# minyoungg/pix2latent

Hardware: AMD Instinct MI355X
Metric: candidate-latent evals/sec (fwd+loss+bwd), BigGAN-256 pop=18 (higher is better)
Workload: dtype f32 (fp32 tensors everywhere; convolutions >= 32x32 and the self-attention multiply on the 16-bit MFMA pipe with fp32-grade operand splits and fp32 accumulate: the 16x16 Winograd, direct and sub-pixel 3x3 kernels and the 1x1 kernels (4x4 layers included) on power-of-two scaled operands in 2 fp16 pie

## Files before the change

### include/p2l.h

```cpp
#ifndef P2L_H_
#define P2L_H_

#include <stddef.h>
#include <stdint.h>

#ifdef __cplusplus
extern "C" {
#endif

#define P2L_OK 0
#define P2L_EINVAL (-1)
#define P2L_ELAUNCH (-2)
#define P2L_EWS (-3)
#define P2L_EUNSUP (-4)

int p2l_version(void);
const char* p2l_strerror(int rc);
int p2l_last_hip_error(void);


enum { P2L_ACT_NONE = 0, P2L_ACT_RELU = 1, P2L_ACT_TANH = 2,
       P2L_ACT_LRELU_SQRT2 = 3  };
enum { P2L_POOL_NONE = 0, P2L_POOL_MAX = 1, P2L_POOL_SUM = 2 };
enum { P2L_PRO_NONE = 0, P2L_PRO_AFFINE_RELU = 1, P2L_PRO_AFFINE = 2 };
// ... 49 lines not shown
int p2l_conv_arb_nblk(const P2LConv* d);
int p2l_conv_dgrad_arb(const P2LConv* d, const P2LArb* arb, const float* dy,
                       const float* w, float* dx, void* stream);
int p2l_conv_arb_split_fusable(const P2LConv* d);
int p2l_conv_arb_nblk_ws(const P2LConv* d);
int p2l_conv_dgrad_arb_ws(const P2LConv* d, const P2LArb* arb, const float* dy, const float* w,
                          float* dx, void* workspace, size_t ws_bytes, void* stream);
int p2l_arb_finish(const float* partial, float* ds, float* dt, int Bn, int nblk, int C,
                   int out_bstride, void* stream);
void p2l_arb_defer_begin(void);
int p2l_arb_defer_flush(void* stream);
void p2l_arb_defer_cancel(void);

int p2l_prof_begin(int max_launches);
typedef struct P2LProfTotals {
  uint32_t size;
  int32_t count[2];
  int32_t reserved0;
  double flops[2];
  double ms[2];
  double bytes[2];
  double exec_flops[2];
  double mfma_flops[2];
  double write_bytes[2];
  int32_t fam_count[8];
  double fam_ms[8], fam_flops[8], fam_mfma_flops[8], fam_bytes[8];
} P2LProfTotals;
enum { P2L_PROF_FAM_OTHER = 0,
       P2L_PROF_FAM_WINO_H2 = 1,
       P2L_PROF_FAM_DIRECT_H2 = 2,
       P2L_PROF_FAM_SUBPIX_H2 = 3,
       P2L_PROF_FAM_THIN = 4,
       P2L_PROF_FAM_PW = 5,
       P2L_PROF_FAM_DIRECT_H2R = 6 };
int p2l_prof_totals(P2LProfTotals* out);
int p2l_prof_step(int step, int period);
int p2l_prof_dump(const char* path);

typedef struct P2LConvExtra {
  const float* oscale;
  int32_t oscale_bstride;
  const float* noise;
  float noise_w;
  P2LAmax amax;
} P2LConvExtra;
int p2l_conv_amax_slots(const P2LConv* d);
int p2l_conv_fwd_ex(const P2LConv* d, const P2LConvExtra* ex, const float* x,
                    const float* w, const float* bias, const float* pro_s,
                    const float* pro_t, const float* res, const float* mask, float* y,
                    float* yp, void* workspace, size_t ws_bytes, void* stream);

int p2l_pack_conv_weight(const float* w_oihw, int O, int I, int taps, int N_pad,
                         int K_pad, int transpose_flip, float* w_packed,
                         void* stream);

int p2l_pack_conv_weight_subpix(const float* w_oihw, int O, int I, int N_pad,
                                int K_pad, int transpose_flip, int mode,
                                float* w_packed, void* stream);

enum { P2L_WFMT_F32 = 0, P2L_WFMT_BF16X3 = 1, P2L_WFMT_BF16X3W = 2, P2L_WFMT_PW = 3,
       P2L_WFMT_BF16X3T = 4, P2L_WFMT_FLAG_PW = 0x10, P2L_WFMT_FLAG_THIN = 0x20,
       P2L_WFMT_FLAG_ATTN_GEMM = 0x40,
       P2L_WFMT_FLAG_NO_AMAX = 0x80
                                       };
int p2l_pack_conv_weight_bf3t(const float* w_oihw, int O, int I, int N_pad, int K_pad,
                              int transpose_flip, float* w_packed, void* stream);
int p2l_pack_conv_weight_pw(const float* w_oihw, int O, int I, int N_pad, int K_pad,
                            int transpose_flip, float* w_packed, void* stream);
size_t p2l_packed_weight_floats(int taps, int N_pad, int K_pad, int wfmt);
enum {
  P2L_FORM_AUTO = 0,
  P2L_FORM_NO_WINO = 1,
  P2L_FORM_WINO_ANY = 2,
  P2L_FORM_WINO_8X16 = 4,
  P2L_FORM_NO_PW = 8,
  P2L_FORM_NO_THIN = 16,
  P2L_FORM_WINO_BF3 = 32,
  P2L_FORM_WINO_H2_8X16 = 64,
  P2L_FORM_WINO_H2_16X16 = 128,
  P2L_FORM_NO_H2R = 256,
  P2L_FORM_H2R_SEQ_EPI = 512,
  P2L_FORM_NO_SP_SKIP = 1024,
  P2L_FORM_NO_SP_PAIR = 2048,
  P2L_FORM_SP_PAIR = 4096
};
int p2l_wino_split_factor(int H, int W, int Cin, int Cout);
int p2l_pack_conv_weight_bf3w(const float* w_oihw, int O, int I, int taps, int N_pad,
                              int K_pad, int transpose_flip, float* w_packed, void* stream);
int p2l_pack_conv_weight_bf3(const float* w_oihw, int O, int I, int taps, int N_pad,
                             int K_pad, int transpose_flip, float* w_packed, void* stream);
int p2l_pack_conv_weight_subpix_bf3(const float* w_oihw, int O, int I, int N_pad, int K_pad,
                                    int transpose_flip, int mode, float* w_packed,
                                    void* stream);
size_t p2l_packed_subpix_weight_floats(int N_pad, int K_pad, int wfmt);
int p2l_pack_conv_weight_subpix_h2(const float* w_oihw, int O, int I, int N_pad, int K_pad,
                                   int transpose_flip, int mode, float* w_packed, void* stream);

typedef struct P2LGemm {
  int32_t batch, M, N, K;
  int32_t lda, ldb, ldc;
  int64_t stride_a, stride_b, stride_c;
  int32_t a_kmajor, b_kmajor;
  float alpha;
  int32_t accumulate;
} P2LGemm;
int p2l_gemm(const P2LGemm* d, const float* A, const float* B, float* C,
             void* stream);
size_t p2l_gemm_ws_bytes(const P2LGemm* d);
int p2l_gemm_ws(const P2LGemm* d, const float* A, const float* B, float* C, void* ws,
                size_t ws_bytes, void* stream);

typedef struct P2LAttn {
  int32_t B, Nq, Nk, d, dv;
} P2LAttn;
int p2l_attn_supported(const P2LAttn* d);
size_t p2l_attn_fwd_ws_bytes(const P2LAttn* d);
int p2l_attn_fwd(const P2LAttn* d, const float* q, const float* k, const float* v, float* out,
                 float* lse, void* ws, size_t ws_bytes, void* stream);
size_t p2l_attn_bwd_dv_ws_bytes(const P2LAttn* d);
int p2l_attn_bwd_dv(const P2LAttn* d, const float* q, const float* k, const float* dout,
                    const float* lse, float* dv, void* ws, size_t ws_bytes, void* stream);
size_t p2l_attn_bwd_qk_ws_bytes(const P2LAttn* d);
int p2l_attn_bwd_qk(const P2LAttn* d, const float* q, const float* k, const float* v,
                    const float* out, const float* dout, const float* lse, float* dst, float* dq,
                    float* dk, void* ws, size_t ws_bytes, void* stream);

int p2l_linear_fwd(const float* x, const float* W, const float* bias, float* y,
                   int Bn, int K, int N, void* stream);
int p2l_linear_bwd(const float* dy, const float* W, float* dx, int Bn, int K,
                   int N, int accumulate, void* stream);
int p2l_linear_fwd_ld(const float* x, int x_ld, const float* W, const float* bias, float* y,
                      int Bn, int K, int N, void* stream);
int p2l_linear_bwd_ld(const float* dy, const float* W, float* dx, int dx_ld, int Bn, int K,
                      int N, int accumulate, void* stream);

int p2l_cbn_fold_fwd(const float* g_raw, const float* b_raw, const float* mean,
                     const float* rstd, float* s, float* t, int Bn, int C,
                     int raw_ld, void* stream);
int p2l_cbn_fold_bwd(const float* ds, const float* dt, const float* mean,
                     const float* rstd, float* dg_raw, float* db_raw, int Bn,
                     int C, int raw_ld, void* stream);

int p2l_affine_relu_bwd_nblk(int P);
int p2l_affine_relu_bwd(const float* da, int da_ld, const float* x, int x_ld,
                        const float* s, const float* t, int st_bstride,
                        const float* skip, int skip_ld, int skip_C, int skip_ups,
                        float* dx, int dx_ld, float* ds, float* dt,
                        int dsdt_bstride, float* partial, int Bn, int H, int W,
                        int C, void* stream);

int p2l_scale_bwd(const float* da, int da_ld, const float* x, int x_ld, const float* s,
                  int st_bstride, const float* skip, int skip_ld, int skip_C, float* dx,
                  int dx_ld, float* ds, float* dt_scratch, int dsdt_bstride, float* partial,
                  int Bn, int H, int W, int C, void* stream);

int p2l_softmax_fwd(const float* S, float* P, int64_t rows, int cols,
                    void* stream);
int p2l_softmax_bwd(const float* P, const float* dP, float* dS, int64_t rows,
                    int cols, void* stream);

int p2l_maxpool2_bwd(const float* y, int y_ld, const float* dyp, int dyp_ld,
                     const float* add, int add_ld, float* dy, int dy_ld, int Bn,
                     int H, int W, int C, int relu_mask, void* stream);
int p2l_maxpool2_bwd_amax_slots(int H, int W, int C);
int p2l_maxpool2_bwd_amax(const float* y, int y_ld, const float* dyp, int dyp_ld,
                          const float* add, int add_ld, float* dy, int dy_ld, int Bn, int H,
                          int W, int C, int relu_mask, float* amax_out, void* stream);
int p2l_relu_mask(const float* y, int y_ld, const float* g, int g_ld, float* dy,
// ... 364 lines not shown
```

### pix2latent_amd/_native.py

```python
import ctypes as C
import os

import torch

_HERE = os.path.dirname(os.path.abspath(__file__))
LIB_PATH = os.environ.get('P2L_LIB_PATH') or os.path.join(_HERE, 'libp2l_hip.so')

c_float_p = C.c_void_p


class P2LConv(C.Structure):
    _fields_ = [('B', C.c_int32), ('H', C.c_int32), ('W', C.c_int32),
                ('Cin', C.c_int32), ('Cout', C.c_int32), ('taps', C.c_int32),
                ('ups', C.c_int32), ('x_ld', C.c_int32), ('pro', C.c_int32),
                ('pro_bstride', C.c_int32), ('alpha', C.c_float), ('act', C.c_int32),
                ('pool', C.c_int32), ('y_ld', C.c_int32), ('yp_ld', C.c_int32),
                ('n_store', C.c_int32), ('res_ld', C.c_int32), ('res_ups', C.c_int32),
                ('mask_ld', C.c_int32), ('splitk', C.c_int32), ('ext', C.c_int32),
                ('wfmt', C.c_int32), ('form', C.c_int32), ('algo_flops', C.c_double),
                ('w_floats', C.c_int64)]


class P2LAmax(C.Structure):
    _fields_ = [('out', C.c_void_p), ('outp', C.c_void_p), ('in_', C.c_void_p), ('in_n', C.c_int32),
# ... 62 lines not shown


class P2LSg2Rgb(C.Structure):
    _fields_ = [('cin', C.c_int32), ('res', C.c_int32), ('latent_idx', C.c_int32),
                ('after_conv', C.c_int32), ('w', C.c_void_p), ('wt', C.c_void_p),
                ('mod_w', C.c_void_p), ('mod_b', C.c_void_p), ('bias', C.c_void_p)]


class P2LStyleGAN2(C.Structure):
    _fields_ = [('size', C.c_int32), ('n_conv', C.c_int32), ('n_rgb', C.c_int32),
                ('style_dim', C.c_int32), ('n_latent', C.c_int32), ('noise_total', C.c_int32),
                ('map_w', C.c_void_p * 8), ('map_b', C.c_void_p * 8), ('const_input', C.c_void_p),
                ('conv', P2LSg2Conv * P2L_SG2_MAX_CONVS), ('rgb', P2LSg2Rgb * P2L_SG2_MAX_RGBS),
                ('wfmt', C.c_int32), ('reserved1', C.c_int32)]


class P2LVggLpips(C.Structure):
    _fields_ = [('w', C.c_void_p * 13), ('b', C.c_void_p * 13), ('wt', C.c_void_p * 13),
                ('lin', C.c_void_p * 5), ('in_s', C.c_void_p), ('in_t', C.c_void_p),
                ('wfmt', C.c_int32), ('reserved1', C.c_int32)]


class P2LGConv(C.Structure):
    _fields_ = [(n, C.c_int32) for n in (
        'B', 'Hi', 'Wi', 'Cin', 'Cout', 'KH', 'KW', 'stride', 'pad', 'x_ld', 'y_ld', 'res_ld',
        'mask_ld', 'n_store', 'relu', 'reserved0')]


class P2LAlexLpips(C.Structure):
    _fields_ = [('w', C.c_void_p * 5), ('b', C.c_void_p * 5), ('wt', C.c_void_p * 5),
                ('lin', C.c_void_p * 5), ('in_s', C.c_void_p), ('in_t', C.c_void_p)]


class P2LSqueezeLpips(C.Structure):
    _fields_ = [('w0', C.c_void_p), ('b0', C.c_void_p), ('wt0', C.c_void_p),
                ('sq_w', C.c_void_p * 8), ('sq_b', C.c_void_p * 8), ('e1_w', C.c_void_p * 8), ('e1_b', C.c_void_p * 8),
                ('e3_w', C.c_void_p * 8), ('e3_b', C.c_void_p * 8),
                ('sq_wt', C.c_void_p * 8), ('e1_wt', C.c_void_p * 8), ('e3_wt', C.c_void_p * 8),
                ('lin', C.c_void_p * 7), ('in_s', C.c_void_p), ('in_t', C.c_void_p)]


class P2LLossCache7(C.Structure):
    _fields_ = [('nft', C.c_void_p * 7), ('wt', C.c_void_p * 7), ('wsum', C.c_void_p)]


class P2LLossCache(C.Structure):
    _fields_ = [('nft', C.c_void_p * 5), ('wt', C.c_void_p * 5), ('wsum', C.c_void_p)]


class P2LProfTotals(C.Structure):
    _fields_ = [('size', C.c_uint32), ('count', C.c_int32 * 2), ('reserved0', C.c_int32),
                ('flops', C.c_double * 2), ('ms', C.c_double * 2), ('bytes', C.c_double * 2),
                ('exec_flops', C.c_double * 2), ('mfma_flops', C.c_double * 2),
                ('write_bytes', C.c_double * 2),
                ('fam_count', C.c_int32 * 8), ('fam_ms', C.c_double * 8), ('fam_flops', C.c_double * 8),
                ('fam_mfma_flops', C.c_double * 8), ('fam_bytes', C.c_double * 8)]


PROF_FAMILIES = {0: 'other (exact-fp32 / bf16x3 direct, 8x16 Winograd)', 1: 'wino16s_conv_kernel<.., H2>',
                 2: 'conv_h2_kernel<9, ..>', 3: 'conv_h2_kernel<4, ..>', 4: 'conv_thinin/thinout_kernel',
                 5: 'pw_h2_kernel / pw_conv_kernel', 6: 'conv_h2r_kernel<..>'}


def prof_totals():
    t = P2LProfTotals()
    t.size = C.sizeof(P2LProfTotals)
    check(lib().p2l_prof_totals(C.byref(t)), 'p2l_prof_totals')
    return t


prof_end = prof_totals


ACT_NONE, ACT_RELU, ACT_TANH, ACT_LRELU_SQRT2 = 0, 1, 2, 3
WFMT_F32, WFMT_BF16X3, WFMT_BF16X3W, WFMT_PW, WFMT_BF16X3T = 0, 1, 2, 3, 4
WFMT_FLAG_PW, WFMT_FLAG_THIN, WFMT_FLAG_ATTN_GEMM, WFMT_FLAG_NO_AMAX = 0x10, 0x20, 0x40, 0x80
FORM_AUTO, FORM_NO_WINO, FORM_WINO_ANY, FORM_WINO_8X16, FORM_NO_PW, FORM_NO_THIN, FORM_WINO_BF3 = 0, 1, 2, 4, 8, 16, 32
FORM_WINO_H2_8X16, FORM_WINO_H2_16X16 = 64, 128
FORM_H2R_SEQ_EPI = 512
FORM_NO_SP_SKIP = 1024
FORM_NO_SP_PAIR = 2048
FORM_SP_PAIR = 4096
FORM_NO_H2R = 256


def default_wfmt():
    v = os.environ.get('P2L_CONV_WFMT', 'bf16x3').lower()
    if v in ('f32', 'fp32', '0'):
        return WFMT_F32
    if v in ('bf16x3-direct', 'bf3d', '1'):
        return WFMT_BF16X3
    if v in ('bf16x3', 'bf3', 'bf16x3w', '2'):
        return WFMT_BF16X3W
    raise ValueError('P2L_CONV_WFMT=%r (expected f32, bf16x3 or bf16x3-direct)' % v)


def default_thin():
    return os.environ.get('P2L_THIN', '1') != '0' and default_wfmt() != WFMT_F32


def default_attn_gemm():
    return os.environ.get('P2L_ATTN', '1') == '0'


def default_no_amax():
    return os.environ.get('P2L_AMAX', '1') == '0'


def default_pw():
    return os.environ.get('P2L_PW', '1') != '0' and default_wfmt() != WFMT_F32


def pack_conv_weight(src, taps, n_pad, k_pad, flip, wfmt, subpix_mode=None):
    L = lib()
    O, I = src.shape[0], src.shape[1]
    src = src.detach().float().contiguous()
    if taps == 1 and wfmt == WFMT_PW:
        dst = torch.empty(L.p2l_packed_weight_floats(1, n_pad, k_pad, WFMT_PW), device=src.device,
                          dtype=torch.float32)
        check(L.p2l_pack_conv_weight_pw(ptr(src), O, I, n_pad, k_pad, int(flip), ptr(dst), stream()),
              'p2l_pack_conv_weight_pw')
        return dst
    if taps != 9:
        wfmt = WFMT_F32
    if subpix_mode is not None:
        dst = torch.empty(L.p2l_packed_subpix_weight_floats(n_pad, k_pad, wfmt), device=src.device,
                          dtype=torch.float32)
        fn = {WFMT_F32: L.p2l_pack_conv_weight_subpix,
              WFMT_BF16X3W: L.p2l_pack_conv_weight_subpix_h2}.get(wfmt, L.p2l_pack_conv_weight_subpix_bf3)
        check(fn(ptr(src), O, I, n_pad, k_pad, int(flip), int(subpix_mode), ptr(dst), stream()),
              'p2l_pack_conv_weight_subpix')
        return dst
    n = L.p2l_packed_weight_floats(taps, n_pad, k_pad, wfmt)
    dst = torch.empty(n, device=src.device, dtype=torch.float32)
    if wfmt == WFMT_BF16X3T:
        check(L.p2l_pack_conv_weight_bf3t(ptr(src), O, I, n_pad, k_pad, int(flip), ptr(dst), stream()),
              'p2l_pack_conv_weight_bf3t')
        return dst
    fn = {WFMT_F32: L.p2l_pack_conv_weight, WFMT_BF16X3: L.p2l_pack_conv_weight_bf3,
          WFMT_BF16X3W: L.p2l_pack_conv_weight_bf3w}[wfmt]
    check(fn(ptr(src), O, I, taps, n_pad, k_pad, int(flip), ptr(dst), stream()),
          'p2l_pack_conv_weight')
    return dst
def pack_gconv_weight(src, taps, n_pad, k_pad, flip):
    L = lib()
    src = src.detach().float().contiguous()
    dst = torch.empty(taps * n_pad * k_pad, device=src.device, dtype=torch.float32)
    check(L.p2l_pack_gconv_weight(ptr(src), src.shape[0], src.shape[1], taps, n_pad, k_pad, int(flip), ptr(dst),
                                  stream()), 'p2l_pack_gconv_weight')
    return dst


POOL_NONE, POOL_MAX, POOL_SUM = 0, 1, 2
PRO_NONE, PRO_AFFINE_RELU, PRO_AFFINE = 0, 1, 2

EXPORTS = [
    'p2l_version', 'p2l_strerror', 'p2l_last_hip_error',
    'p2l_conv_workspace_bytes', 'p2l_conv_amax_slots', 'p2l_selftest_amaxreg', 'p2l_conv_suggest_splitk', 'p2l_conv_fwd', 'p2l_conv_fwd_ex',
    'p2l_pack_conv_weight', 'p2l_pack_conv_weight_subpix', 'p2l_pack_conv_weight_bf3',
    'p2l_pack_conv_weight_bf3w', 'p2l_packed_weight_floats', 
    'p2l_pack_conv_weight_bf3t',
    'p2l_pack_conv_weight_pw', 'p2l_adam_step_dev',
    'p2l_attn_supported', 'p2l_attn_fwd_ws_bytes', 'p2l_attn_fwd', 'p2l_attn_bwd_dv_ws_bytes',
    'p2l_attn_bwd_dv', 'p2l_attn_bwd_qk_ws_bytes', 'p2l_attn_bwd_qk',
    'p2l_pack_conv_weight_subpix_bf3', 'p2l_pack_conv_weight_subpix_h2', 'p2l_packed_subpix_weight_floats', 'p2l_gemm', 'p2l_gemm_ws_bytes', 'p2l_gemm_ws', 'p2l_linear_fwd', 'p2l_linear_bwd',
    'p2l_cbn_fold_fwd', 'p2l_cbn_fold_bwd', 'p2l_affine_relu_bwd_nblk',
    'p2l_affine_relu_bwd', 'p2l_softmax_fwd', 'p2l_softmax_bwd', 'p2l_maxpool2_bwd', 'p2l_maxpool2_bwd_amax', 'p2l_maxpool2_bwd_amax_slots',
    'p2l_relu_mask', 'p2l_nchw3_to_nhwc16', 'p2l_nhwc16_to_nchw3', 'p2l_tanh_bwd16',
    'p2l_weight_sum', 'p2l_weight_map', 'p2l_l1_loss_nblk', 'p2l_l1_loss_fwd',
    'p2l_l1_loss_bwd', 'p2l_lpips_normalize', 'p2l_lpips_tap_nblk', 'p2l_lpips_tap_fwd',
    'p2l_lpips_tap_bwd', 'p2l_lpips_tap_pool_bwd', 'p2l_bilinear_adjoint', 'p2l_reduce_rows', 'p2l_adam_step',
    'p2l_clamp', 'p2l_affine_grid_sample', 'p2l_affine_grid_sample_bwd', 'p2l_affine_grid_sample_bwd_ws_bytes', 'p2l_vec_scale_div', 'p2l_concat2', 'p2l_split2',
    'p2l_biggan_ws_bytes', 'p2l_biggan_fwd', 'p2l_biggan_bwd', 'p2l_biggan_ws_lookup',
    'p2l_loss_cache_floats', 'p2l_projloss_ws_bytes', 'p2l_projloss_ws_lookup', 'p2l_projloss_prepare',
    'p2l_projloss_fwd', 'p2l_projloss_bwd', 'p2l_mfma_probe', 'p2l_prof_begin', 'p2l_prof_totals', 'p2l_prof_step', 'p2l_prof_dump', 'p2l_wino_split_factor', 'p2l_linear_fwd_ld', 'p2l_linear_bwd_ld', 'p2l_scale_bwd',
    'p2l_sg2_pixelnorm_fwd', 'p2l_sg2_pixelnorm_bwd', 'p2l_sg2_bias_lrelu_fwd', 'p2l_sg2_lrelu_bwd',
    'p2l_sg2_demod_fwd', 'p2l_sg2_demod_bwd', 'p2l_sg2_blur_fwd', 'p2l_sg2_act_bwd_nblk',
    'p2l_sg2_styled_act_bwd', 'p2l_sg2_blur_bwd', 'p2l_sg2_rgb_up_fwd', 'p2l_sg2_rgb_up_bwd',
    'p2l_sg2_clamp16_fwd', 'p2l_sg2_clamp16_bwd', 'p2l_broadcast_rows', 'p2l_add_inplace',
    'p2l_sg2_ws_bytes', 'p2l_sg2_ws_lookup', 'p2l_sg2_synthesis_fwd', 'p2l_sg2_synthesis_bwd', 'p2l_sg2_mapping_fwd',
    'p2l_sg2_mapping_bwd', 'p2l_conv_arb_fusable', 'p2l_conv_arb_nblk',
    'p2l_conv_dgrad_arb', 'p2l_conv_arb_split_fusable', 'p2l_conv_arb_nblk_ws',
    'p2l_conv_dgrad_arb_ws', 'p2l_arb_finish', 'p2l_arb_defer_begin', 'p2l_arb_defer_flush',
    'p2l_arb_defer_cancel',
    'p2l_gconv_fwd', 'p2l_maxpool3s2_fwd', 'p2l_maxpool3s2_bwd', 'p2l_conv1_dgrad',
    'p2l_alex_cache_floats', 'p2l_alexloss_ws_bytes', 'p2l_alexloss_prepare', 'p2l_alexloss_fwd',
    'p2l_alexloss_bwd',
    'p2l_pack_gconv_weight', 'p2l_sqz_cache_floats', 'p2l_sqzloss_ws_bytes', 'p2l_sqzloss_prepare', 'p2l_sqzloss_fwd',
    'p2l_sqzloss_bwd', 'p2l_sqzloss_ws_lookup',
    'p2l_sg2_blur_fwd_amax', 'p2l_sg2_styled_act_bwd_amax', 'p2l_sg2_blur_bwd_amax', 'p2l_sg2_noise_relayout',
    'p2l_sg2_rows_defer_begin', 'p2l_sg2_rows_defer_flush', 'p2l_sg2_rows_defer_cancel',
    'p2l_color_adjust_ws_bytes', 'p2l_color_adjust',
    'p2l_gram_f64_ws_bytes', 'p2l_gram_f64', 'p2l_gram_f64_wide_ws_bytes', 'p2l_gram_f64_wide',
    'p2l_poisson_blend_ws_bytes', 'p2l_poisson_blend',
    'p2l_sg2_noise_reg_ws_bytes', 'p2l_sg2_noise_reg_fwd', 'p2l_sg2_noise_reg_bwd', 'p2l_sg2_noise_normalize',
    'p2l_area_pool3_to_nhwc16', 'p2l_area_pool_nchw', 'p2l_area_unpool16_add_nchw3',
    'p2l_latent_prior_ws_bytes', 'p2l_latent_prior_fwd', 'p2l_latent_prior_bwd',
    'p2l_l2_loss_nblk', 'p2l_l2_loss_fwd', 'p2l_l2_loss_bwd', 'p2l_adam_step_sched',
]

_lib = None
ABI_VERSION = 101


class NativeError(RuntimeError):
    pass


def lib():
    global _lib
    if _lib is None:
        if not os.path.exists(LIB_PATH):
            raise NativeError(
                'libp2l_hip.so not found at %s: the HIP extension is required '
                '(no CPU fallback). Run __graft_entry__.build().' % LIB_PATH)
        _lib = C.CDLL(LIB_PATH)
        if _lib.p2l_version() < ABI_VERSION:
            v, _lib = _lib.p2l_version(), None
            raise NativeError('libp2l_hip.so at %s is version %d, this package binds version %d: rebuild it '
                              '(__graft_entry__.build())' % (LIB_PATH, v, ABI_VERSION))
        _lib.p2l_strerror.restype = C.c_char_p
        _lib.p2l_arb_defer_begin.restype = None
        _lib.p2l_arb_defer_cancel.restype = None
        _lib.p2l_sg2_rows_defer_begin.restype = None
        _lib.p2l_sg2_rows_defer_cancel.restype = None
        for name in ('p2l_conv_workspace_bytes', 'p2l_biggan_ws_bytes',
                     'p2l_projloss_ws_bytes', 'p2l_loss_cache_floats', 'p2l_sg2_ws_bytes',
                     'p2l_alexloss_ws_bytes', 'p2l_alex_cache_floats', 'p2l_sqzloss_ws_bytes', 'p2l_sqz_cache_floats', 'p2l_gemm_ws_bytes',
                     'p2l_packed_weight_floats', 'p2l_packed_subpix_weight_floats', 'p2l_attn_fwd_ws_bytes', 'p2l_affine_grid_sample_bwd_ws_bytes',
                     'p2l_attn_bwd_dv_ws_bytes', 'p2l_attn_bwd_qk_ws_bytes', 'p2l_color_adjust_ws_bytes',
                     'p2l_gram_f64_ws_bytes', 'p2l_gram_f64_wide_ws_bytes', 'p2l_poisson_blend_ws_bytes',
                     'p2l_sg2_noise_reg_ws_bytes', 'p2l_latent_prior_ws_bytes'):
            getattr(_lib, name).restype = C.c_size_t
        vp, i32, i64_, f32_ = C.c_void_p, C.c_int, C.c_int64, C.c_float
        _lib.p2l_relu_mask.argtypes = [vp, i32, vp, i32, vp, i32, i64_, i32, vp]
        _lib.p2l_tanh_bwd16.argtypes = [vp, vp, i64_, vp]
        _lib.p2l_clamp.argtypes = [vp, i64_, f32_, f32_, vp]
        _lib.p2l_adam_step.argtypes = [vp, vp, vp, vp, i64_, f32_, f32_, f32_, f32_, i32, vp]
        _lib.p2l_adam_step_dev.argtypes = [vp, vp, vp, vp, i64_, f32_, f32_, f32_, f32_, vp, i32, vp]
        _lib.p2l_adam_step_sched.argtypes = [vp, vp, vp, vp, i64_, vp, i32, f32_, f32_, f32_, vp, i32, vp]
        _lib.p2l_l2_loss_nblk.argtypes = [i32, i32]
        _lib.p2l_l2_loss_fwd.argtypes = [vp, vp, vp, vp, vp, vp, vp, i32, i32, i32, vp]
        _lib.p2l_l2_loss_bwd.argtypes = [vp, vp, vp, vp, vp, vp, vp, i32, i32, i32, i32, vp]
        _lib.p2l_reduce_rows.argtypes = [vp, vp, i32, i32, f32_, vp, i32, vp]
        _lib.p2l_vec_scale_div.argtypes = [vp, vp, vp, i32, f32_, vp]
        _lib.p2l_sg2_bias_lrelu_fwd.argtypes = [vp, vp, f32_, i32, i32, vp]
        _lib.p2l_sg2_clamp16_fwd.argtypes = [vp, vp, i64_, vp]
        _lib.p2l_sg2_clamp16_bwd.argtypes = [vp, vp, vp, i64_, vp]
        _lib.p2l_broadcast_rows.argtypes = [vp, vp, i64_, i32, vp]
        _lib.p2l_add_inplace.argtypes = [vp, vp, i64_, vp]
        _lib.p2l_sg2_styled_act_bwd.argtypes = [vp, vp, vp, vp, f32_, vp, vp, vp, vp, vp, vp, i32, i32, i32, vp]
        _lib.p2l_sg2_styled_act_bwd_amax.argtypes = [vp, vp, vp, vp, f32_, vp, vp, vp, vp, vp, vp, i32, i32, i32, vp, vp]
        _lib.p2l_softmax_fwd.argtypes = [vp, vp, i64_, i32, vp]
        _lib.p2l_softmax_bwd.argtypes = [vp, vp, vp, i64_, i32, vp]
        _lib.p2l_sg2_blur_fwd.argtypes = [vp, vp, vp, f32_, vp, vp, i32, i32, i32, i32, vp]
        _lib.p2l_sg2_blur_fwd_amax.argtypes = [vp, vp, vp, f32_, vp, vp, i32, i32, i32, i32, vp, vp, vp]
        _lib.p2l_sg2_blur_bwd.argtypes = [vp, vp, i32, i32, i32, i32, vp]
        _lib.p2l_sg2_blur_bwd_amax.argtypes = [vp, vp, i32, i32, i32, i32, vp, vp]
        _lib.p2l_gram_f64_ws_bytes.argtypes = [C.c_int64, C.c_int, C.c_int]
        _lib.p2l_gram_f64.argtypes = [C.c_void_p, C.c_int64, C.c_int, C.c_int64, C.c_int, C.c_void_p,
                                      C.c_void_p, C.c_void_p, C.c_size_t, C.c_void_p]
        _lib.p2l_gram_f64_wide_ws_bytes.argtypes = [C.c_int64, C.c_int]
        _lib.p2l_gram_f64_wide.argtypes = [C.c_void_p, C.c_int64, C.c_int, C.c_int64, C.c_void_p, C.c_void_p,
                                           C.c_void_p, C.c_size_t, C.c_void_p]
        _lib.p2l_poisson_blend_ws_bytes.argtypes = [i32, i32, i32, i32]
        _lib.p2l_poisson_blend.argtypes = [vp, i64_, vp, i64_, vp, vp, i32, i32, i32, i32, C.c_double, i32,
                                           vp, vp, vp, C.c_size_t, vp]
        _lib.p2l_poisson_blend.restype = i32
        _lib.p2l_sg2_noise_reg_ws_bytes.argtypes = [vp, i32, i32]
        _lib.p2l_sg2_noise_reg_fwd.argtypes = [vp, vp, i32, i32, vp, vp, vp, C.c_size_t, vp]
        _lib.p2l_sg2_noise_reg_bwd.argtypes = [vp, vp, i32, i32, vp, vp, vp, C.c_size_t, vp]
        _lib.p2l_sg2_noise_normalize.argtypes = [vp, vp, i32, i32, vp, C.c_size_t, vp]
        _lib.p2l_area_pool3_to_nhwc16.argtypes = [vp, vp, i32, i32, i32, i32, vp]
        _lib.p2l_area_pool_nchw.argtypes = [vp, vp, vp, i32, i32, i32, i32, i32, vp]
        _lib.p2l_area_unpool16_add_nchw3.argtypes = [vp, vp, vp, i32, i32, i32, i32, vp]
        _lib.p2l_latent_prior_ws_bytes.argtypes = [i32, i32, i32]
        _lib.p2l_latent_prior_fwd.argtypes = [vp, vp, vp, vp, i32, i32, i32, i32, i32, vp, vp, C.c_size_t, vp]
        _lib.p2l_latent_prior_bwd.argtypes = [vp, vp, vp, vp, i32, i32, i32, i32, i32, vp, C.c_size_t, vp, vp]
    return _lib


def check(rc, what=''):
    if rc != 0:
        L = lib()
        raise NativeError('%s failed: %s (rc=%d, hipError=%d)' % (
            what or 'p2l call', L.p2l_strerror(rc).decode(), rc, L.p2l_last_hip_error()))


def ptr(t):
    if t is None:
        return C.c_void_p(0)
    assert t.dtype == torch.float32 and t.is_contiguous(), 'expect contiguous fp32'
    return C.c_void_p(t.data_ptr())


def stream():
    return C.c_void_p(torch.cuda.current_stream().cuda_stream)


def f32(v):
    return C.c_float(float(v))


def i64(v):
    return C.c_int64(int(v))
```

### pix2latent_amd/csrc/p2l_conv.hip

```cpp
#include "p2l_conv_k.h"

#include <cstdlib>
#include <cstring>
#include <cstddef>
#include <array>
#include <atomic>
#include <cstdio>
#include <mutex>
#include <string>
#include <vector>

using namespace p2lconv;

namespace {

struct ConvProf {
  std::atomic<bool> on{false};
  int n = 0;
  std::vector<hipEvent_t> ev;
  std::vector<double> flops;
  std::vector<double> xflops;
  std::vector<int> nprod;
  std::vector<double> bytes;
  std::vector<double> wbytes;
// ... 981 lines not shown
  const int nchunks = 4 * (d->Cin / 16);
  while (s > 1 && nchunks / s < 8) s >>= 1;
  return s <= 2 ? 1 : s;
}

extern "C" int p2l_conv_suggest_splitk(const P2LConv* d) {
  ConvK k{};
  if (d && d->ups == 3 && d->ext) return subpix_bwd_split(d);
  if (!d || d->ups >= 2) return 1;
  if (choose_tile(d, k) == P2L_OK && wino_split(d) > 1 && !(d->form & P2L_FORM_WINO_ANY) &&
      (d->H / 8) * (d->W / 16) * (d->Cout / 64) < 64)
    return wino_split(d);
  if (choose_tile(d, k) != P2L_OK || k.partial || wino_shape(d) || pw_any(d)) return 1;
  return direct_split(d);
}

static bool wino_h2(const P2LConv* d) {
  return wino_shape(d) && d->H % 16 == 0 && d->W % 16 == 0 &&
         !(d->form & (P2L_FORM_WINO_8X16 | P2L_FORM_WINO_BF3));
}
static int effective_splitk(const P2LConv* d);
static bool finish_v4_ok(const P2LConv* d) {
#ifdef P2L_AB_SCALAR_FINISH
  return false;
#endif
  return d->n_store % 4 == 0 && d->Cout % 4 == 0 && d->y_ld % 4 == 0 && d->yp_ld % 4 == 0 &&
         d->res_ld % 4 == 0 && d->mask_ld % 4 == 0;
}
extern "C" int p2l_conv_amax_slots(const P2LConv* d) {
  if (!d) return 0;
  if (wino_shape(d)) {
    if (d->H % 16 || d->W % 16 || (d->form & P2L_FORM_WINO_8X16)) return 0;
    if (d->splitk > 1 && wino_split(d) == d->splitk) {
      const int per_image = (d->H / 2) * (d->W / 2) * (d->n_store / 4);
      return (per_image % 64 == 0 && d->n_store % 4 == 0) ? per_image / 64 : 0;
    }
    return (d->H / 16) * (d->W / 16) * (d->Cout / 64) * 8;
  }
  if (d->ups == 3 && effective_splitk(d) > 1) return 0;
  if (effective_splitk(d) > 1) {
    const int per_image = (d->H / 2) * (d->W / 2) * (finish_v4_ok(d) ? d->n_store / 4 : d->n_store);
    return (per_image % 64 == 0) ? per_image / 64 : 0;
  }
  ConvK k{};
  if (choose_tile(d, k) != P2L_OK || k.tb_log != 0 || k.partial) return 0;
  const int tm = thin_shape(d);
  if (tm >= 0) {
    const bool geom = k.tw_log == 4 && k.th_log == 3;
    return (tm == 1 && geom) ? k.tiles_x * k.tiles_y * 4 : 0;
  }
#ifdef P2L_AB_PW_SLOTS_R4
  const int nnt = pw_shape(d) ? d->Cout / 64 : d->Cout / choose_bn(d, k.n_mtiles);
#else
  const int nnt = (pw_shape(d) || pw_small_h2(d)) ? d->Cout / 64 : direct_h2r(d) ? 1 : d->Cout / choose_bn(d, k.n_mtiles);
#endif
  return k.tiles_x * k.tiles_y * nnt * (d->ups == 2 ? 4 : 1) * 4;
}
extern "C" size_t p2l_conv_workspace_bytes(const P2LConv* d) {
  const size_t h2 = (wino_h2(d) || direct_h2(d) || pw_small_h2(d)) ? (size_t)d->B * 64 * sizeof(float) : 0;
  if (d->splitk <= 1) return h2;
  return h2 + (size_t)d->splitk * d->B * d->H * d->W * d->Cout * sizeof(float);
}

static int effective_splitk(const P2LConv* d) {
  if (d->splitk > 1 && d->ups == 3 && d->ext && subpix_bwd_split(d) > 1) {
    const int nchunks = 4 * (d->Cin / 16);
    const int sk = d->splitk > nchunks ? nchunks : d->splitk;
    return cdiv(nchunks, cdiv(nchunks, sk));
  }
  if (d->splitk > 1 && d->ups == 0 && wino_split(d) == d->splitk && wino_shape(d)) return d->splitk;
  if (d->splitk <= 1 || d->ups >= 2 || wino_shape(d) || pw_any(d)) return 1;
  const int kc = (d->taps == 9) ? 16 : (d->Cin % 32 == 0 ? 32 : 16);
  const int nchunks = d->Cin / kc;
  int sk = d->splitk > nchunks ? nchunks : d->splitk;
  const int per = cdiv(nchunks, sk);
  return cdiv(nchunks, per);
}

static int conv_launch_impl(const P2LConv* d, const P2LArb* arb, const P2LConvExtra* ex,
                            const float* x, const float* w,
                            const float* bias, const float* pro_s,
                            const float* pro_t, const float* res,
                            const float* mask, float* y, float* yp,
                            void* workspace, size_t ws_bytes, void* stream) {
  if (!d || !x || !w) return P2L_EINVAL;
  if (d->taps != 1 && d->taps != 9) return P2L_EINVAL;
  const int kc = (d->taps == 9) ? 16 : (d->Cin % 32 == 0 ? 32 : 16);
  if (d->Cin % kc || d->Cout % 32 || d->B < 1) return P2L_EINVAL;
  if (d->x_ld % 4 || d->x_ld < d->Cin) return P2L_EINVAL;
  if (d->pro != P2L_PRO_NONE && (!pro_s || !pro_t || d->pro_bstride % 4)) return P2L_EINVAL;
  if (d->pool != P2L_POOL_NONE && !yp) return P2L_EINVAL;
  if (!y && !yp) return P2L_EINVAL;
  if (d->ups && d->taps != 9) return P2L_EUNSUP;
  if (d->taps == 9 && d->wfmt != P2L_WFMT_F32 && d->wfmt != P2L_WFMT_BF16X3 &&
      d->wfmt != P2L_WFMT_BF16X3W && d->wfmt != P2L_WFMT_BF16X3T)
    return P2L_EUNSUP;
  if (d->taps == 1 && d->wfmt != P2L_WFMT_F32 && d->wfmt != P2L_WFMT_PW) return P2L_EUNSUP;
  if (d->ups < 0 || d->ups > 3) return P2L_EINVAL;
  if (d->w_floats != 0) {
    const size_t need = d->ups >= 2 ? p2l_packed_subpix_weight_floats(d->Cout, d->Cin, d->wfmt)
                                    : p2l_packed_weight_floats(d->taps, d->Cout, d->Cin, d->wfmt);
    if (d->w_floats < 0 || (size_t)d->w_floats < need) return P2L_EINVAL;
  }
  if (d->n_store < 1 || d->n_store > d->Cout || d->n_store % 4) return P2L_EINVAL;
  if ((y && d->y_ld % 4) || (yp && d->yp_ld % 4) || (res && d->res_ld % 4) ||
      (mask && d->mask_ld % 4))
    return P2L_EINVAL;
  if ((y && d->y_ld < d->n_store) || (yp && d->yp_ld < d->n_store) || (res && d->res_ld < d->n_store) ||
      (mask && d->mask_ld < d->n_store))
    return P2L_EINVAL;
  if (d->pro != P2L_PRO_NONE && d->pro_bstride != 0 && d->pro_bstride < d->Cin) return P2L_EINVAL;
  if (arb) {
    if (arb->x && arb->x_ld < d->n_store) return P2L_EINVAL;
    if (arb->st_bstride != 0 && arb->st_bstride < d->n_store) return P2L_EINVAL;
    if (arb->skip && (arb->skip_C < 0 || arb->skip_C > d->n_store || arb->skip_ld < arb->skip_C)) return P2L_EINVAL;
  }
  if (ex && ex->oscale && ex->oscale_bstride != 0 && ex->oscale_bstride < d->n_store) return P2L_EINVAL;
  {
    const int64_t px = (int64_t)d->B * d->H * d->W;
    int64_t ldmax = d->x_ld;
    if (d->y_ld > ldmax) ldmax = d->y_ld;
    if (d->res_ld > ldmax) ldmax = d->res_ld;
    if (d->mask_ld > ldmax) ldmax = d->mask_ld;
    if (px * ldmax >= ((int64_t)1 << 31)) return P2L_EUNSUP;
  }

  ConvK k{};
  k.x = x; k.w = w; k.bias = bias; k.pro_s = pro_s; k.pro_t = pro_t;
  k.res = res; k.mask = mask; k.y = y; k.yp = yp; k.ws = (float*)workspace;
  k.B = d->B; k.H = d->H; k.W = d->W; k.Cin = d->Cin; k.Cout = d->Cout;
  k.x_ld = d->x_ld; k.y_ld = d->y_ld; k.yp_ld = d->yp_ld; k.res_ld = d->res_ld;
  k.mask_ld = d->mask_ld; k.n_store = d->n_store; k.pro_bstride = d->pro_bstride;
  k.alpha = d->alpha; k.act = d->act; k.pool = d->pool; k.res_ups = d->res_ups;
  k.ups = d->ups;
  k.form = d->form;
  int rc = choose_tile(d, k);
  if (rc) return rc;
  k.iH = d->H; k.iW = d->W; k.ibH = d->H; k.ibW = d->W; k.obH = d->H; k.obW = d->W;
  k.hp = halo_pitch(1 << k.tw_log, d->wfmt != P2L_WFMT_F32 && d->taps == 9);
  const bool bf3_3x3 = d->taps == 9 && d->wfmt != P2L_WFMT_F32;
  if (ex) {
    k.oscale = ex->oscale; k.oscale_bstride = ex->oscale_bstride;
    k.noise = ex->noise; k.noise_w = ex->noise_w;
  }
  if ((k.oscale || k.noise || d->act == P2L_ACT_LRELU_SQRT2) && !finish_v4_ok(d) && !wino_shape(d) &&
      effective_splitk(d) > 1)
    return P2L_EUNSUP;
  if (k.partial && (arb || d->pool != P2L_POOL_NONE || d->splitk > 1)) return P2L_EUNSUP;
  if (arb) {
    if ((k.tb_log != 0 && effective_splitk(d) <= 1) || res || mask || d->act != P2L_ACT_NONE ||
        d->pool == P2L_POOL_MAX || !arb->x || !arb->s || !arb->t || !arb->partial)
      return P2L_EUNSUP;
    k.arb_x = arb->x; k.arb_s = arb->s; k.arb_t = arb->t; k.arb_skip = arb->skip;
    k.arb_partial = arb->partial; k.arb_x_ld = arb->x_ld; k.arb_bstride = arb->st_bstride;
    k.arb_skip_ld = arb->skip_ld; k.arb_skip_C = arb->skip_C; k.arb_skip_ups = arb->skip_ups;
    k.arb_nblk = k.n_mtiles / d->B;
    k.arb_nomask = arb->nomask;
  }
  const int bn = direct_h2r(d) ? 64 : choose_bn(d, k.n_mtiles);
  k.n_ntiles = d->Cout / bn;
  k.nchunks = d->Cin / kc;
  const bool wino_sliced = wino_shape(d) && d->splitk > 1 && wino_split(d) == d->splitk;
  k.splitk = (d->splitk < 1 || (wino_shape(d) && !wino_sliced) || pw_any(d)) ? 1 : d->splitk;
  if (k.splitk > k.nchunks) k.splitk = k.nchunks;
  k.chunks_per_split = cdiv(k.nchunks, k.splitk);
  k.splitk = cdiv(k.nchunks, k.chunks_per_split);
  const bool h2_direct = direct_h2(d), h2_pw_small = pw_small_h2(d);
  const size_t h2_bytes = (wino_h2(d) || h2_direct || h2_pw_small) ? (size_t)d->B * 64 * sizeof(float) : 0;
  const bool use_h2 = h2_bytes && workspace &&
                      ws_bytes >= h2_bytes + (k.splitk > 1 ? (size_t)k.splitk * d->B * d->H * d->W * d->Cout * sizeof(float) : 0);
  if (use_h2) {
    k.amax = (float*)workspace;
    k.ws = (float*)workspace + (size_t)d->B * 64;
  }
  {
    const P2LAmax* am = ex ? &ex->amax : (arb ? &arb->amax : nullptr);
    if (am && am->in && am->in_n > 0 && !(am->in_applied && d->pro == P2L_PRO_NONE) &&
        (use_h2 || (pw_shape(d) && !(d->form & P2L_FORM_WINO_BF3)))) {
      k.amax_in = am->in; k.amax_in_n = am->in_n;
      k.amax_in_applied = am->in_applied ? 1 : 0;
    }
    int nslots = (am && (am->out || am->outp)) ? p2l_conv_amax_slots(d) : 0;
    if (thin_shape(d) >= 0 && ex && (ex->oscale || ex->noise)) nslots = 0;
    if (nslots > 0 && h2_pw_small && !use_h2 && effective_splitk(d) <= 1) return P2L_EWS;
    if (nslots > 0 && direct_h2r(d) && !use_h2) return P2L_EWS;
    if (nslots > 0) { k.amax_out = am->out; k.amax_outp = am->outp; k.amax_out_n = nslots; }
    if (nslots > 0 && am->out && am->next_s && am->next_t && !arb) {
      if (am->next_bstride != 0 && am->next_bstride < d->n_store) return P2L_EINVAL;
      k.amax_ps = am->next_s; k.amax_pt = am->next_t; k.amax_pbstride = am->next_bstride;
    }
  }
  if (k.splitk > 1) {
    const size_t need = (use_h2 ? h2_bytes : 0) + (size_t)k.splitk * d->B * d->H * d->W * d->Cout * sizeof(float);
    if (!workspace || ws_bytes < need) return P2L_EWS;
    if (arb) k.arb_nblk = p2l_conv_arb_nblk_ws(d);
    if (arb && d->ups < 2 && !wino_shape(d) && finish_v4_ok(d) &&
        (arb->x_ld % 4 || (arb->skip && arb->skip_ld % 4)))
      return P2L_EINVAL;
  }
  hipStream_t st = (hipStream_t)stream;

  int prof_slot = -1;
  bool prof_ok = g_prof.on;
  if (prof_ok) {
    hipStreamCaptureStatus cs = hipStreamCaptureStatusNone;
    if (hipStreamIsCapturing(st, &cs) != hipSuccess || cs != hipStreamCaptureStatusNone) prof_ok = false;
  }
  if (prof_ok) {
    std::lock_guard<std::mutex> lk(g_prof.mu);
    if (g_prof.on && g_prof.n < (int)g_prof.flops.size() && (g_prof.seq++ % g_prof.period) == g_prof.phase)
      prof_slot = g_prof.n++;
  }
  if (prof_slot >= 0) {
    g_prof.flops[prof_slot] = d->algo_flops > 0.0
        ? d->algo_flops
        : 2.0 * d->B * d->H * d->W * (double)d->Cin * d->Cout * d->taps;
    g_prof.xflops[prof_slot] =
        2.0 * d->B * d->H * d->W * (double)d->Cin * d->Cout * (d->ups >= 2 ? 4 : d->taps);
    g_prof.kind[prof_slot] = d->taps == 9 ? 0 : 1;
    g_prof.fam[prof_slot] = P2L_PROF_FAM_OTHER;
    g_prof.nprod[prof_slot] = (d->wfmt == P2L_WFMT_F32 || (d->taps == 1 && !pw_shape(d))) ? 16 : 6;
    g_prof.shape[prof_slot] = {d->taps, d->B, d->H, d->W, d->Cin, d->Cout, d->ups, d->pro,
                               arb ? (arb->skip ? 2 : 1) : 0, d->splitk};
    {
      const double opx = (double)d->B * d->H * d->W;
      const double ipx = d->ups == 1 || d->ups == 2 ? opx / 4 : (d->ups == 3 ? opx * 4 : opx);
      double by = ipx * d->Cin + (double)d->taps * d->Cin * d->Cout;
      if (y) by += opx * d->n_store;
      if (yp) by += opx / 4 * d->n_store;
      if (res) by += (d->res_ups ? opx / 4 : opx) * d->n_store;
      if (mask) by += opx * d->n_store;
      if (arb) by += opx * d->n_store * (arb->skip ? 2.0 : 1.0);
      g_prof.bytes[prof_slot] = 4.0 * by;
      g_prof.wbytes[prof_slot] = 4.0 * ((y ? opx * d->n_store : 0.0) + (yp ? opx / 4 * d->n_store : 0.0));
    }
    (void)hipEventRecord(g_prof.ev[2 * prof_slot], st);
  }
  if (wino_shape(d)) {
    ConvK kw = k;
    kw.w = w + (size_t)9 * d->Cout * d->Cin * 3 / 2;
    if (use_h2) {
      kw.w += p2l_wino_weight_floats(d->Cout, d->Cin);
      kw.w_tail = reinterpret_cast<const unsigned*>(kw.w + (size_t)d->Cout * d->Cin * 16);
    }
    kw.tiles_x = d->W / 16; kw.tiles_y = d->H / 8;
    kw.n_mtiles = d->B * kw.tiles_x * kw.tiles_y;
    kw.n_ntiles = d->Cout / 64;
    kw.nchunks = d->Cin / 16;
    if (wino_sliced) {
      kw.splitk = d->splitk;
      kw.chunks_per_split = kw.nchunks / kw.splitk;
    } else {
      kw.splitk = 1;
    }
    rc = p2l_wino_launch(kw, d->pro, st);
    if (rc == P2L_OK && wino_sliced) {
      const size_t total = (size_t)k.B * (k.H >> 1) * (k.W >> 1) * (k.n_store >> 2);
      hipLaunchKernelGGL(conv_splitk_finish4, dim3(cdiv(total, 256)), dim3(256), 0, st, k);
      rc = p2l_check_launch();
    }
    if (prof_slot >= 0) {
      g_prof.xflops[prof_slot] = 2.0 * d->B * d->H * d->W * (double)d->Cin * d->Cout * 4;
      if (use_h2) g_prof.nprod[prof_slot] = 3;
      g_prof.fam[prof_slot] = use_h2 ? P2L_PROF_FAM_WINO_H2 : P2L_PROF_FAM_OTHER;
      (void)hipEventRecord(g_prof.ev[2 * prof_slot + 1], st);
    }
    return rc;
  }
  if (pw_shape(d)) {
    ConvK kp = k;
    kp.w = w + (size_t)d->Cout * d->Cin;
    if (k.amax_in != nullptr) {
      kp.w += (size_t)d->Cout * d->Cin * 3 / 2;
      kp.w_tail = reinterpret_cast<const unsigned*>(kp.w + (size_t)d->Cout * d->Cin);
    }
    kp.n_ntiles = d->Cout / 64;
    kp.nchunks = d->Cin / 64;
    kp.splitk = 1;
    rc = p2l_pw_launch(kp, d->pro, st);
    if (prof_slot >= 0) {
      if (k.amax_in != nullptr) g_prof.nprod[prof_slot] = 3;
      g_prof.fam[prof_slot] = P2L_PROF_FAM_PW;
      (void)hipEventRecord(g_prof.ev[2 * prof_slot + 1], st);
    }
    return rc;
  }
  {
    const int tm = thin_shape(d);
    const bool geom = k.tw_log == 4 && k.th_log == 3 && k.tb_log == 0 && !k.partial && !(ex && (ex->oscale || ex->noise));
    if (tm == 1 && geom) {
      ConvK kt = k;
      kt.w = w + (size_t)9 * d->Cout * d->Cin * 3 / 2;
      kt.splitk = 1;
      rc = p2l_thinin_launch(kt, d->pro, st);
      if (prof_slot >= 0) {
        g_prof.xflops[prof_slot] = 2.0 * d->B * d->H * d->W * 32.0 * d->Cout;
        g_prof.fam[prof_slot] = P2L_PROF_FAM_THIN;
        (void)hipEventRecord(g_prof.ev[2 * prof_slot + 1], st);
      }
      return rc;
    }
    if (tm == 0 && geom && !arb && !res && !mask && d->pool == P2L_POOL_NONE && y) {
      ConvK kt = k;
      kt.w = w + (size_t)9 * d->Cout * d->Cin * 3 / 2;
      kt.nchunks = d->Cin / 16;
      kt.splitk = 1;
      rc = p2l_thinout_launch(kt, d->pro, st);
      if (prof_slot >= 0) {
        g_prof.xflops[prof_slot] = 2.0 * d->B * d->H * d->W * 1.5 * d->Cin * 32.0;
        g_prof.fam[prof_slot] = P2L_PROF_FAM_THIN;
        (void)hipEventRecord(g_prof.ev[2 * prof_slot + 1], st);
      }
      return rc;
    }
  }
  if (d->ups >= 2) {
    const int sk3 = (d->taps == 9 && d->splitk > 1) ? ((d->ups == 3 && d->ext) ? effective_splitk(d) : 1) : 1;
    if (sk3 > 1 && !(use_h2 && direct_h2(d))) return P2L_EWS;
    if (d->taps != 9 || (k.splitk != 1 && sk3 == 1) || d->Cin % 16 || d->pool != P2L_POOL_NONE ||
        (arb && k.tb_log != 0 && sk3 == 1) || (d->ups == 2 && (res || mask)))
      return P2L_EUNSUP;
    {
      int gH, gW;
      grid_dims(d, gH, gW);
      const int e = d->ext ? 1 : 0, e2 = d->ext ? 2 : 0;
      k.H = gH; k.W = gW;
      if (d->ups == 2) {
        k.iH = d->H >> 1; k.iW = d->W >> 1; k.ibH = k.iH; k.ibW = k.iW;
        k.obH = d->H + e2; k.obW = d->W + e2;
      } else {
        k.iH = (d->H >> 1) + e; k.iW = (d->W >> 1) + e;
        k.ibH = d->H + e2; k.ibW = d->W + e2;
        k.obH = gH; k.obW = gW;
      }
    }
    k.sp_mode = d->ups - 1;
    k.sp_skip = (d->ext && !(d->form & P2L_FORM_NO_SP_SKIP)) ? 1 : 0;
    k.sp_ncc = d->Cin / 16;
    k.nchunks = (d->ups == 3) ? 4 * k.sp_ncc : k.sp_ncc;
    k.chunks_per_split = cdiv(k.nchunks, sk3);
    k.splitk = sk3;
    k.ups = 0;
    const int a_rows_sp = (1 << k.tb_log) * ((1 << k.th_log) + 2) * ((1 << k.tw_log) + 2);
    const bool small_sp = (a_rows_sp * 4 <= 3 * 256) && k.tb_log == 0;
    const bool bf3 = bf3_3x3;
    if (use_h2 && h2_direct) {
      ConvK kh = k;
      kh.hp = halo_pitch_h2(1 << k.tw_log);
      kh.w = w + (size_t)16 * d->Cout * d->Cin * 3 / 2;
      kh.w_tail = reinterpret_cast<const unsigned*>(kh.w + (size_t)16 * d->Cout * d->Cin);
      if (kh.amax_in == nullptr) {
        ConvK ka = kh;
        ka.H = k.ibH; ka.W = k.ibW;
        rc = p2l_amax_launch(ka, d->pro, st);
        if (rc) return rc;
      }
#ifdef P2L_AB_NO_SP_PAIR
      const bool pair = d->ups == 2 && !(d->form & P2L_FORM_NO_SP_PAIR) && (d->form & P2L_FORM_SP_PAIR);
#else
      const bool pair = d->ups == 2 && !(d->form & P2L_FORM_NO_SP_PAIR) &&
                        ((d->ext && bn == 64) || (d->form & P2L_FORM_SP_PAIR));
#endif
      rc = p2l_h2_launch(kh, d->pro, pair ? 8 : 4, bn, small_sp, st);
      if (rc == P2L_OK && k.splitk > 1) {
        const bool arb_al = !arb || (k.arb_x_ld % 4 == 0 && (!k.arb_skip || k.arb_skip_ld % 4 == 0));
        if (finish_v4_ok(d) && arb_al) {
          const size_t total = (size_t)k.B * (k.H >> 1) * (k.W >> 1) * (k.n_store >> 2);
          hipLaunchKernelGGL(conv_splitk_finish_v4, dim3(cdiv(total, 64)), dim3(256), 0, st, k);
        } else {
          const size_t total = (size_t)k.B * (k.H >> 1) * (k.W >> 1) * k.n_store;
          hipLaunchKernelGGL(conv_splitk_finish, dim3(cdiv(total, 64)), dim3(256), 0, st, k);
        }
        rc = p2l_check_launch();
      }
      if (prof_slot >= 0) {
        g_prof.nprod[prof_slot] = 3;
        g_prof.fam[prof_slot] = P2L_PROF_FAM_SUBPIX_H2;
        (void)hipEventRecord(g_prof.ev[2 * prof_slot + 1], st);
      }
      return rc;
    }
    const int a_lds_sp = (1 << k.tb_log) * ((1 << k.th_log) + 2) * k.hp;
    size_t lds_sp = (size_t)(a_lds_sp + 4 * bn) * (bf3 ? 24 : 20) * sizeof(float);
    const size_t lds_epi = (size_t)4 * 32 * (bn + 4) * sizeof(float);
    if (lds_epi > lds_sp) lds_sp = lds_epi;
    dim3 grid(k.n_mtiles * k.n_ntiles, d->ups == 2 ? 4 : 1), block(256);
#define P2L_LAUNCH_SP(BNV, AIT, PROV)                                                     \
    do {                                                                                  \
      if (bf3) { P2L_LAUNCH_SP2(BNV, AIT, PROV, true); } else { P2L_LAUNCH_SP2(BNV, AIT, PROV, false); } \
    } while (0)
#define P2L_LAUNCH_SP2(BNV, AIT, PROV, BF3V)                                              \
    do {                                                                                  \
      auto kfn = pick_kernel<4, BNV, 16, AIT, PROV, false, BF3V>();                       \
      static std::atomic<bool> attr_set{false};                                                       \
      if (!attr_set) {                                                                    \
        (void)hipFuncSetAttribute((const void*)kfn,                                       \
                                  hipFuncAttributeMaxDynamicSharedMemorySize, 160 * 1024); \
        attr_set = true;                                                                  \
      }                                                                                   \
      hipLaunchKernelGGL(kfn, grid, block, lds_sp, st, k);                                \
    } while (0)
#define P2L_LAUNCH_SP_PRO(BNV, AIT)                                                       \
    do {                                                                                  \
      if (d->pro == P2L_PRO_NONE) P2L_LAUNCH_SP(BNV, AIT, P2L_PRO_NONE);                  \
      else if (d->pro == P2L_PRO_AFFINE_RELU) P2L_LAUNCH_SP(BNV, AIT, P2L_PRO_AFFINE_RELU); \
      else P2L_LAUNCH_SP(BNV, AIT, P2L_PRO_AFFINE);                                       \
    } while (0)
    if (bn == 64) {
      if (small_sp) P2L_LAUNCH_SP_PRO(64, 3); else P2L_LAUNCH_SP_PRO(64, 5);
    } else {
      if (small_sp) P2L_LAUNCH_SP_PRO(32, 3); else P2L_LAUNCH_SP_PRO(32, 5);
    }
#undef P2L_LAUNCH_SP_PRO
#undef P2L_LAUNCH_SP
#undef P2L_LAUNCH_SP2
    rc = p2l_check_launch();
    if (prof_slot >= 0) (void)hipEventRecord(g_prof.ev[2 * prof_slot + 1], st);
    return rc;
  }
  const int TW = 1 << k.tw_log, TH = 1 << k.th_log, TB = 1 << k.tb_log;
  const int a_rows = (d->taps == 9) ? TB * (TH + 2) * (TW + 2) : 128;
  const bool bf3 = bf3_3x3;
  const int a_rows_lds = (d->taps == 9) ? TB * (TH + 2) * k.hp : 128;
  size_t lds = (size_t)(a_rows_lds + d->taps * bn) * (bf3 ? 24 : kc + 4) * sizeof(float);
  {
    const size_t lds_epi = (size_t)4 * 32 * (bn + 4) * sizeof(float);
    if (lds_epi > lds) lds = lds_epi;
  }

  if (d->taps == 9 && use_h2 && h2_direct) {
    ConvK kh = k;
    kh.hp = halo_pitch_h2(TW);
    kh.w = w + (size_t)9 * d->Cout * d->Cin * 3 / 2;
    if (p2l_wino_weight_ok(d->Cout, d->Cin))
      kh.w += p2l_wino_weight_floats(d->Cout, d->Cin) + p2l_wino_h2_weight_floats(d->Cout, d->Cin);
    kh.w_tail = reinterpret_cast<const unsigned*>(kh.w + (size_t)9 * d->Cout * d->Cin);
    if (kh.amax_in == nullptr) {
      rc = p2l_amax_launch(kh, d->pro, st);
      if (rc) return rc;
    }
    const bool small = (a_rows * 4 <= 3 * 256) && TB == 1;
    const bool h2r = direct_h2r(d) && k.splitk == 1 && !k.partial && TB == 1 && p2l_h2r_takes(kh);
    rc = h2r ? p2l_h2r_launch(kh, d->pro, st) : p2l_h2_launch(kh, d->pro, 9, bn, small, st);
    if (prof_slot >= 0) { g_prof.nprod[prof_slot] = 3; g_prof.fam[prof_slot] = h2r ? P2L_PROF_FAM_DIRECT_H2R : P2L_PROF_FAM_DIRECT_H2; }
  } else
  if (d->taps == 9) {
    const bool small = (a_rows * 4 <= 3 * 256) && TB == 1;
    if (bf3) {
      if (bn == 64) rc = small ? launch_conv<9, 64, 16, 3, true>(k, d->pro, d->ups, lds, st)
                               : launch_conv<9, 64, 16, 5, true>(k, d->pro, d->ups, lds, st);
      else          rc = small ? launch_conv<9, 32, 16, 3, true>(k, d->pro, d->ups, lds, st)
                               : launch_conv<9, 32, 16, 5, true>(k, d->pro, d->ups, lds, st);
    } else
    if (bn == 64) rc = small ? launch_conv<9, 64, 16, 3>(k, d->pro, d->ups, lds, st)
                             : launch_conv<9, 64, 16, 5>(k, d->pro, d->ups, lds, st);
    else          rc = small ? launch_conv<9, 32, 16, 3>(k, d->pro, d->ups, lds, st)
                             : launch_conv<9, 32, 16, 5>(k, d->pro, d->ups, lds, st);
  } else if (d->taps == 1 && use_h2 && h2_pw_small) {
    ConvK kp = k;
    kp.w = w + (size_t)d->Cout * d->Cin + (size_t)d->Cout * d->Cin * 3 / 2;
    kp.w_tail = reinterpret_cast<const unsigned*>(kp.w + (size_t)d->Cout * d->Cin);
    kp.n_ntiles = d->Cout / 64;
    if (kp.amax_in == nullptr) {
      rc = p2l_amax_launch(kp, d->pro, st);
      if (rc) return rc;
    }
    rc = p2l_pw_launch(kp, d->pro, st);
    if (prof_slot >= 0) { g_prof.nprod[prof_slot] = 3; g_prof.fam[prof_slot] = P2L_PROF_FAM_PW; }
  } else if (kc == 32) {
    if (bn == 64) rc = launch_conv<1, 64, 32, 4>(k, d->pro, 0, lds, st);
    else          rc = launch_conv<1, 32, 32, 4>(k, d->pro, 0, lds, st);
  } else {
    if (bn == 64) rc = launch_conv<1, 64, 16, 2>(k, d->pro, 0, lds, st);
    else          rc = launch_conv<1, 32, 16, 2>(k, d->pro, 0, lds, st);
  }
  if (rc) return rc;
  if (k.splitk > 1) {
    if (finish_v4_ok(d)) {
      const size_t total = (size_t)k.B * (k.H >> 1) * (k.W >> 1) * (k.n_store >> 2);
      hipLaunchKernelGGL(conv_splitk_finish_v4, dim3(cdiv(total, 64)), dim3(256), 0, st, k);
    } else {
      const size_t total = (size_t)k.B * (k.H >> 1) * (k.W >> 1) * k.n_store;
      hipLaunchKernelGGL(conv_splitk_finish, dim3(cdiv(total, 64)), dim3(256), 0, st, k);
    }
    rc = p2l_check_launch();
  }
  if (prof_slot >= 0) (void)hipEventRecord(g_prof.ev[2 * prof_slot + 1], st);
  return rc;
}

extern "C" int p2l_conv_fwd(const P2LConv* d, const float* x, const float* w,
                            const float* bias, const float* pro_s,
                            const float* pro_t, const float* res,
                            const float* mask, float* y, float* yp,
                            void* workspace, size_t ws_bytes, void* stream) {
  return conv_launch_impl(d, nullptr, nullptr, x, w, bias, pro_s, pro_t, res, mask, y, yp,
                          workspace, ws_bytes, stream);
}

extern "C" int p2l_conv_fwd_ex(const P2LConv* d, const P2LConvExtra* ex, const float* x,
                               const float* w, const float* bias, const float* pro_s,
                               const float* pro_t, const float* res, const float* mask,
                               float* y, float* yp, void* workspace, size_t ws_bytes,
                               void* stream) {
  return conv_launch_impl(d, nullptr, ex, x, w, bias, pro_s, pro_t, res, mask, y, yp, workspace,
                          ws_bytes, stream);
}

extern "C" int p2l_conv_arb_fusable(const P2LConv* d) {
  ConvK k{};
  if (!d || choose_tile(d, k) != P2L_OK) return 0;
  return k.tb_log == 0;
}

extern "C" int p2l_conv_arb_nblk(const P2LConv* d) {
  ConvK k{};
  if (!d || choose_tile(d, k) != P2L_OK) return 0;
  return k.n_mtiles / d->B;
}

extern "C" int p2l_conv_arb_split_fusable(const P2LConv* d) {
  ConvK k{};
  if (!d || choose_tile(d, k) != P2L_OK || k.partial) return 0;
  return effective_splitk(d) > 1 && d->pool != P2L_POOL_MAX;
}

extern "C" int p2l_conv_arb_nblk_ws(const P2LConv* d) {
  if (!d) return 0;
  const int sh = d->ups == 3 ? 2 : 1;
  return effective_splitk(d) > 1 ? (d->H >> sh) * (d->W >> sh) : p2l_conv_arb_nblk(d);
}

static int dgrad_arb_unsplit(const P2LConv* d, const P2LArb* arb, const float* dy, const float* w,
                             float* dx, void* workspace, size_t ws_bytes, void* stream);
static int arb_outputs_ok(const P2LConv* d, const P2LArb* arb) {
  if (!arb->ds || !arb->dt) return P2L_EINVAL;
  if (arb->dsdt_bstride % 4 || arb->dsdt_bstride < d->Cout) return P2L_EINVAL;
  return P2L_OK;
}
extern "C" int p2l_conv_dgrad_arb_ws(const P2LConv* d, const P2LArb* arb, const float* dy,
                                     const float* w, float* dx, void* workspace, size_t ws_bytes,
                                     void* stream) {
  if (!d || !arb || !dx) return P2L_EINVAL;
  if (int rc0 = arb_outputs_ok(d, arb)) return rc0;
  P2LConv dd = *d;
  if (dd.ups == 3) dd.pool = P2L_POOL_NONE;
  if (effective_splitk(&dd) <= 1) return dgrad_arb_unsplit(d, arb, dy, w, dx, workspace, ws_bytes, stream);
  const bool pooled = dd.pool == P2L_POOL_SUM;
  int rc = conv_launch_impl(&dd, arb, nullptr, dy, w, nullptr, nullptr, nullptr, nullptr, nullptr,
                            pooled ? nullptr : dx, pooled ? dx : nullptr, workspace, ws_bytes,
                            stream);
  if (rc) return rc;
  return p2l_arb_finish(arb->partial, arb->ds, arb->dt, dd.B, p2l_conv_arb_nblk_ws(&dd), dd.Cout,
                        arb->dsdt_bstride, stream);
}

static int dgrad_arb_unsplit(const P2LConv* d, const P2LArb* arb, const float* dy, const float* w,
                             float* dx, void* workspace, size_t ws_bytes, void* stream) {
  if (!d || !arb || !dx) return P2L_EINVAL;
  if (int rc0 = arb_outputs_ok(d, arb)) return rc0;
  P2LConv dd = *d;
  dd.splitk = 1;
  if (dd.ups == 3) dd.pool = P2L_POOL_NONE;
  const bool pooled = dd.pool == P2L_POOL_SUM;
  int rc = conv_launch_impl(&dd, arb, nullptr, dy, w, nullptr, nullptr, nullptr, nullptr, nullptr,
                            pooled ? nullptr : dx, pooled ? dx : nullptr, workspace, ws_bytes, stream);
  if (rc) return rc;
  const int nblk = p2l_conv_arb_nblk(&dd);
  return p2l_arb_finish(arb->partial, arb->ds, arb->dt, dd.B, nblk, dd.Cout,
                        arb->dsdt_bstride, stream);
}
extern "C" int p2l_conv_dgrad_arb(const P2LConv* d, const P2LArb* arb, const float* dy,
                                  const float* w, float* dx, void* stream) {
  return dgrad_arb_unsplit(d, arb, dy, w, dx, nullptr, 0, stream);
}

extern "C" int p2l_pack_conv_weight_subpix(const float* w_oihw, int O, int I, int N_pad,
                                           int K_pad, int transpose_flip, int mode,
                                           float* w_packed, void* stream) {
  if (!w_oihw || !w_packed || mode < 0 || mode > 1) return P2L_EINVAL;
  const int N = transpose_flip ? I : O, K = transpose_flip ? O : I;
  if (K_pad % 16 || N_pad % 32 || N_pad < N || K_pad < K) return P2L_EINVAL;
  const size_t total = (size_t)16 * K_pad * N_pad;
  hipLaunchKernelGGL(pack_subpix_kernel, dim3(cdiv(total, 256)), dim3(256), 0,
                     (hipStream_t)stream, w_oihw, w_packed, O, I, N_pad, K_pad, transpose_flip,
                     mode, 0);
  return p2l_check_launch();
}

// ... 200 lines not shown
```

### pix2latent_amd/csrc/p2l_conv_k.h

```cpp
#pragma once
#include "p2l_common.h"

namespace p2lconv {

struct ConvK {
  const float* x;
  const float* w;
  const float* bias;
  const float* pro_s;
  const float* pro_t;
  const float* res;
  const float* mask;
  float* y;
  float* yp;
  float* ws;
  int B, H, W, Cin, Cout;
  int x_ld, y_ld, yp_ld, res_ld, mask_ld, n_store;
  int pro_bstride;
  float alpha;
  int act, pool, res_ups, ups;
  int nchunks, chunks_per_split, splitk;
  int tw_log, th_log, tb_log;
  int tiles_x_log, tiles_y_log;
  int n_mtiles, n_ntiles;
// ... 163 lines not shown
  }
  const unsigned ppix = (unsigned)((b * (k.H >> 1) + (oy0 >> 1)) * (k.W >> 1) + (ox0 >> 1));

  if (!arb) {
    f32x4 bias4 = {0, 0, 0, 0};
    if (k.bias) bias4 = ld4(k.bias, (unsigned)n);
    f32x4 osc = {1.f, 1.f, 1.f, 1.f};
    if (k.oscale) osc = ld4(k.oscale, (unsigned)(b * k.oscale_bstride + n));
    f32x4 ns4 = {1.f, 1.f, 1.f, 1.f}, nt4 = {0, 0, 0, 0};
    if (k.amax_ps) { ns4 = ld4(k.amax_ps, (unsigned)(b * k.amax_pbstride + n)); nt4 = ld4(k.amax_pt, (unsigned)(b * k.amax_pbstride + n)); }
#pragma unroll
    for (int s = 0; s < 4; ++s) {
      if (!ok[s]) continue;
      const unsigned pix = pix0 + sub[s];
      f32x4 t = v[s] * osc + bias4;
      if (k.noise) t += k.noise_w * k.noise[(size_t)pix];
      if (k.res) t += ld4(k.res, (k.res_ups ? ppix : pix) * (unsigned)k.res_ld + (unsigned)n);
      t = act4(t, k.act);
      if (k.mask) {
        const f32x4 m = ld4(k.mask, pix * (unsigned)k.mask_ld + (unsigned)n);
        t.x = m.x > 0.f ? t.x : 0.f; t.y = m.y > 0.f ? t.y : 0.f;
        t.z = m.z > 0.f ? t.z : 0.f; t.w = m.w > 0.f ? t.w : 0.f;
      }
      if (k.y) st4(k.y, pix * (unsigned)k.y_ld + (unsigned)n, t);
      if (k.amax_out) S.amax = absmax4(S.amax, k.amax_ps ? t * ns4 + nt4 : t);
      v[s] = t;
    }
    if (k.pool) {
      f32x4 p;
      if (k.pool == P2L_POOL_MAX) {
        p.x = fmaxf(fmaxf(v[0].x, v[1].x), fmaxf(v[2].x, v[3].x));
        p.y = fmaxf(fmaxf(v[0].y, v[1].y), fmaxf(v[2].y, v[3].y));
        p.z = fmaxf(fmaxf(v[0].z, v[1].z), fmaxf(v[2].z, v[3].z));
        p.w = fmaxf(fmaxf(v[0].w, v[1].w), fmaxf(v[2].w, v[3].w));
      } else {
        p = (v[0] + v[1]) + (v[2] + v[3]);
      }
      st4(k.yp, ppix * (unsigned)k.yp_ld + (unsigned)n, p);
      if (k.amax_outp) S.amaxp = absmax4(S.amaxp, p);
    }
  } else {
    const f32x4 s4 = ld4(k.arb_s, (unsigned)(b * k.arb_bstride + n));
    const f32x4 t4 = ld4(k.arb_t, (unsigned)(b * k.arb_bstride + n));
    const bool has_skip = k.arb_skip && n < k.arb_skip_C;
    const int nv = pool_sum ? 1 : 4;
    if (pool_sum) v[0] = (v[0] + v[1]) + (v[2] + v[3]);
    float* dst = pool_sum ? k.yp : k.y;
    const unsigned dld = (unsigned)(pool_sum ? k.yp_ld : k.y_ld);
#pragma unroll
    for (int s = 0; s < 4; ++s) {
      if (s < nv) {
        const unsigned pix = pool_sum ? ppix : pix0 + sub[s];
        const f32x4 xv = ld4(k.arb_x, pix * (unsigned)k.arb_x_ld + (unsigned)n);
        const f32x4 pre = xv * s4 + t4;
        f32x4 g = v[s];
        if (!k.arb_nomask) {
          g.x = pre.x > 0.f ? g.x : 0.f; g.y = pre.y > 0.f ? g.y : 0.f;
          g.z = pre.z > 0.f ? g.z : 0.f; g.w = pre.w > 0.f ? g.w : 0.f;
        }
        f32x4 o = g * s4;
        if (has_skip) {
          const unsigned ld = (unsigned)k.arb_skip_ld;
          if (k.arb_skip_ups) {
            const int Wo = pool_sum ? (k.W >> 1) : k.W, Ho = pool_sum ? (k.H >> 1) : k.H;
            const int yy = pool_sum ? (oy0 >> 1) : oy0 + (s >> 1);
            const int xx = pool_sum ? (ox0 >> 1) : ox0 + (s & 1);
            const unsigned W2 = 2u * (unsigned)Wo;
            const unsigned cq = ((unsigned)(b * 2 * Ho + 2 * yy)) * W2 + 2u * (unsigned)xx;
            o += (ld4(k.arb_skip, cq * ld + n) + ld4(k.arb_skip, (cq + 1) * ld + n)) +
                 (ld4(k.arb_skip, (cq + W2) * ld + n) + ld4(k.arb_skip, (cq + W2 + 1) * ld + n));
          } else {
            o += ld4(k.arb_skip, pix * ld + (unsigned)n);
          }
        }
        st4(dst, pix * dld + (unsigned)n, o);
        if (k.amax_out || k.amax_outp) { if (pool_sum) S.amaxp = absmax4(S.amaxp, o); else S.amax = absmax4(S.amax, o); }
        S.sgx += g * xv;
        S.sg += g;
      }
    }
  }
}

template <int COLS, int C4>
__device__ __forceinline__ void epi_arb_reduce(const ConvK& k, EpiSums& S, float* smem, int wave,
                                               int lane, int tid, size_t slot, int n0,
                                               const EpiSums* S2 = nullptr) {
  f32x4 sgx = S.sgx, sg = S.sg;
  f32x4 sgx2 = {0, 0, 0, 0}, sg2 = {0, 0, 0, 0};
  if (C4 == 16 && S2 != nullptr) { sgx2 = S2->sgx; sg2 = S2->sg; }
#pragma unroll
  for (int o = C4; o < 64; o <<= 1) {
    sgx.x += __shfl_xor(sgx.x, o, 64); sgx.y += __shfl_xor(sgx.y, o, 64);
    sgx.z += __shfl_xor(sgx.z, o, 64); sgx.w += __shfl_xor(sgx.w, o, 64);
    sg.x += __shfl_xor(sg.x, o, 64); sg.y += __shfl_xor(sg.y, o, 64);
    sg.z += __shfl_xor(sg.z, o, 64); sg.w += __shfl_xor(sg.w, o, 64);
    if (C4 == 16 && S2 != nullptr) {
      sgx2.x += __shfl_xor(sgx2.x, o, 64); sgx2.y += __shfl_xor(sgx2.y, o, 64);
      sgx2.z += __shfl_xor(sgx2.z, o, 64); sgx2.w += __shfl_xor(sgx2.w, o, 64);
      sg2.x += __shfl_xor(sg2.x, o, 64); sg2.y += __shfl_xor(sg2.y, o, 64);
      sg2.z += __shfl_xor(sg2.z, o, 64); sg2.w += __shfl_xor(sg2.w, o, 64);
    }
  }
  if (C4 == 16 && S2 != nullptr) { sgx = sgx + sgx2; sg = sg + sg2; }
  __syncthreads();
  float* red = smem;
  if (lane < C4 && wave < 4) {
    *reinterpret_cast<f32x4*>(red + wave * COLS + lane * 4) = sgx;
    *reinterpret_cast<f32x4*>(red + (4 + wave) * COLS + lane * 4) = sg;
  }
  __syncthreads();
  if (tid < COLS && n0 + tid < k.n_store) {
    const float a = (red[tid] + red[COLS + tid]) + (red[2 * COLS + tid] + red[3 * COLS + tid]);
    const float t = (red[4 * COLS + tid] + red[5 * COLS + tid]) +
                    (red[6 * COLS + tid] + red[7 * COLS + tid]);
    const size_t o = slot * k.Cout + n0 + tid;
    k.arb_partial[o] = a;
    k.arb_partial[(size_t)k.B * k.arb_nblk * k.Cout + o] = t;
  }
}

template <int NT>
__device__ __forceinline__ void epilogue_vec_items(const ConvK& k, float* smem, int wave, int lane, int b0,
                                                   int y0, int x0, int n0, int tile_in_image, int osh,
                                                   int ph_y, int ph_x);
template <int NT>
__device__ __forceinline__ void epilogue_vec(const ConvK& k, const f32x16 (&acc)[NT],
                                             float* smem, int wave, int lane, int b0, int y0,
                                             int x0, int n0, int tile_in_image, int osh,
                                             int ph_y, int ph_x) {
  constexpr int COLS = NT * 32, EP = COLS + 4;
  const int l31 = lane & 31, lhi = lane >> 5;
  float* tb = smem + wave * 32 * EP;
#pragma unroll
  for (int j = 0; j < NT; ++j)
#pragma unroll
    for (int r = 0; r < 16; ++r)
      tb[((r & 3) + 8 * (r >> 2) + 4 * lhi) * EP + j * 32 + l31] = acc[j][r];
  __syncthreads();
  epilogue_vec_items<NT>(k, smem, wave, lane, b0, y0, x0, n0, tile_in_image, osh, ph_y, ph_x);
}
template <int NT>
__device__ __forceinline__ void epilogue_vec_items(const ConvK& k, float* smem, int wave, int lane, int b0,
                                                   int y0, int x0, int n0, int tile_in_image, int osh,
                                                   int ph_y, int ph_x) {
  constexpr int COLS = NT * 32, EP = COLS + 4, C4 = COLS / 4, ITEMS = 8 * C4;
  float* tb = smem + wave * 32 * EP;

  const int TWh = (1 << k.tw_log) >> 1, THh = (1 << k.th_log) >> 1;
  EpiSums S, S2;
#pragma unroll
  for (int it0 = 0; it0 < ITEMS; it0 += 64) {
    EpiSums& Sx = (it0 == 0) ? S : S2;
    const int it = it0 + lane;
    const int q = it / C4, c4 = it - q * C4;
    const int n = n0 + c4 * 4;
    const int Q = wave * 8 + q;
    const int qx = Q & (TWh - 1), qy = (Q >> (k.tw_log - 1)) & (THh - 1);
    const int b = b0 + (Q >> (k.tw_log + k.th_log - 2));
    if (b >= k.B || n >= k.n_store) continue;
    const int oy0 = y0 + 2 * qy, ox0 = x0 + 2 * qx;
    f32x4 v[4];
#pragma unroll
    for (int s = 0; s < 4; ++s)
      v[s] = *reinterpret_cast<const f32x4*>(tb + (4 * q + s) * EP + c4 * 4) * k.alpha;
    epi_item(k, v, b, oy0, ox0, n, osh, ph_y, ph_x, Sx);
  }
  static_assert(ITEMS == 64 || ITEMS == 128, "one or two items per lane");
  if (k.arb_x != nullptr)
    epi_arb_reduce<COLS, C4>(k, S, smem, wave, lane, threadIdx.x,
                             (size_t)b0 * k.arb_nblk + tile_in_image, n0, &S2);
  S.amax = fmaxf(S.amax, S2.amax); S.amaxp = fmaxf(S.amaxp, S2.amaxp);
  if (k.amax_out != nullptr || k.amax_outp != nullptr) {
    float m = S.amax, mp = S.amaxp;
#pragma unroll
    for (int o = 1; o < 64; o <<= 1) { m = fmaxf(m, __shfl_xor(m, o, 64)); mp = fmaxf(mp, __shfl_xor(mp, o, 64)); }
    if (lane == 0) {
      const int nph = osh ? 4 : 1;
      const size_t slot = (size_t)b0 * k.amax_out_n +
                          (((size_t)tile_in_image * k.n_ntiles + n0 / COLS) * nph + (osh ? ph_y * 2 + ph_x : 0)) * 4 + wave;
      if (k.amax_out != nullptr) k.amax_out[slot] = m;
      if (k.amax_outp != nullptr) k.amax_outp[slot] = mp;
    }
  }
}


}

int p2l_pw_launch(const p2lconv::ConvK& k, int pro, hipStream_t st);

size_t p2l_thin_weight_floats(int N_pad, int K_pad);
int p2l_thin_mode(int N_pad, int K_pad);
int p2l_thin_pack(const float* w_oihw, int O, int I, int N_pad, int K_pad, int flip, float* dst,
                  hipStream_t st);
int p2l_thinin_launch(const p2lconv::ConvK& k, int pro, hipStream_t st);
int p2l_thinout_launch(const p2lconv::ConvK& k, int pro, hipStream_t st);

extern "C" size_t p2l_wino_weight_floats(int N_pad, int K_pad);
extern "C" int p2l_wino_weight_ok(int N_pad, int K_pad);
extern "C" int p2l_wino_split_factor(int H, int W, int Cin, int Cout);
extern "C" size_t p2l_wino_h2_weight_floats(int N_pad, int K_pad);
extern "C" size_t p2l_pw_h2_weight_floats(int N_pad, int K_pad);
int p2l_pw_pack_h2(const float* w_oihw, int O, int I, int N_pad, int K_pad, int flip, float* dst, hipStream_t st);
int p2l_wino_pack(const float* w_oihw, int O, int I, int N_pad, int K_pad, int transpose_flip,
                  float* dst, hipStream_t st);
int p2l_wino_launch(const p2lconv::ConvK& k, int pro, hipStream_t st);
int p2l_amax_launch(const p2lconv::ConvK& k, int pro, hipStream_t st);

size_t p2l_h2_weight_floats(int N_pad, int K_pad, int subpix);
int p2l_h2_pack(const float* w_oihw, int O, int I, int N_pad, int K_pad, int flip, int mode, float* dst,
                hipStream_t st);
int p2l_h2_launch(const p2lconv::ConvK& k, int pro, int taps, int bn, bool small, hipStream_t st);

bool p2l_h2r_shape(int taps, int ups, int H, int W, int Cin, int Cout, int x_ld);
bool p2l_h2r_takes(const p2lconv::ConvK& k);
int p2l_h2r_launch(const p2lconv::ConvK& k, int pro, hipStream_t st);
```

### pix2latent_amd/csrc/p2l_h2.hip

```cpp
#include "p2l_conv_k.h"

#include <atomic>
#include <type_traits>

using namespace p2lconv;

namespace {

#ifndef P2L_H2_ABL
#define P2L_H2_ABL 0
#endif

__device__ __forceinline__ int h2c(int c, int row) { return c ^ ((row >> 2) & 3) ^ (((row >> 1) & 1) << 1); }

#define P2L_WAIT(VM, LGKM) __builtin_amdgcn_s_waitcnt(((VM) & 15) | (7 << 4) | ((LGKM) << 8) | (((VM) >> 4) << 14))

template <int TAPS, int BN, int A_ITERS, int PRO, bool SKIP = false>
__global__ __launch_bounds__(256, 2) void conv_h2_kernel(const ConvK k) {
  constexpr bool SUBPIX = (TAPS == 4 || TAPS == 8);
  constexpr int NP = (TAPS == 8) ? 2 : 1;
  constexpr int NT = BN / 32;
  constexpr int B_ITEMS = TAPS * BN * 4;
  constexpr int B_ITERS = (B_ITEMS + 255) / 256;
  constexpr int SL = SUBPIX ? 16 : TAPS;
  constexpr int T0 = (TAPS == 4) ? 2 : 4;
  constexpr int NU = TAPS * NT, U0 = T0 * NT;
  constexpr int H0 = U0 * 128;
  static_assert(H0 % 256 == 0, "half 0 must be whole DMA instructions");
  constexpr int NH1_MIN = (B_ITEMS - H0) / 256;
  constexpr bool S_UNI = (A_ITERS == 3);
  constexpr int S_ITERS = S_UNI ? 1 : A_ITERS;
  constexpr int NA_LD = A_ITERS + ((PRO != P2L_PRO_NONE) ? 2 * S_ITERS : 0);

  extern __shared__ __attribute__((aligned(16))) float smem[];

  const int tid = threadIdx.x;
  const int lane = tid & 63, wave = tid >> 6;
  const int l31 = lane & 31, lhi = lane >> 5;

  const int TW = 1 << k.tw_log, TH = 1 << k.th_log, TB = 1 << k.tb_log;
  const int HW_ = TW + 2, HH_ = TH + 2;
  const int HP = k.hp;
  const int a_rows = TB * HH_ * HW_;
  const int a_rows_lds = TB * HH_ * HP;
  char* As = reinterpret_cast<char*>(smem);
  char* Bs = As + (size_t)a_rows_lds * 64;
  const int main_floats = max(a_rows_lds * 16 + TAPS * BN * 16, 4 * 32 * (BN + 4));
  float* scl = smem + main_floats;

  const int swz = xcd_remap(blockIdx.x, gridDim.x);
  const int mt = swz / k.n_ntiles, nt = swz - mt * k.n_ntiles;
  const int tiles_per_image = k.tiles_x * k.tiles_y;
  const int bt = mt / tiles_per_image;
  const int tile_in_image = mt - bt * tiles_per_image;
  const int ty = tile_in_image / k.tiles_x, tx = tile_in_image - ty * k.tiles_x;
  const int n0 = nt * BN;
  const int y0 = ty << k.th_log, x0 = tx << k.tw_log, b0 = bt << k.tb_log;

  const bool sp_fwd = SUBPIX && (TAPS == 8 || k.sp_mode == 1);
  const bool sp_bwd = (TAPS == 4) && k.sp_mode == 2;
  const int z = sp_fwd ? 0 : blockIdx.y;
  const int ph_y = sp_fwd ? (TAPS == 8 ? (int)blockIdx.y : (int)(blockIdx.y >> 1)) : 0;
  const int ph_x = (sp_fwd && TAPS == 4) ? (int)(blockIdx.y & 1) : 0;
  const int c_begin = z * k.chunks_per_split;
  const int c_end = min(k.nchunks, c_begin + k.chunks_per_split);

  const int av = tid & 3;
  int a_goff[A_ITERS];
  int a_soff[A_ITERS];
  int a_row[A_ITERS];
  float a_xs[S_ITERS];
  int a_tb[S_ITERS];
  unsigned a_valid = 0;
#pragma unroll
  for (int it = 0; it < A_ITERS; ++it) {
    const int p = (tid + 256 * it) >> 2;
    a_goff[it] = 0;
    a_soff[it] = 0;
    a_row[it] = -1;
    if (it < S_ITERS) { a_xs[it] = 1.f; a_tb[it] = 0; }
    if (p < a_rows) {
      const int tb = p / (HH_ * HW_);
      const int rem = p - tb * (HH_ * HW_);
      const int hy = rem / HW_, hx = rem - hy * HW_;
      const int iy = y0 + hy - 1, ix = x0 + hx - 1;
      a_row[it] = (tb * HH_ + hy) * HP + hx;
      const int b = b0 + tb;
      if (!S_UNI) a_tb[it] = tb;
      if (b < k.B && iy >= 0 && iy < k.iH && ix >= 0 && ix < k.iW) {
        int pix;
        if (sp_bwd)
          pix = (b * k.ibH + 2 * iy) * k.ibW + 2 * ix;
        else
          pix = (b * k.ibH + iy) * k.ibW + ix;
        a_goff[it] = pix * k.x_ld + av * 4;
        a_soff[it] = b * k.pro_bstride + av * 4;
        a_valid |= 1u << it;
      }
    }
  }
  const int s_uni = b0 * k.pro_bstride + av * 4;
// ... 221 lines not shown
        const int tn = (u + 1) / NT, jn = (u + 1) - tn * NT;
        if (!(SUBPIX && SKIP) || ((live >> tn) & 1u)) {
          if (jn == 0) lda(tn, af[tn & 1]);
          ldb(u + 1, bq[(u + 1) & 1]);
        }
      }
      __builtin_amdgcn_sched_barrier(0);
      const h16x8 (&a)[2] = af[tap & 1];
      const h16x8 (&b)[2] = bq[u & 1];
      if (SUBPIX && SKIP && !((live >> tap) & 1u)) continue;
      const int ja = (TAPS == 8) ? (tap >> 2) * NT + j : j;
      if (!(P2L_H2_ABL & 8)) {
      acc[ja] = __builtin_amdgcn_mfma_f32_32x32x16_f16(a[1], b[0], acc[ja], 0, 0, 0);
      acc[ja] = __builtin_amdgcn_mfma_f32_32x32x16_f16(a[0], b[1], acc[ja], 0, 0, 0);
      acc[ja] = __builtin_amdgcn_mfma_f32_32x32x16_f16(a[0], b[0], acc[ja], 0, 0, 0);
      } else { acc[ja][0] += (float)a[0][0] * (float)b[0][0]; }
      __builtin_amdgcn_sched_barrier(0);
    }
    P2L_WAIT(63, 0);
    if (!(P2L_H2_ABL & 16)) __builtin_amdgcn_s_barrier();
    if (more) {
      if (!(P2L_H2_ABL & 1)) write_a();
      __builtin_amdgcn_sched_barrier(0);
      const bool more2 = (c + 2 < c_end);
      if (!(P2L_H2_ABL & 4)) dma_b(c + 1, H1c{});
      __builtin_amdgcn_sched_barrier(0);
      if (more2 && !(P2L_H2_ABL & 2)) load_a(c + 2);
      __builtin_amdgcn_sched_barrier(0);
      if (more2) P2L_WAIT(NA_LD + NH1_MIN, 0); else P2L_WAIT(NH1_MIN, 0);
    } else {
      P2L_WAIT(63, 0);
    }
    if (!(P2L_H2_ABL & 16)) __builtin_amdgcn_s_barrier();
  }

  if (S_UNI) {
    const float os = scl[1];
#pragma unroll
    for (int j = 0; j < NP * NT; ++j)
#pragma unroll
      for (int r = 0; r < 16; ++r) acc[j][r] *= os;
  } else {
#pragma unroll
    for (int g = 0; g < 4; ++g) {
      const int Q = wave * 8 + 2 * g + lhi;
      const float os = scl[2 * (Q >> (k.tw_log + k.th_log - 2)) + 1];
#pragma unroll
      for (int j = 0; j < NP * NT; ++j)
#pragma unroll
        for (int s = 0; s < 4; ++s) acc[j][4 * g + s] *= os;
    }
  }

  if (k.splitk > 1) {
    const size_t mtot = (size_t)k.B * k.H * k.W;
#pragma unroll
    for (int g = 0; g < 4; ++g) {
      const int Q = wave * 8 + 2 * g + lhi;
      const int qx = Q & ((TW >> 1) - 1);
      const int qy = (Q >> (k.tw_log - 1)) & ((TH >> 1) - 1);
      const int b = b0 + (Q >> (k.tw_log + k.th_log - 2));
      if (b >= k.B) continue;
      const size_t pix0 = ((size_t)b * k.H + y0 + 2 * qy) * k.W + x0 + 2 * qx;
#pragma unroll
      for (int j = 0; j < NT; ++j) {
        float* wp = k.ws + ((size_t)z * mtot + pix0) * k.Cout + n0 + j * 32 + l31;
        wp[0] = acc[j][g * 4 + 0];
        wp[k.Cout] = acc[j][g * 4 + 1];
        wp[(size_t)k.W * k.Cout] = acc[j][g * 4 + 2];
        wp[(size_t)(k.W + 1) * k.Cout] = acc[j][g * 4 + 3];
      }
    }
  } else {
    __syncthreads();
    if (!(P2L_H2_ABL & 32) || acc[0][0] == 12345.678f) {
      if (TAPS == 8) {
#pragma unroll
        for (int p = 0; p < NP; ++p) {
          if (p) __syncthreads();
          epilogue_vec<NT>(k, reinterpret_cast<f32x16 (&)[NT]>(acc[p * NT]), smem, wave, lane, b0, y0, x0, n0,
                           tile_in_image, 1, ph_y, p);
        }
      } else {
        epilogue_vec<NT>(k, reinterpret_cast<f32x16 (&)[NT]>(acc[0]), smem, wave, lane, b0, y0, x0, n0, tile_in_image,
                         sp_fwd ? 1 : 0, ph_y, ph_x);
      }
    }
  }
}
#undef P2L_WAIT

__global__ void h2_wmax_kernel(const float* w, size_t n, unsigned* tail) {
  float mx = 0.f;
  for (size_t i = (size_t)blockIdx.x * 256 + threadIdx.x; i < n; i += (size_t)gridDim.x * 256)
    mx = fmaxf(mx, fabsf(w[i]));
#pragma unroll
  for (int o = 1; o < 64; o <<= 1) mx = fmaxf(mx, __shfl_xor(mx, o, 64));
  if ((threadIdx.x & 63) == 0) atomicMax(tail, __builtin_bit_cast(unsigned, mx));
}
__global__ void h2_tail_x4_kernel(unsigned* tail) {
  const float m = __builtin_bit_cast(float, tail[0]);
  tail[0] = __builtin_bit_cast(unsigned, m > 0.f && m < 1e37f ? 4.f * m : m);
}

__device__ __forceinline__ unsigned h2_sp_tapset(int mode, int flip, int p, int i) {
  if (mode == 0) {
    if (!flip) {
      if (p == 0) return i == 0 ? 1u : 6u;
      return i == 0 ? 3u : 4u;
    }
    const int u = 2 * i - p;
    return u == 2 ? 1u : u == 0 ? 6u : u == 1 ? 3u : 4u;
  }
  if (!flip) {
    if (p == 0) return i == 0 ? 4u : 1u;
    return i == 0 ? 2u : 0u;
  }
  if (p == 0) return i == 0 ? 1u : 4u;
  return i == 0 ? 0u : 2u;
}

__global__ __launch_bounds__(256) void h2_pack_kernel(const float* __restrict__ src, float* __restrict__ dst,
                                                      int O, int I, int N_pad, int K_pad, int flip,
                                                      int mode, const unsigned* tail) {
  const int n_slabs = mode < 0 ? 9 : 16;
  const size_t total = (size_t)(K_pad >> 4) * (N_pad >> 5) * n_slabs * 32 * 2;
  const size_t idx = (size_t)blockIdx.x * 256 + threadIdx.x;
  if (idx >= total) return;
  float scale, inv;
  h2_scales(tail[0], scale, inv);
  const int kh = (int)(idx & 1);
  size_t r = idx >> 1;
  const int row = (int)(r & 31); r >>= 5;
  const int slab = (int)(r % n_slabs); r /= n_slabs;
  const int tile = (int)(r % (N_pad >> 5));
  const int q = (int)(r / (N_pad >> 5));
  const int n = tile * 32 + row;
  const bool n_ok = flip ? (n < I) : (n < O);
  h16x8 ph, pm;
  for (int e = 0; e < 8; ++e) {
    const int c = q * 16 + kh * 8 + e;
    const bool ok = n_ok && (flip ? (c < O) : (c < I));
    float v = 0.f;
    if (ok) {
      if (mode < 0) {
        v = flip ? src[((size_t)c * I + n) * 9 + (8 - slab)] : src[((size_t)n * I + c) * 9 + slab];
      } else {
        const int ph_ = slab >> 2, tap = slab & 3;
        const unsigned my = h2_sp_tapset(mode, flip, ph_ >> 1, tap >> 1);
        const unsigned mx = h2_sp_tapset(mode, flip, ph_ & 1, tap & 1);
        for (int dy = 0; dy < 3; ++dy)
          for (int dx = 0; dx < 3; ++dx)
            if (((my >> dy) & 1u) && ((mx >> dx) & 1u))
              v += flip ? src[((size_t)c * I + n) * 9 + dy * 3 + dx]
                        : src[((size_t)n * I + c) * 9 + dy * 3 + dx];
      }
    }
    const float x = v * scale;
    const _Float16 h = (_Float16)x;
    ph[e] = h; pm[e] = (_Float16)(x - (float)h);
  }
  char* rb = reinterpret_cast<char*>(dst) +
             ((((size_t)q * (N_pad >> 5) + tile) * n_slabs + slab) * 32 + row) * 64;
  *reinterpret_cast<h16x8*>(rb + h2c(kh, row) * 16) = ph;
  *reinterpret_cast<h16x8*>(rb + h2c(2 + kh, row) * 16) = pm;
}

}

size_t p2l_h2_weight_floats(int N_pad, int K_pad, int subpix) {
  return (size_t)N_pad * K_pad * (subpix ? 16 : 9) + 4;
}
int p2l_h2_pack(const float* w_oihw, int O, int I, int N_pad, int K_pad, int flip, int mode, float* dst,
                hipStream_t st) {
  const int n_slabs = mode < 0 ? 9 : 16;
  unsigned* tail = reinterpret_cast<unsigned*>(dst + (size_t)N_pad * K_pad * n_slabs);
  if (hipMemsetAsync(tail, 0, 16, st) != hipSuccess) return P2L_ELAUNCH;
  const size_t nw = (size_t)O * I * 9;
  hipLaunchKernelGGL(h2_wmax_kernel, dim3((unsigned)(cdiv(nw, 256) < 256 ? cdiv(nw, 256) : 256)), dim3(256), 0, st,
                     w_oihw, nw, tail);
  if (mode >= 0) hipLaunchKernelGGL(h2_tail_x4_kernel, dim3(1), dim3(1), 0, st, tail);
  const size_t total = (size_t)(K_pad >> 4) * (N_pad >> 5) * n_slabs * 32 * 2;
  hipLaunchKernelGGL(h2_pack_kernel, dim3(cdiv(total, 256)), dim3(256), 0, st, w_oihw, dst, O, I, N_pad, K_pad,
                     flip, mode, tail);
  return p2l_check_launch();
}

size_t p2l_h2_lds_bytes(const ConvK& k, int taps, int bn) {
  const int TB = 1 << k.tb_log, TH = 1 << k.th_log;
  const int a_rows_lds = TB * (TH + 2) * k.hp;
  int main_floats = a_rows_lds * 16 + taps * bn * 16;
  const int epi = 4 * 32 * (bn + 4);
  if (epi > main_floats) main_floats = epi;
  return (size_t)(main_floats + 2 * TB + 16) * sizeof(float);
}

int p2l_h2_launch(const ConvK& k, int pro, int taps, int bn, bool small, hipStream_t st) {
  dim3 grid(k.n_mtiles * k.n_ntiles, taps == 8 ? 2 : (taps == 4 && k.sp_mode == 1) ? 4 : k.splitk), block(256);
  const size_t lds = p2l_h2_lds_bytes(k, taps, bn);
#define P2L_H2L(TAPS, BNV, AIT, PROV)                                                         \
  do {                                                                                        \
    if ((TAPS == 4 || TAPS == 8) && k.sp_skip) P2L_H2K(TAPS, BNV, AIT, PROV, (TAPS == 4 || TAPS == 8)); \
    else P2L_H2K(TAPS, BNV, AIT, PROV, false);                                                \
  } while (0)
#define P2L_H2K(TAPS, BNV, AIT, PROV, SKIPV)                                                  \
  do {                                                                                        \
    auto kfn = conv_h2_kernel<TAPS, BNV, AIT, PROV, SKIPV>;                                   \
    static std::atomic<bool> attr_set{false};                                                 \
    if (!attr_set) {                                                                          \
      (void)hipFuncSetAttribute((const void*)kfn, hipFuncAttributeMaxDynamicSharedMemorySize, \
                                160 * 1024);                                                  \
      attr_set = true;                                                                        \
    }                                                                                         \
    hipLaunchKernelGGL(kfn, grid, block, lds, st, k);                                         \
  } while (0)
#define P2L_H2P(TAPS, BNV, AIT)                                                               \
  do {                                                                                        \
    if (pro == P2L_PRO_NONE) P2L_H2L(TAPS, BNV, AIT, P2L_PRO_NONE);                           \
    else if (pro == P2L_PRO_AFFINE_RELU) P2L_H2L(TAPS, BNV, AIT, P2L_PRO_AFFINE_RELU);        \
    else P2L_H2L(TAPS, BNV, AIT, P2L_PRO_AFFINE);                                             \
  } while (0)
  if (taps == 9) {
    if (bn == 64) { if (small) P2L_H2P(9, 64, 3); else P2L_H2P(9, 64, 5); }
    else          { if (small) P2L_H2P(9, 32, 3); else P2L_H2P(9, 32, 5); }
  } else if (taps == 8) {
    if (bn == 64) { if (small) P2L_H2P(8, 64, 3); else P2L_H2P(8, 64, 5); }
    else          { if (small) P2L_H2P(8, 32, 3); else P2L_H2P(8, 32, 5); }
  } else {
    if (bn == 64) { if (small) P2L_H2P(4, 64, 3); else P2L_H2P(4, 64, 5); }
    else          { if (small) P2L_H2P(4, 32, 3); else P2L_H2P(4, 32, 5); }
  }
#undef P2L_H2P
#undef P2L_H2L
#undef P2L_H2K
  return p2l_check_launch();
}
```

### pix2latent_amd/csrc/p2l_pw.hip

```cpp
#include "p2l_conv_k.h"
#include <type_traits>

#include <atomic>

using namespace p2lconv;

namespace {

template <int KS> struct PwCfg {
  static constexpr int SUB = KS / 16;
  static constexpr int A_FLOATS = SUB * 128 * 24;
  static constexpr int B_FLOATS = SUB * 64 * 24;
  static constexpr size_t LDS_BYTES = (size_t)(A_FLOATS + B_FLOATS) * sizeof(float);
};

__device__ __forceinline__ void pw_store_split(float* As, int row, int q4, const f32x4 x) {
  bf16x4 ph, pm, pl;
  split3(x, ph, pm, pl);
  char* rb = reinterpret_cast<char*>(As) + row * 96 + (q4 & 1) * 8;
  char* rq = rb + bf3_chunk(q4 >> 1, row) * 16;
  *reinterpret_cast<bf16x4*>(rq) = ph;
  *reinterpret_cast<bf16x4*>(rq + 32) = pm;
  *reinterpret_cast<bf16x4*>(rq + 64) = pl;
}
// ... 59 lines not shown
  auto write_lds = [&]() {
#pragma unroll
    for (int it = 0; it < A_ITERS; ++it) {
      f32x4 v = xr[it];
      if (PRO != P2L_PRO_NONE) {
        v = v * sr + tr;
        if (PRO == P2L_PRO_AFFINE_RELU) {
          v.x = fmaxf(v.x, 0.f); v.y = fmaxf(v.y, 0.f);
          v.z = fmaxf(v.z, 0.f); v.w = fmaxf(v.w, 0.f);
        }
      }
      const int p = (tid + 256 * it) / VPP;
      pw_store_split(As + (av >> 2) * (128 * 24), p, av & 3, v);
    }
#pragma unroll
    for (int it = 0; it < B_ITERS; ++it)
      *reinterpret_cast<f32x4*>(Bs + (tid + 256 * it) * 4) = wr[it];
  };

  f32x16 acc[2];
#pragma unroll
  for (int j = 0; j < 2; ++j)
#pragma unroll
    for (int r = 0; r < 16; ++r) acc[j][r] = 0.f;

  const int a_row = wave * 32 + l31;
  const int a_c = bf3_chunk(lhi, a_row) * 4, b_c = bf3_chunk(lhi, l31) * 4;
  const int nstages = k.Cin / KS;
  load_regs(0);
  write_lds();
  __syncthreads();
  for (int st = 0; st < nstages; ++st) {
    const bool more = st + 1 < nstages;
    if (more) load_regs(st + 1);
#pragma unroll
    for (int sub = 0; sub < PW_SUB; ++sub) {
      const float* ar = As + (sub * 128 + a_row) * 24 + a_c;
      const bf16x8 a1 = *reinterpret_cast<const bf16x8*>(ar);
      const bf16x8 a2 = *reinterpret_cast<const bf16x8*>(ar + 8);
      const bf16x8 a3 = *reinterpret_cast<const bf16x8*>(ar + 16);
#pragma unroll
      for (int j = 0; j < 2; ++j) {
        const float* br = Bs + (sub * 64 + j * 32 + l31) * 24 + b_c;
        const bf16x8 b1 = *reinterpret_cast<const bf16x8*>(br);
        const bf16x8 b2 = *reinterpret_cast<const bf16x8*>(br + 8);
        const bf16x8 b3 = *reinterpret_cast<const bf16x8*>(br + 16);
        f32x16 t = acc[j];
        t = __builtin_amdgcn_mfma_f32_32x32x16_bf16(a3, b1, t, 0, 0, 0);
        t = __builtin_amdgcn_mfma_f32_32x32x16_bf16(a1, b3, t, 0, 0, 0);
        t = __builtin_amdgcn_mfma_f32_32x32x16_bf16(a2, b2, t, 0, 0, 0);
        t = __builtin_amdgcn_mfma_f32_32x32x16_bf16(a2, b1, t, 0, 0, 0);
        t = __builtin_amdgcn_mfma_f32_32x32x16_bf16(a1, b2, t, 0, 0, 0);
        t = __builtin_amdgcn_mfma_f32_32x32x16_bf16(a1, b1, t, 0, 0, 0);
        acc[j] = t;
      }
    }
    __syncthreads();
    if (more) write_lds();
    __syncthreads();
  }
  epilogue_vec<2>(k, acc, smem, wave, lane, b0, y0, x0, n0, tile_in_image, 0, 0, 0);
}


constexpr int PWH_SUB = 2;
constexpr int PWH_A_FLOATS = PWH_SUB * 128 * 16, PWH_B_FLOATS = PWH_SUB * 64 * 16;
constexpr int PWH_EPI_FLOATS = 4 * 32 * (64 + 4);
constexpr size_t PWH_LDS_BYTES =
    (size_t)(PWH_A_FLOATS + PWH_B_FLOATS > PWH_EPI_FLOATS ? PWH_A_FLOATS + PWH_B_FLOATS : PWH_EPI_FLOATS) * sizeof(float);
__device__ __forceinline__ int h2_chunk(int c, int row) { return c ^ ((row >> 2) & 3); }
__device__ __forceinline__ int h2_chunk_a(int c, int row, int sub) { return h2_chunk(c, row) ^ ((sub & 1) << 1); }
__device__ __forceinline__ void pw_store_split_h2(float* As, int row, int q4, int sub, const f32x4 x) {
  const h16x4 h = __builtin_convertvector(x, h16x4);
  const f32x4 w = __builtin_convertvector(h, f32x4);
  const h16x4 m = __builtin_convertvector(x - w, h16x4);
  char* rb = reinterpret_cast<char*>(As) + row * 64 + (q4 & 1) * 8;
  *reinterpret_cast<h16x4*>(rb + h2_chunk_a(q4 >> 1, row, sub) * 16) = h;
  *reinterpret_cast<h16x4*>(rb + h2_chunk_a(2 + (q4 >> 1), row, sub) * 16) = m;
}

#ifndef P2L_PW_ABL
#define P2L_PW_ABL 0
#endif
template <int PRO, bool SM = false>
__global__ __launch_bounds__(256, SM ? 3 : 4) void pw_h2_kernel(const ConvK k) {
  constexpr int KS = 32, VPP = KS / 4;
  constexpr int A_ITERS = 128 * VPP / 256;
  extern __shared__ __attribute__((aligned(16))) float smem[];
  float* As = smem;
  float* Bs = smem + PWH_A_FLOATS;
  float* scl = smem + PWH_LDS_BYTES / sizeof(float);

  const int tid = threadIdx.x;
  const int lane = tid & 63, wave = tid >> 6;
  const int l31 = lane & 31, lhi = lane >> 5;

  const int TW = 1 << k.tw_log, TH = 1 << k.th_log;
  const int swz = xcd_remap(blockIdx.x, gridDim.x);
  const int mt = swz / k.n_ntiles, nt = swz - mt * k.n_ntiles;
  const int tiles_per_image = k.tiles_x * k.tiles_y;
  const int bt = mt / tiles_per_image;
  const int b0 = SM ? (bt << k.tb_log) : bt;
  const int tile_in_image = mt - bt * tiles_per_image;
  const int ty = tile_in_image / k.tiles_x, tx = tile_in_image - ty * k.tiles_x;
  const int n0 = nt * 64;
  const int y0 = ty << k.th_log, x0 = tx << k.tw_log;

  float x_scale = 1.f, out_scale = 1.f;
  {
    float sw, inv_w;
    h2_scales(__builtin_amdgcn_readfirstlane(k.w_tail[0]), sw, inv_w);
    if (!SM) {
      float a = 0.f, ms = 0.f, mt_ = 0.f;
      for (int i = tid; i < k.amax_in_n; i += 256) a = fmaxf(a, k.amax_in[(size_t)b0 * k.amax_in_n + i]);
      const bool bound = PRO != P2L_PRO_NONE && !k.amax_in_applied;
      if (bound) {
        const float* ps = k.pro_s + (size_t)b0 * k.pro_bstride;
        const float* pt = k.pro_t + (size_t)b0 * k.pro_bstride;
        for (int c = tid; c < k.Cin; c += 256) { ms = fmaxf(ms, fabsf(ps[c])); mt_ = fmaxf(mt_, fabsf(pt[c])); }
      }
#pragma unroll
      for (int o = 1; o < 64; o <<= 1) {
        a = fmaxf(a, __shfl_xor(a, o, 64));
        if (PRO != P2L_PRO_NONE) { ms = fmaxf(ms, __shfl_xor(ms, o, 64)); mt_ = fmaxf(mt_, __shfl_xor(mt_, o, 64)); }
      }
      if (lane == 0) { smem[wave * 4] = a; smem[wave * 4 + 1] = ms; smem[wave * 4 + 2] = mt_; }
      __syncthreads();
      a = fmaxf(fmaxf(smem[0], smem[4]), fmaxf(smem[8], smem[12]));
      ms = fmaxf(fmaxf(smem[1], smem[5]), fmaxf(smem[9], smem[13]));
      mt_ = fmaxf(fmaxf(smem[2], smem[6]), fmaxf(smem[10], smem[14]));
      __syncthreads();
      if (PRO != P2L_PRO_NONE) a = (bound ? ms * a + mt_ : a) * 1.001f;
      float inv_x;
      h2_scales(__builtin_amdgcn_readfirstlane(__builtin_bit_cast(unsigned, a)), x_scale, inv_x);
      out_scale = inv_x * inv_w;
    } else {
      const int TBn = 1 << k.tb_log;
      for (int t = wave; t < TBn; t += 4) {
        const int b = b0 + t;
        float a = 0.f, ms = 0.f, mt_ = 0.f;
        if (b < k.B) {
          if (k.amax_in != nullptr) {
            for (int i = lane; i < k.amax_in_n; i += 64) a = fmaxf(a, k.amax_in[(size_t)b * k.amax_in_n + i]);
            if (PRO != P2L_PRO_NONE && !k.amax_in_applied) {
              const f32x4* ps = reinterpret_cast<const f32x4*>(k.pro_s + (size_t)b * k.pro_bstride);
              const f32x4* pt = reinterpret_cast<const f32x4*>(k.pro_t + (size_t)b * k.pro_bstride);
              for (int c = lane; c < (k.Cin >> 2); c += 64) {
                const f32x4 s4 = ps[c], t4 = pt[c];
                ms = fmaxf(fmaxf(ms, fmaxf(fabsf(s4.x), fabsf(s4.y))), fmaxf(fabsf(s4.z), fabsf(s4.w)));
                mt_ = fmaxf(fmaxf(mt_, fmaxf(fabsf(t4.x), fabsf(t4.y))), fmaxf(fabsf(t4.z), fabsf(t4.w)));
              }
            }
          } else {
            a = k.amax[b * 64 + lane];
          }
        }
#pragma unroll
        for (int o = 1; o < 64; o <<= 1) {
          a = fmaxf(a, __shfl_xor(a, o, 64));
          if (PRO != P2L_PRO_NONE) { ms = fmaxf(ms, __shfl_xor(ms, o, 64)); mt_ = fmaxf(mt_, __shfl_xor(mt_, o, 64)); }
        }
        if (PRO != P2L_PRO_NONE && k.amax_in != nullptr) a = (k.amax_in_applied ? a : ms * a + mt_) * 1.001f;
        float xs, inv_x;
        h2_scales(__builtin_bit_cast(unsigned, a), xs, inv_x);
        if (lane == 0) { scl[2 * t] = xs; scl[2 * t + 1] = inv_x * inv_w; }
      }
      __syncthreads();
    }
// ... 112 lines not shown
      *reinterpret_cast<f32x4*>(Bs + (tid + 256 * it) * 4) = wr[it];
  };

  f32x16 acc[2];
#pragma unroll
  for (int j = 0; j < 2; ++j)
#pragma unroll
    for (int r = 0; r < 16; ++r) acc[j][r] = 0.f;

  const int a_row = wave * 32 + l31;
  const int a_h = h2_chunk(lhi, a_row) * 4, a_m = h2_chunk(2 + lhi, a_row) * 4;
  const int b_h = h2_chunk(lhi, l31) * 4, b_m = h2_chunk(2 + lhi, l31) * 4;
  const int nstages = k.Cin / KS;
  const int st_lo = SM ? (int)blockIdx.y * k.chunks_per_split : 0;
  const int st_hi = SM ? min(nstages, st_lo + k.chunks_per_split) : nstages;
  using S0_ = std::integral_constant<int, 0>;
  using S1_ = std::integral_constant<int, NSET - 1>;
  auto stage = [&](int st, auto P_, auto Q_, auto FULL_) {
    constexpr bool full = decltype(FULL_)::value;
    const bool more = full || st + 1 < st_hi;
    if (DEEP) {
      if (more && !(P2L_PW_ABL & 2)) load_b(st + 1);
      if ((full || st + 2 < st_hi) && !(P2L_PW_ABL & 2)) load_a(st + 2, P_);
    } else if (more && !(P2L_PW_ABL & 2)) {
      load_a(st + 1, P_);
      load_b(st + 1);
    }
#pragma unroll
    for (int sub = 0; sub < PWH_SUB; ++sub) {
      const float* ar = As + (sub * 128 + a_row) * 16;
      const h16x8 ah = *reinterpret_cast<const h16x8*>(ar + ((sub & 1) ? a_m : a_h));
      const h16x8 am = *reinterpret_cast<const h16x8*>(ar + ((sub & 1) ? a_h : a_m));
#pragma unroll
      for (int j = 0; j < 2; ++j) {
        const float* br = Bs + (sub * 64 + j * 32 + l31) * 16;
        const h16x8 bh = *reinterpret_cast<const h16x8*>(br + b_h);
        const h16x8 bm = *reinterpret_cast<const h16x8*>(br + b_m);
        f32x16 t = acc[j];
        if (!(P2L_PW_ABL & 8)) {
        t = __builtin_amdgcn_mfma_f32_32x32x16_f16(am, bh, t, 0, 0, 0);
        t = __builtin_amdgcn_mfma_f32_32x32x16_f16(ah, bm, t, 0, 0, 0);
        t = __builtin_amdgcn_mfma_f32_32x32x16_f16(ah, bh, t, 0, 0, 0);
        } else { t[0] += (float)am[0] * (float)bh[0] + (float)ah[1] * (float)bm[1]; }
        acc[j] = t;
      }
    }
    if (!(P2L_PW_ABL & 16)) __syncthreads();
    if (more && !(P2L_PW_ABL & 1)) write_lds(Q_, st + 1);
    if (!(P2L_PW_ABL & 16)) __syncthreads();
  };
  load_a(st_lo, S0_{});
  load_b(st_lo);
  if (!SM && DEEP && PRO != P2L_PRO_NONE) {
    const float* ps = k.pro_s + (size_t)b0 * k.pro_bstride;
    const float* pt = k.pro_t + (size_t)b0 * k.pro_bstride;
    for (int c = tid * 4; c < k.Cin; c += 1024) {
      *reinterpret_cast<f32x4*>(st_lds + c) = *reinterpret_cast<const f32x4*>(ps + c);
      *reinterpret_cast<f32x4*>(st_lds + k.Cin + c) = *reinterpret_cast<const f32x4*>(pt + c);
    }
    __syncthreads();
  }
  write_lds(S0_{}, st_lo);
  if (DEEP && st_lo + 1 < st_hi) load_a(st_lo + 1, S1_{});
  __syncthreads();
  if (DEEP) {
    int st = st_lo;
    for (; st + 3 < st_hi; st += 2) {
      stage(st, S0_{}, S1_{}, std::true_type{});
      stage(st + 1, S1_{}, S0_{}, std::true_type{});
    }
    for (; st < st_hi; st += 2) {
      stage(st, S0_{}, S1_{}, std::false_type{});
      if (st + 1 < st_hi) stage(st + 1, S1_{}, S0_{}, std::false_type{});
    }
  } else {
    for (int st = st_lo; st < st_hi; ++st) stage(st, S0_{}, S0_{}, std::false_type{});
  }
  if (!SM) {
#pragma unroll
    for (int j = 0; j < 2; ++j)
#pragma unroll
      for (int r = 0; r < 16; ++r) acc[j][r] *= out_scale;
    if (!(P2L_PW_ABL & 32) || acc[0][0] == 12345.678f)
    epilogue_vec<2>(k, acc, smem, wave, lane, b0, y0, x0, n0, tile_in_image, 0, 0, 0);
    return;
  }
#pragma unroll
  for (int g = 0; g < 4; ++g) {
    const int Q = wave * 8 + 2 * g + lhi;
    const float os = scl[2 * (Q >> (k.tw_log + k.th_log - 2)) + 1];
#pragma unroll
    for (int j = 0; j < 2; ++j)
#pragma unroll
      for (int s = 0; s < 4; ++s) acc[j][4 * g + s] *= os;
  }
  if (k.splitk > 1) {
    const size_t mtot = (size_t)k.B * k.H * k.W;
#pragma unroll
    for (int g = 0; g < 4; ++g) {
      const int Q = wave * 8 + 2 * g + lhi;
      const int qx = Q & ((TW >> 1) - 1);
      const int qy = (Q >> (k.tw_log - 1)) & ((TH >> 1) - 1);
      const int b = b0 + (Q >> (k.tw_log + k.th_log - 2));
      if (b >= k.B) continue;
      const size_t pix0 = ((size_t)b * k.H + y0 + 2 * qy) * k.W + x0 + 2 * qx;
#pragma unroll
      for (int j = 0; j < 2; ++j) {
        float* wp = k.ws + ((size_t)blockIdx.y * mtot + pix0) * k.Cout + n0 + j * 32 + l31;
        wp[0] = acc[j][g * 4 + 0];
        wp[k.Cout] = acc[j][g * 4 + 1];
        wp[(size_t)k.W * k.Cout] = acc[j][g * 4 + 2];
        wp[(size_t)(k.W + 1) * k.Cout] = acc[j][g * 4 + 3];
      }
    }
    return;
  }
  __syncthreads();
  epilogue_vec<2>(k, acc, smem, wave, lane, b0, y0, x0, n0, tile_in_image, 0, 0, 0);
}

__global__ void pw_wmax_kernel(const float* w, size_t n, unsigned* tail) {
  float mx = 0.f;
  for (size_t i = (size_t)blockIdx.x * 256 + threadIdx.x; i < n; i += (size_t)gridDim.x * 256)
    mx = fmaxf(mx, fabsf(w[i]));
#pragma unroll
  for (int o = 1; o < 64; o <<= 1) mx = fmaxf(mx, __shfl_xor(mx, o, 64));
  if ((threadIdx.x & 63) == 0) atomicMax(tail, __builtin_bit_cast(unsigned, mx));
}
__global__ void pw_pack_h2_kernel(const float* w, float* dst, int O, int I, int N_pad, int K_pad,
                                  int flip, const unsigned* tail) {
  const size_t idx = (size_t)blockIdx.x * 256 + threadIdx.x;
  const size_t total = (size_t)(K_pad >> 4) * N_pad * 2;
  if (idx >= total) return;
  float scale, inv;
  h2_scales(tail[0], scale, inv);
  const int kh = (int)(idx & 1);
  size_t q = idx >> 1;
  const int n = (int)(q % N_pad);
  const int cc = (int)(q / N_pad);
  const int N = flip ? I : O, K = flip ? O : I;
  h16x8 ph, pm;
  for (int e = 0; e < 8; ++e) {
    const int kk = cc * 16 + kh * 8 + e;
    float v = 0.f;
    if (n < N && kk < K) v = flip ? w[(size_t)kk * I + n] : w[(size_t)n * I + kk];
    const float x = v * scale;
    const _Float16 h = (_Float16)x;
    ph[e] = h; pm[e] = (_Float16)(x - (float)h);
  }
  const int row = n & 31;
  char* rb = reinterpret_cast<char*>(dst) + (((size_t)cc * (N_pad >> 5) + (n >> 5)) * 32 + row) * 64;
  *reinterpret_cast<h16x8*>(rb + h2_chunk(kh, row) * 16) = ph;
  *reinterpret_cast<h16x8*>(rb + h2_chunk(2 + kh, row) * 16) = pm;
}

}

extern "C" size_t p2l_pw_h2_weight_floats(int N_pad, int K_pad) { return (size_t)N_pad * K_pad + 4; }
int p2l_pw_pack_h2(const float* w_oihw, int O, int I, int N_pad, int K_pad, int flip, float* dst,
                   hipStream_t st) {
  unsigned* tail = reinterpret_cast<unsigned*>(dst + (size_t)N_pad * K_pad);
  if (hipMemsetAsync(tail, 0, 16, st) != hipSuccess) return P2L_ELAUNCH;
  const size_t nw = (size_t)O * I;
  hipLaunchKernelGGL(pw_wmax_kernel, dim3((unsigned)(cdiv(nw, 256) < 256 ? cdiv(nw, 256) : 256)), dim3(256), 0, st,
                     w_oihw, nw, tail);
  const size_t total = (size_t)(K_pad >> 4) * N_pad * 2;
  hipLaunchKernelGGL(pw_pack_h2_kernel, dim3(cdiv(total, 256)), dim3(256), 0, st, w_oihw, dst, O, I, N_pad,
                     K_pad, flip, tail);
  return p2l_check_launch();
}

int p2l_pw_launch(const ConvK& k, int pro, hipStream_t st) {
  dim3 grid(k.n_mtiles * k.n_ntiles), block(256);
#define P2L_PW(PRO)                                                                          \
  do {                                                                                       \
    static std::atomic<bool> attr_set{false};                                                \
    if (!attr_set) {                                                                         \
      (void)hipFuncSetAttribute((const void*)pw_bf3_kernel<PRO, 32>,                         \
                                hipFuncAttributeMaxDynamicSharedMemorySize, 160 * 1024);     \
      attr_set = true;                                                                       \
    }                                                                                        \
    hipLaunchKernelGGL((pw_bf3_kernel<PRO, 32>), grid, block, PwCfg<32>::LDS_BYTES, st, k);  \
  } while (0)
#define P2L_PWH(PRO, SMV)                                                                    \
  do {                                                                                       \
    static std::atomic<bool> attr_set{false};                                                \
    if (!attr_set) {                                                                         \
      (void)hipFuncSetAttribute((const void*)pw_h2_kernel<PRO, SMV>,                         \
                                hipFuncAttributeMaxDynamicSharedMemorySize, 160 * 1024);     \
      attr_set = true;                                                                       \
    }                                                                                        \
    hipLaunchKernelGGL((pw_h2_kernel<PRO, SMV>), gridh, block,                               \
                       PWH_LDS_BYTES + 128 + ((!SMV && PRO != P2L_PRO_NONE) ? (size_t)k.Cin * 8 : 0), st, k); \
  } while (0)
  if (k.amax_in != nullptr || k.amax != nullptr) {
    const bool sm = k.amax != nullptr;
    dim3 gridh(k.n_mtiles * k.n_ntiles, sm ? k.splitk : 1);
    if (sm) {
      if (pro == P2L_PRO_NONE) P2L_PWH(P2L_PRO_NONE, true);
      else if (pro == P2L_PRO_AFFINE_RELU) P2L_PWH(P2L_PRO_AFFINE_RELU, true);
      else P2L_PWH(P2L_PRO_AFFINE, true);
      return p2l_check_launch();
    }
    if (pro == P2L_PRO_NONE) P2L_PWH(P2L_PRO_NONE, false);
    else if (pro == P2L_PRO_AFFINE_RELU) P2L_PWH(P2L_PRO_AFFINE_RELU, false);
    else P2L_PWH(P2L_PRO_AFFINE, false);
    return p2l_check_launch();
  }
#undef P2L_PWH
  if (pro == P2L_PRO_NONE) P2L_PW(P2L_PRO_NONE);
  else if (pro == P2L_PRO_AFFINE_RELU) P2L_PW(P2L_PRO_AFFINE_RELU);
  else P2L_PW(P2L_PRO_AFFINE);
#undef P2L_PW
  return p2l_check_launch();
}
```

### pix2latent_amd/csrc/p2l_wino.hip

```cpp
#include "p2l_conv_k.h"

#include <atomic>
#include <type_traits>

using namespace p2lconv;

namespace {

constexpr int WN_THREADS = 256;
constexpr int WN_RAW_PITCH = 24;
constexpr int WN_RAW_ROWS = 10 * 18;
constexpr int WN_RAW_FLOATS = WN_RAW_ROWS * WN_RAW_PITCH;
constexpr int WN_V_ROWS = 16 * 32;
constexpr int WN_DUMP_PITCH = 32;
constexpr size_t WN_LDS_BYTES = (size_t)(WN_RAW_FLOATS + WN_V_ROWS * 24) * sizeof(float);
static_assert(16 * 32 * WN_DUMP_PITCH <= WN_RAW_FLOATS + WN_V_ROWS * 24, "epilogue dump fits");

__device__ __forceinline__ void store_split(float* Vs, int row, int v, const f32x4 x) {
  bf16x4 ph, pm, pl;
  split3(x, ph, pm, pl);
  char* rb = reinterpret_cast<char*>(Vs) + row * 96 + (v & 1) * 8;
  char* rq = rb + bf3_chunk(v >> 1, row) * 16;
  *reinterpret_cast<bf16x4*>(rq) = ph;
  *reinterpret_cast<bf16x4*>(rq + 32) = pm;
// ... 161 lines not shown
#pragma unroll
    for (int fi = 0; fi < 4; ++fi)
#pragma unroll
      for (int r = 0; r < 16; ++r) {
        const int tile = (r & 3) + 8 * (r >> 2) + 4 * lhi;
        dump[((4 * wave + fi) * 32 + tile) * WN_DUMP_PITCH + l31] = acc[fi][j][r];
      }
    __syncthreads();
    const int nb = n0 + j * 32;
    if (nb + e_c4 * 4 < k.n_store) {
      f32x4 T[2][4];
#pragma unroll
      for (int jj = 0; jj < 4; ++jj) {
        const f32x4 m0 = *reinterpret_cast<const f32x4*>(dump + ((0 + jj) * 32 + e_t) * WN_DUMP_PITCH + e_c4 * 4);
        const f32x4 m1 = *reinterpret_cast<const f32x4*>(dump + ((4 + jj) * 32 + e_t) * WN_DUMP_PITCH + e_c4 * 4);
        const f32x4 m2 = *reinterpret_cast<const f32x4*>(dump + ((8 + jj) * 32 + e_t) * WN_DUMP_PITCH + e_c4 * 4);
        const f32x4 m3 = *reinterpret_cast<const f32x4*>(dump + ((12 + jj) * 32 + e_t) * WN_DUMP_PITCH + e_c4 * 4);
        T[0][jj] = (m0 + m1) + m2;
        T[1][jj] = (m1 - m2) - m3;
      }
      f32x4 v[4];
#pragma unroll
      for (int i = 0; i < 2; ++i) {
        v[2 * i + 0] = ((T[i][0] + T[i][1]) + T[i][2]) * k.alpha;
        v[2 * i + 1] = ((T[i][1] - T[i][2]) - T[i][3]) * k.alpha;
      }
      epi_item(k, v, b, y0 + 2 * ety, x0 + 2 * etx, nb + e_c4 * 4, 0, 0, 0, S);
    }
    if (k.arb_x != nullptr) {
      epi_arb_reduce<32, 8>(k, S, smem, wave, lane, tid,
                            (size_t)b * k.arb_nblk + tile_in_image, nb);
      S = EpiSums();
    }
    __syncthreads();
  }
}

__device__ __forceinline__ const char* sgpr_ptr(const char* p) {
  const unsigned long long v = reinterpret_cast<unsigned long long>(p);
  const unsigned lo = __builtin_amdgcn_readfirstlane((unsigned)v);
  const unsigned hi = __builtin_amdgcn_readfirstlane((unsigned)(v >> 32));
  return reinterpret_cast<const char*>(((unsigned long long)hi << 32) | lo);
}

constexpr int W16_THREADS = 512;
constexpr int W16_RAW_ROWS = 18 * 18;
constexpr int W16_RAW_FLOATS = W16_RAW_ROWS * WN_RAW_PITCH;
constexpr int W16_V_FLOATS = 16 * 64 * 16;
constexpr size_t W16_LDS_BYTES = (size_t)(W16_RAW_FLOATS + 2 * W16_V_FLOATS) * sizeof(float);
static_assert(W16_LDS_BYTES <= 160 * 1024, "one block per CU");
static_assert(16 * 64 * WN_DUMP_PITCH <= 2 * W16_V_FLOATS, "epilogue dump fits");
constexpr size_t W8_LDS_BYTES = (size_t)(10 * 18 * WN_RAW_PITCH + 2 * 16 * 32 * 16) * sizeof(float);

struct TxTable {
  int slot[48];
  constexpr TxTable() : slot{} {
    constexpr int seq[28] = {0 * 8 + 0, -1, 0 * 8 + 1, -1, 0 * 8 + 2, 0 * 8 + 3,
                             1 * 8 + 0, -1, 1 * 8 + 1, -1, 1 * 8 + 2, 1 * 8 + 3, 1 * 8 + 4, 1 * 8 + 5,
                             2 * 8 + 0, -1, 2 * 8 + 1, -1, 2 * 8 + 2, 2 * 8 + 3,
                             3 * 8 + 0, -1, 3 * 8 + 1, -1, 3 * 8 + 2, 3 * 8 + 3, 3 * 8 + 4, 3 * 8 + 5};
    int n = 0;
    for (int g = 0; g < 48; ++g) {
      const int q = g % 12;
      slot[g] = -1;
      if (g < 8 || q == 9 || q == 11) continue;
      if (n < 28) slot[g] = seq[n];
      ++n;
    }
  }
};
constexpr TxTable kTx{};

struct TxTableH {
  int slot[24];
  constexpr TxTableH() : slot{} {
    constexpr int seq[20] = {0 * 8 + 0, 0 * 8 + 1, 0 * 8 + 2, 0 * 8 + 3,
                             1 * 8 + 0, 1 * 8 + 1, 1 * 8 + 2, 1 * 8 + 3, 1 * 8 + 4, 1 * 8 + 5,
                             2 * 8 + 0, 2 * 8 + 1, 2 * 8 + 2, 2 * 8 + 3,
                             3 * 8 + 0, 3 * 8 + 1, 3 * 8 + 2, 3 * 8 + 3, 3 * 8 + 4, 3 * 8 + 5};
    for (int g = 0; g < 24; ++g) slot[g] = g < 4 ? -1 : seq[g - 4];
  }
};
constexpr TxTableH kTxH{};
template <int PRO, int ABL = 0, bool H2 = false, int MT = 2>
__global__ __launch_bounds__(256 * MT, 1) void wino16s_conv_kernel(const ConvK k) {
  static_assert(MT == 2 || (MT == 1 && H2), "the 4-wave block exists in the fp16 x 2 arithmetic only");
  constexpr int THREADS = 256 * MT, TILES = 32 * MT, NW = 4 * MT, NF = 4 / MT;
  constexpr int RAW_ROWS = (8 * MT + 2) * 18, RAW_FLOATS = RAW_ROWS * WN_RAW_PITCH, V_FLOATS = 16 * TILES * 16;
  constexpr int FV = TILES * 16;
  extern __shared__ __attribute__((aligned(16))) float smem[];
  float* raw = smem;
  float* Vs = smem + RAW_FLOATS;

  const int tid = threadIdx.x;
  const int lane = tid & 63, wave = __builtin_amdgcn_readfirstlane(tid >> 6);
  const int l31 = lane & 31, lhi = lane >> 5;

  const int swz = xcd_remap(blockIdx.x, gridDim.x);
  const int mt = swz / k.n_ntiles, nt = swz - mt * k.n_ntiles;
  const int tiles_per_image = k.tiles_x * k.tiles_y;
  const int b = __builtin_amdgcn_readfirstlane(mt / tiles_per_image);
  const int tile_in_image = mt - b * tiles_per_image;
  const int by = tile_in_image / k.tiles_x, bx = tile_in_image - by * k.tiles_x;
  const int y0 = by * (8 * MT), x0 = bx * 16, n0 = __builtin_amdgcn_readfirstlane(nt * 64);

  const int z = blockIdx.y;
  const int c_lo = z * k.chunks_per_split;
  const int nchunks = min(k.chunks_per_split, k.nchunks - c_lo);

  float x_scale = 1.f, out_scale = 1.f;

  constexpr int A_ITERS = 3;
  const int sv = tid & 3;
  unsigned a_goff[A_ITERS];
  const int a_loff0 = (tid >> 2) * WN_RAW_PITCH + sv * 4;
  const bool a_third = tid < 4 * (RAW_ROWS - THREADS / 2);
  unsigned a_valid = 0;
#pragma unroll
  for (int it = 0; it < A_ITERS; ++it) {
    const int p = (tid + THREADS * it) >> 2;
    a_goff[it] = 0x80000000u;
    if (p < RAW_ROWS) {
      const int hy = p / 18, hx = p - hy * 18;
      const int iy = y0 + hy - 1, ix = x0 + hx - 1;
      if (iy >= 0 && iy < k.H && ix >= 0 && ix < k.W) {
        a_goff[it] = ((iy * k.W + ix) * k.x_ld + sv * 4) * 4;
        a_valid |= 1u << it;
      }
    }
  }
  const char* ps_img = reinterpret_cast<const char*>(k.pro_s + (size_t)b * k.pro_bstride);
  const char* pt_img = reinterpret_cast<const char*>(k.pro_t + (size_t)b * k.pro_bstride);
  const unsigned s_off = sv * 16;
  f32x4 xr[A_ITERS], sr, tr;
  const __amdgpu_buffer_rsrc_t x_rs = __builtin_amdgcn_make_buffer_rsrc(
      const_cast<char*>(sgpr_ptr(reinterpret_cast<const char*>(k.x + (size_t)b * k.H * k.W * k.x_ld))), 0,
      __builtin_amdgcn_readfirstlane(k.H * k.W * k.x_ld * 4), 0x00020000);
  auto load_raw = [&](int c) {
#pragma unroll
    for (int it = 0; it < A_ITERS; ++it)
      xr[it] = __builtin_bit_cast(f32x4, __builtin_amdgcn_raw_buffer_load_b128(x_rs, a_goff[it], (c_lo + c) * 64, 0));
    if (PRO != P2L_PRO_NONE) {
      sr = *reinterpret_cast<const f32x4*>(ps_img + (c_lo + c) * 64 + s_off);
      tr = *reinterpret_cast<const f32x4*>(pt_img + (c_lo + c) * 64 + s_off);
    }
  };
  auto write_raw1 = [&](int it) {
    if (it == 2 && !a_third) return;
    f32x4 v = xr[it];
    if (PRO != P2L_PRO_NONE) {
      v = v * sr + tr;
      if (PRO == P2L_PRO_AFFINE_RELU) {
        v.x = fmaxf(v.x, 0.f); v.y = fmaxf(v.y, 0.f);
        v.z = fmaxf(v.z, 0.f); v.w = fmaxf(v.w, 0.f);
      }
    }
    if (PRO != P2L_PRO_NONE && !((a_valid >> it) & 1u)) v = f32x4{0.f, 0.f, 0.f, 0.f};
    if (H2) v = v * x_scale;
    *reinterpret_cast<f32x4*>(raw + a_loff0 + it * (THREADS / 4) * WN_RAW_PITCH) = v;
  };

  const int th = __builtin_amdgcn_readfirstlane(tid / (THREADS / 2));
  const int tt = (tid >> 2) & (TILES - 1), tv = tid & 3;
  const int tty = tt >> 3, ttx = tt & 7;
  const float* t_src = raw + (2 * tty * 18 + 2 * ttx) * WN_RAW_PITCH + tv * 4;
  const int t_dst = tt * 16 + ((tv ^ ((tt >> 2) & 3)) << 2);
  f32x4 tq[2], tRa, tRb;
  f32x4 tR2;
  auto t_load = [&](int part, int h) {
// ... 264 lines not shown
      for (int w = 0; w < NW; ++w) { a = fmaxf(a, raw[w * 4]); ms = fmaxf(ms, raw[w * 4 + 1]); mt = fmaxf(mt, raw[w * 4 + 2]); }
      __syncthreads();
      if (PRO != P2L_PRO_NONE) a = (bound ? ms * a + mt : a) * 1.001f;
    } else {
      a = k.amax[b * 64 + lane];
#pragma unroll
      for (int o = 1; o < 64; o <<= 1) a = fmaxf(a, __shfl_xor(a, o, 64));
    }
    float inv_x, sw, inv_w;
    h2_scales(__builtin_amdgcn_readfirstlane(__builtin_bit_cast(unsigned, a)), x_scale, inv_x);
    h2_scales(__builtin_amdgcn_readfirstlane(k.w_tail[0]), sw, inv_w);
    out_scale = inv_x * inv_w;
  }

#pragma unroll
  for (int it = 0; it < A_ITERS; ++it) write_raw1(it);
  __syncthreads();
  if (nchunks > 1) load_raw(1);
#pragma unroll
  for (int part = 0; part < 4; ++part) {
    t_load(part, 0); t_rows(part, 0); t_load(part, 1); t_rows(part, 1);
    t_cols(part, 0, Vs);
    if (part & 1) { t_cols(part, 1, Vs); t_cols(part, 2, Vs); }
  }
  __syncthreads();
  using T_ = std::true_type; using F_ = std::false_type;
  if ((ABL & 1) && MT == 2) load_b(0, 1, 0);
  P2L_TR(1, 63);
  for (int c = 0; c + 1 < nchunks; ++c) {
    float* Vc = Vs + (c & 1) * V_FLOATS;
    float* Vn = Vs + ((c + 1) & 1) * V_FLOATS;
    P2L_TR(0, c);
    if constexpr (H2) {
      if (!(ABL & 32) || c == 0) { lda(Vc, 0); hstageH(); }
      P2L_SB();
      using B0_ = std::integral_constant<int, 0>;
      stepH(std::integral_constant<int, 0>{}, T_{}, B0_{}, Vc, Vn, c);
      stepH(std::integral_constant<int, 1>{}, T_{}, B0_{}, Vc, Vn, c);
      stepH(std::integral_constant<int, 2>{}, T_{}, B0_{}, Vc, Vn, c);
      stepH(std::integral_constant<int, 3>{}, T_{}, B0_{}, Vc, Vn, c);
    } else {
      if (!(ABL & 32) || c == 0) { lda(Vc, 0); hstage(); }
      P2L_SB();
      step(std::integral_constant<int, 0>{}, T_{}, Vc, Vn, c);
      step(std::integral_constant<int, 1>{}, T_{}, Vc, Vn, c);
      step(std::integral_constant<int, 2>{}, T_{}, Vc, Vn, c);
      step(std::integral_constant<int, 3>{}, T_{}, Vc, Vn, c);
    }
    if (!(ABL & 4)) __syncthreads();
    P2L_TR(5, c);
  }
  {
    const int c = nchunks - 1;
    float* Vc = Vs + (c & 1) * V_FLOATS;
    lda(Vc, 0);
    if constexpr (H2) {
      hstageH();
      P2L_SB();
      using B0_ = std::integral_constant<int, 0>;
      stepH(std::integral_constant<int, 0>{}, F_{}, B0_{}, Vc, Vc, c);
      stepH(std::integral_constant<int, 1>{}, F_{}, B0_{}, Vc, Vc, c);
      stepH(std::integral_constant<int, 2>{}, F_{}, B0_{}, Vc, Vc, c);
      stepH(std::integral_constant<int, 3>{}, F_{}, B0_{}, Vc, Vc, c);
    } else {
      hstage();
      P2L_SB();
      step(std::integral_constant<int, 0>{}, F_{}, Vc, Vc, c);
      step(std::integral_constant<int, 1>{}, F_{}, Vc, Vc, c);
      step(std::integral_constant<int, 2>{}, F_{}, Vc, Vc, c);
      step(std::integral_constant<int, 3>{}, F_{}, Vc, Vc, c);
    }
    __syncthreads();
  }
  P2L_TR(2, 63); P2L_TR(0, 62);
#undef P2L_TX
#undef P2L_PIN
#undef P2L_MF
#undef P2L_SB

  float* dump = Vs;
  const int e_t = tid >> 3, e_c4 = tid & 7;
  const int ety = e_t >> 3, etx = e_t & 7;
  float* red = raw;
  const bool split = k.splitk > 1;
  const float alpha = (split ? 1.f : k.alpha) * out_scale;
  float blk_amax = 0.f, blk_amaxp = 0.f;
#pragma unroll
  for (int j = 0; j < 2; ++j) {
#pragma unroll
    for (int fi = 0; fi < NF; ++fi)
#pragma unroll
      for (int m = 0; m < MT; ++m)
#pragma unroll
        for (int r = 0; r < 16; ++r) {
          const int tile = m * 32 + (r & 3) + 8 * (r >> 2) + 4 * lhi;
          dump[((NF * wave + fi) * TILES + tile) * WN_DUMP_PITCH + l31] = acc[fi][m][j][r];
        }
    if (j == 0) { P2L_TR(1, 62); }
    __syncthreads();
    if (j == 0) { P2L_TR(2, 62); }
    const int nb = n0 + j * 32;
    EpiSums S;
    S.amax = blk_amax; S.amaxp = blk_amaxp;
    if (nb + e_c4 * 4 < k.n_store) {
      f32x4 T[2][4];
#pragma unroll
      for (int jj = 0; jj < 4; ++jj) {
        const f32x4 m0 = *reinterpret_cast<const f32x4*>(dump + ((0 + jj) * TILES + e_t) * WN_DUMP_PITCH + e_c4 * 4);
        const f32x4 m1 = *reinterpret_cast<const f32x4*>(dump + ((4 + jj) * TILES + e_t) * WN_DUMP_PITCH + e_c4 * 4);
        const f32x4 m2 = *reinterpret_cast<const f32x4*>(dump + ((8 + jj) * TILES + e_t) * WN_DUMP_PITCH + e_c4 * 4);
        const f32x4 m3 = *reinterpret_cast<const f32x4*>(dump + ((12 + jj) * TILES + e_t) * WN_DUMP_PITCH + e_c4 * 4);
        T[0][jj] = (m0 + m1) + m2;
        T[1][jj] = (m1 - m2) - m3;
      }
      f32x4 v[4];
#pragma unroll
      for (int i = 0; i < 2; ++i) {
        v[2 * i + 0] = ((T[i][0] + T[i][1]) + T[i][2]) * alpha;
        v[2 * i + 1] = ((T[i][1] - T[i][2]) - T[i][3]) * alpha;
      }
      if (j == 0) { P2L_TR(3, 62); }
      if (split) {
        const size_t pix = ((size_t)b * k.H + y0 + 2 * ety) * k.W + x0 + 2 * etx;
        float* wp = k.ws + (((size_t)z * k.B * k.H * k.W + pix) * k.Cout + nb + e_c4 * 4);
        *reinterpret_cast<f32x4*>(wp) = v[0];
        *reinterpret_cast<f32x4*>(wp + k.Cout) = v[1];
        *reinterpret_cast<f32x4*>(wp + (size_t)k.W * k.Cout) = v[2];
        *reinterpret_cast<f32x4*>(wp + (size_t)(k.W + 1) * k.Cout) = v[3];
      } else if (ABL & 128) {
        float* yp0 = k.y + (((size_t)b * k.H + y0 + 2 * ety) * k.W + x0 + 2 * etx) * k.y_ld + nb + e_c4 * 4;
        *reinterpret_cast<f32x4*>(yp0) = v[0];
        *reinterpret_cast<f32x4*>(yp0 + k.y_ld) = v[1];
        *reinterpret_cast<f32x4*>(yp0 + (size_t)k.W * k.y_ld) = v[2];
        *reinterpret_cast<f32x4*>(yp0 + (size_t)(k.W + 1) * k.y_ld) = v[3];
      } else if (ABL & 256) {
        if (v[0].x == 123.456f) k.y[0] = v[1].x + v[2].x + v[3].x;
      } else {
        epi_item(k, v, b, y0 + 2 * ety, x0 + 2 * etx, nb + e_c4 * 4, 0, 0, 0, S);
      }
    }
    if (j == 0) { P2L_TR(4, 62); }
    if (k.arb_x != nullptr && !split) {
      f32x4 sgx = S.sgx, sg = S.sg;
#pragma unroll
      for (int o = 8; o < 64; o <<= 1) {
        sgx.x += __shfl_xor(sgx.x, o, 64); sgx.y += __shfl_xor(sgx.y, o, 64);
        sgx.z += __shfl_xor(sgx.z, o, 64); sgx.w += __shfl_xor(sgx.w, o, 64);
        sg.x += __shfl_xor(sg.x, o, 64); sg.y += __shfl_xor(sg.y, o, 64);
        sg.z += __shfl_xor(sg.z, o, 64); sg.w += __shfl_xor(sg.w, o, 64);
      }
      if (lane < 8) {
        *reinterpret_cast<f32x4*>(red + wave * 32 + lane * 4) = sgx;
        *reinterpret_cast<f32x4*>(red + NW * 32 + wave * 32 + lane * 4) = sg;
      }
      __syncthreads();
      if (tid < 32 * MT && nb + (tid & 31) < k.n_store) {
        const int g = tid >> 5, col = tid & 31;
        const float* r0 = red + g * 128 + col;
        const float s0 = (r0[0] + r0[32]) + (r0[64] + r0[96]);
        const float s1 = (r0[NW * 32] + r0[NW * 32 + 32]) + (r0[NW * 32 + 64] + r0[NW * 32 + 96]);
        const size_t slot = (size_t)b * k.arb_nblk + (size_t)(MT * by + g) * k.tiles_x + bx;
        const size_t o = slot * k.Cout + nb + col;
        k.arb_partial[o] = s0;
        k.arb_partial[(size_t)k.B * k.arb_nblk * k.Cout + o] = s1;
      }
    }
    blk_amax = S.amax; blk_amaxp = S.amaxp;
    __syncthreads();
    P2L_TR(3 + j, 63);
  }
#undef P2L_TR
  if ((k.amax_out != nullptr || k.amax_outp != nullptr) && !split) {
#pragma unroll
    for (int o = 1; o < 64; o <<= 1) {
      blk_amax = fmaxf(blk_amax, __shfl_xor(blk_amax, o, 64));
      blk_amaxp = fmaxf(blk_amaxp, __shfl_xor(blk_amaxp, o, 64));
    }
    if (lane == 0) {
      const size_t t16 = MT == 2 ? (size_t)tile_in_image : (size_t)(by >> 1) * k.tiles_x + bx;
      const size_t slot = (size_t)b * k.amax_out_n + (t16 * k.n_ntiles + (n0 >> 6)) * 8 + (MT == 2 ? 0 : (by & 1) * 4) + wave;
      if (k.amax_out != nullptr) k.amax_out[slot] = blk_amax;
      if (k.amax_outp != nullptr) k.amax_outp[slot] = blk_amaxp;
    }
  }
}

__global__ void wino_pack_kernel(const float* w, float* dst, int O, int I, int N_pad, int K_pad,
                                 int transpose_flip) {
  const size_t idx = (size_t)blockIdx.x * 256 + threadIdx.x;
  const int n_t32 = N_pad >> 5;
  const size_t total = (size_t)(K_pad >> 4) * 16 * n_t32 * 64;
  if (idx >= total) return;
  const int lane = (int)(idx & 63);
  size_t q = idx >> 6;
  const int jn = (int)(q % n_t32); q /= n_t32;
  const int f = (int)(q & 15);
  const int cc = (int)(q >> 4);
  const int n = jn * 32 + (lane & 31);
  const int fi = f >> 2, fj = f & 3;
  const double G[4][3] = {{1, 0, 0}, {.5, .5, .5}, {.5, -.5, .5}, {0, 0, 1}};
  const int N = transpose_flip ? I : O, K = transpose_flip ? O : I;
  bf16x8 p1, p2, p3;
  for (int e = 0; e < 8; ++e) {
    const int kk = cc * 16 + (lane >> 5) * 8 + e;
    double u = 0.0;
    if (n < N && kk < K) {
      for (int a = 0; a < 3; ++a)
        for (int bb = 0; bb < 3; ++bb) {
          const float g = transpose_flip ? w[(((size_t)kk * I + n) * 3 + (2 - a)) * 3 + (2 - bb)]
                                         : w[(((size_t)n * I + kk) * 3 + a) * 3 + bb];
          u += G[fi][a] * (double)g * G[fj][bb];
        }
    }
    const float x = (float)u;
    const __bf16 h = (__bf16)x;
    const float r1 = x - (float)h;
    const __bf16 m = (__bf16)r1;
    const float r2 = r1 - (float)m;
    p1[e] = h; p2[e] = m; p3[e] = (__bf16)r2;
  }
  bf16x8* out = reinterpret_cast<bf16x8*>(dst) +
                ((((size_t)cc * 16 + f) * n_t32 + jn) * 3) * 64 + lane;
  out[0] = p1; out[64] = p2; out[128] = p3;
}

__global__ void wino_wmax_kernel(const float* w, size_t n, unsigned* tail) {
  float mx = 0.f;
  for (size_t i = (size_t)blockIdx.x * 256 + threadIdx.x; i < n; i += (size_t)gridDim.x * 256)
    mx = fmaxf(mx, fabsf(w[i]));
#pragma unroll
  for (int o = 1; o < 64; o <<= 1) mx = fmaxf(mx, __shfl_xor(mx, o, 64));
  if ((threadIdx.x & 63) == 0) atomicMax(tail, __builtin_bit_cast(unsigned, mx));
}
__global__ void wino_pack_h2_kernel(const float* w, float* dst, int O, int I, int N_pad, int K_pad,
                                    int transpose_flip, const unsigned* tail) {
  const size_t idx = (size_t)blockIdx.x * 256 + threadIdx.x;
  const int n_t32 = N_pad >> 5;
  const size_t total = (size_t)(K_pad >> 4) * 16 * n_t32 * 64;
  if (idx >= total) return;
  float scale, inv;
  h2_scales(tail[0], scale, inv);
  const int lane = (int)(idx & 63);
  size_t q = idx >> 6;
  const int jn = (int)(q % n_t32); q /= n_t32;
  const int f = (int)(q & 15);
  const int cc = (int)(q >> 4);
  const int n = jn * 32 + (lane & 31);
  const int fi = f >> 2, fj = f & 3;
  const double G[4][3] = {{1, 0, 0}, {.5, .5, .5}, {.5, -.5, .5}, {0, 0, 1}};
  const int N = transpose_flip ? I : O, K = transpose_flip ? O : I;
  h16x8 p1, p2;
  for (int e = 0; e < 8; ++e) {
    const int kk = cc * 16 + (lane >> 5) * 8 + e;
    double u = 0.0;
    if (n < N && kk < K) {
      for (int a = 0; a < 3; ++a)
        for (int bb = 0; bb < 3; ++bb) {
          const float g = transpose_flip ? w[(((size_t)kk * I + n) * 3 + (2 - a)) * 3 + (2 - bb)]
                                         : w[(((size_t)n * I + kk) * 3 + a) * 3 + bb];
          u += G[fi][a] * (double)g * G[fj][bb];
        }
    }
    const float x = (float)u * scale;
    const _Float16 h = (_Float16)x;
    p1[e] = h; p2[e] = (_Float16)(x - (float)h);
// ... 5 lines not shown
template <int PRO>
__global__ __launch_bounds__(256) void wino_amax_kernel(const ConvK k) {
  const int b = blockIdx.y;
  const int q4 = k.Cin >> 2;
  const unsigned total = (unsigned)k.H * k.W * q4;
  const float* xi = k.x + (size_t)b * k.H * k.W * k.x_ld;
  float mx = 0.f;
  for (unsigned i = blockIdx.x * 256 + threadIdx.x; i < total; i += 64 * 256) {
    const unsigned pix = i / q4, c4 = i - pix * q4;
    f32x4 v = *reinterpret_cast<const f32x4*>(xi + (size_t)pix * k.x_ld + c4 * 4);
    if (PRO != P2L_PRO_NONE) {
      const f32x4 sr = *reinterpret_cast<const f32x4*>(k.pro_s + (size_t)b * k.pro_bstride + c4 * 4);
      const f32x4 tr = *reinterpret_cast<const f32x4*>(k.pro_t + (size_t)b * k.pro_bstride + c4 * 4);
      v = v * sr + tr;
      if (PRO == P2L_PRO_AFFINE_RELU) {
        v.x = fmaxf(v.x, 0.f); v.y = fmaxf(v.y, 0.f); v.z = fmaxf(v.z, 0.f); v.w = fmaxf(v.w, 0.f);
      }
    }
    mx = fmaxf(fmaxf(mx, fmaxf(fabsf(v.x), fabsf(v.y))), fmaxf(fabsf(v.z), fabsf(v.w)));
  }
#pragma unroll
  for (int o = 1; o < 64; o <<= 1) mx = fmaxf(mx, __shfl_xor(mx, o, 64));
  __shared__ float red[4];
  if ((threadIdx.x & 63) == 0) red[threadIdx.x >> 6] = mx;
  __syncthreads();
  if (threadIdx.x == 0) k.amax[b * 64 + blockIdx.x] = fmaxf(fmaxf(red[0], red[1]), fmaxf(red[2], red[3]));
}

}

extern "C" size_t p2l_wino_weight_floats(int N_pad, int K_pad) {
  return (size_t)N_pad * K_pad * 24;
}
extern "C" size_t p2l_wino_h2_weight_floats(int N_pad, int K_pad) {
  return (size_t)N_pad * K_pad * 16 + 4;
}

extern "C" int p2l_wino_split_factor(int H, int W, int Cin, int Cout) {
#ifdef P2L_NO_WINO_SLICES
  return 1;
#endif
  if (H % 16 || W % 16 || Cout % 64 || Cin % 16) return 1;
  const int per_image = (H / 8) * (W / 16) * (Cout / 64);
  if (per_image >= 64 || per_image < 16) return 1;
  int s = 64 / per_image;
  const int nchunks = Cin / 16;
  while (s > 1 && nchunks / s < 8) s >>= 1;
  return s;
}

extern "C" int p2l_wino_weight_ok(int N_pad, int K_pad) {
  return N_pad % 64 == 0 && K_pad % 16 == 0;
}

int p2l_wino_pack(const float* w_oihw, int O, int I, int N_pad, int K_pad, int transpose_flip,
                  float* dst, hipStream_t st) {
  const size_t total = (size_t)(K_pad >> 4) * 16 * (N_pad >> 5) * 64;
  hipLaunchKernelGGL(wino_pack_kernel, dim3(cdiv(total, 256)), dim3(256), 0, st, w_oihw, dst, O,
                     I, N_pad, K_pad, transpose_flip);
  float* h2 = dst + p2l_wino_weight_floats(N_pad, K_pad);
  unsigned* tail = reinterpret_cast<unsigned*>(h2 + (size_t)N_pad * K_pad * 16);
  if (hipMemsetAsync(tail, 0, 16, st) != hipSuccess) return P2L_ELAUNCH;
  const size_t nw = (size_t)O * I * 9;
  hipLaunchKernelGGL(wino_wmax_kernel, dim3((unsigned)(cdiv(nw, 256) < 256 ? cdiv(nw, 256) : 256)), dim3(256),
                     0, st, w_oihw, nw, tail);
  hipLaunchKernelGGL(wino_pack_h2_kernel, dim3(cdiv(total, 256)), dim3(256), 0, st, w_oihw, h2, O,
                     I, N_pad, K_pad, transpose_flip, tail);
  return p2l_check_launch();
}

int p2l_amax_launch(const ConvK& k, int pro, hipStream_t st) {
  if (pro == P2L_PRO_NONE) hipLaunchKernelGGL(wino_amax_kernel<P2L_PRO_NONE>, dim3(64, k.B), dim3(256), 0, st, k);
  else if (pro == P2L_PRO_AFFINE_RELU) hipLaunchKernelGGL(wino_amax_kernel<P2L_PRO_AFFINE_RELU>, dim3(64, k.B), dim3(256), 0, st, k);
  else hipLaunchKernelGGL(wino_amax_kernel<P2L_PRO_AFFINE>, dim3(64, k.B), dim3(256), 0, st, k);
  return p2l_check_launch();
}

#ifdef P2L_LAB
static int g_lab_abl = 0;
static void* g_lab_trace = nullptr;
extern "C" int p2l_lab_set(int abl, void* trace) { g_lab_abl = abl; g_lab_trace = trace; return P2L_OK; }
#endif

int p2l_wino_launch(const ConvK& k_in, int pro, hipStream_t st) {
  ConvK k = k_in;
  if (k.H % 16 == 0 && k.W % 16 == 0 && !(k.form & P2L_FORM_WINO_8X16)) {
    k.tiles_y = k.H / 16;
    k.n_mtiles = k.B * k.tiles_x * k.tiles_y;
    if (k.splitk <= 1) { k.ws = nullptr; k.splitk = 1; k.chunks_per_split = k.nchunks; }
    dim3 grid(k.n_mtiles * k.n_ntiles, k.splitk), block(W16_THREADS);
#ifdef P2L_LAB
    if (k.splitk <= 1) k.ws = (float*)g_lab_trace;
#define P2L_W16L(ABL)                                                                        \
  case ABL: {                                                                                \
    (void)hipFuncSetAttribute((const void*)wino16s_conv_kernel<P2L_PRO_NONE, ABL>,           \
                              hipFuncAttributeMaxDynamicSharedMemorySize, 160 * 1024);       \
    hipLaunchKernelGGL((wino16s_conv_kernel<P2L_PRO_NONE, ABL>), grid, block, W16_LDS_BYTES, st, k); \
    return p2l_check_launch();                                                               \
  }
    if (pro == P2L_PRO_NONE && k.amax != nullptr && (k.form & P2L_FORM_WINO_H2_8X16)) {
      ConvK k8 = k;
      k8.tiles_y = k.H / 8;
      k8.n_mtiles = k.B * k.tiles_x * k8.tiles_y;
      dim3 grid8(k8.n_mtiles * k8.n_ntiles, k8.splitk), block8(256);
#define P2L_W8LH(ABL)                                                                        \
  case ABL: {                                                                                \
    (void)hipFuncSetAttribute((const void*)wino16s_conv_kernel<P2L_PRO_NONE, ABL, true, 1>,  \
                              hipFuncAttributeMaxDynamicSharedMemorySize, 160 * 1024);       \
    hipLaunchKernelGGL(wino_amax_kernel<P2L_PRO_NONE>, dim3(64, k.B), dim3(256), 0, st, k8); \
    hipLaunchKernelGGL((wino16s_conv_kernel<P2L_PRO_NONE, ABL, true, 1>), grid8, block8, W8_LDS_BYTES, st, k8); \
    return p2l_check_launch();                                                               \
  }
      switch (g_lab_abl) {
        P2L_W8LH(0) P2L_W8LH(1) P2L_W8LH(2) P2L_W8LH(4) P2L_W8LH(8) P2L_W8LH(16) P2L_W8LH(64) P2L_W8LH(3) P2L_W8LH(67) P2L_W8LH(79)
        default: return P2L_EINVAL;
      }
#undef P2L_W8LH
    }
    if (pro == P2L_PRO_NONE && k.amax != nullptr) {
#define P2L_W16LH(ABL)                                                                       \
  case ABL: {                                                                                \
    (void)hipFuncSetAttribute((const void*)wino16s_conv_kernel<P2L_PRO_NONE, ABL, true>,     \
                              hipFuncAttributeMaxDynamicSharedMemorySize, 160 * 1024);       \
    hipLaunchKernelGGL(wino_amax_kernel<P2L_PRO_NONE>, dim3(64, k.B), dim3(256), 0, st, k);  \
    hipLaunchKernelGGL((wino16s_conv_kernel<P2L_PRO_NONE, ABL, true>), grid, block, W16_LDS_BYTES, st, k); \
    return p2l_check_launch();                                                               \
  }
      switch (g_lab_abl) {
        P2L_W16LH(0) P2L_W16LH(1) P2L_W16LH(2) P2L_W16LH(4) P2L_W16LH(8) P2L_W16LH(16) P2L_W16LH(64)
        P2L_W16LH(3) P2L_W16LH(10) P2L_W16LH(67) P2L_W16LH(75) P2L_W16LH(79) P2L_W16LH(111) P2L_W16LH(128) P2L_W16LH(256)
        default: return P2L_EINVAL;
      }
#undef P2L_W16LH
    }
    if (pro == P2L_PRO_NONE && k.amax == nullptr) {
      switch (g_lab_abl) {
        P2L_W16L(0) P2L_W16L(1) P2L_W16L(2) P2L_W16L(4) P2L_W16L(8) P2L_W16L(16) P2L_W16L(64)
        P2L_W16L(3) P2L_W16L(10) P2L_W16L(67) P2L_W16L(75) P2L_W16L(79) P2L_W16L(111)
        default: return P2L_EINVAL;
      }
    }
#undef P2L_W16L
#endif
#define P2L_W16S(PRO)                                                                        \
  do {                                                                                       \
    static std::atomic<bool> attr_set{false};                                                \
    if (!attr_set) {                                                                         \
      (void)hipFuncSetAttribute((const void*)wino16s_conv_kernel<PRO>,                       \
                                hipFuncAttributeMaxDynamicSharedMemorySize, 160 * 1024);     \
      attr_set = true;                                                                       \
    }                                                                                        \
    hipLaunchKernelGGL(wino16s_conv_kernel<PRO>, grid, block, W16_LDS_BYTES, st, k);         \
  } while (0)
#define P2L_W16H(PRO, MTV, LDSB)                                                             \
  do {                                                                                       \
    static std::atomic<bool> attr_set{false};                                                \
    if (!attr_set) {                                                                         \
      (void)hipFuncSetAttribute((const void*)wino16s_conv_kernel<PRO, 0, true, MTV>,         \
                                hipFuncAttributeMaxDynamicSharedMemorySize, 160 * 1024);     \
      attr_set = true;                                                                       \
    }                                                                                        \
    if (k.amax_in == nullptr)                                                                \
      hipLaunchKernelGGL(wino_amax_kernel<PRO>, dim3(64, k.B), dim3(256), 0, st, k);         \
    hipLaunchKernelGGL((wino16s_conv_kernel<PRO, 0, true, MTV>), grid, block, LDSB, st, k);  \
  } while (0)
    if (k.amax != nullptr) {
      const long blocks16 = (long)k.n_mtiles * k.n_ntiles * k.splitk;
      const bool half = (k.form & P2L_FORM_WINO_H2_8X16) ||
                        (!(k.form & P2L_FORM_WINO_H2_16X16) && blocks16 <= 128);
      if (half) {
        k.tiles_y = k.H / 8;
        k.n_mtiles = k.B * k.tiles_x * k.tiles_y;
        grid = dim3(k.n_mtiles * k.n_ntiles, k.splitk);
        block = dim3(256);
        if (pro == P2L_PRO_NONE) P2L_W16H(P2L_PRO_NONE, 1, W8_LDS_BYTES);
        else if (pro == P2L_PRO_AFFINE_RELU) P2L_W16H(P2L_PRO_AFFINE_RELU, 1, W8_LDS_BYTES);
        else P2L_W16H(P2L_PRO_AFFINE, 1, W8_LDS_BYTES);
        return p2l_check_launch();
      }
      if (pro == P2L_PRO_NONE) P2L_W16H(P2L_PRO_NONE, 2, W16_LDS_BYTES);
      else if (pro == P2L_PRO_AFFINE_RELU) P2L_W16H(P2L_PRO_AFFINE_RELU, 2, W16_LDS_BYTES);
      else P2L_W16H(P2L_PRO_AFFINE, 2, W16_LDS_BYTES);
      return p2l_check_launch();
    }
#undef P2L_W16H
    if (pro == P2L_PRO_NONE) P2L_W16S(P2L_PRO_NONE);
    else if (pro == P2L_PRO_AFFINE_RELU) P2L_W16S(P2L_PRO_AFFINE_RELU);
    else P2L_W16S(P2L_PRO_AFFINE);
#undef P2L_W16S
    return p2l_check_launch();
  }
  dim3 grid(k.n_mtiles * k.n_ntiles), block(WN_THREADS);
#define P2L_WN(PRO)                                                                          \
  do {                                                                                       \
    static std::atomic<bool> attr_set{false};                                                \
    if (!attr_set) {                                                                         \
      (void)hipFuncSetAttribute((const void*)wino_conv_kernel<PRO>,                          \
                                hipFuncAttributeMaxDynamicSharedMemorySize, 160 * 1024);     \
      attr_set = true;                                                                       \
    }                                                                                        \
    hipLaunchKernelGGL(wino_conv_kernel<PRO>, grid, block, WN_LDS_BYTES, st, k);             \
  } while (0)
  if (pro == P2L_PRO_NONE) P2L_WN(P2L_PRO_NONE);
  else if (pro == P2L_PRO_AFFINE_RELU) P2L_WN(P2L_PRO_AFFINE_RELU);
  else P2L_WN(P2L_PRO_AFFINE);
#undef P2L_WN
  return p2l_check_launch();
}
```

Before: 1190.

## Compile specialized conv epilogues per fusion class via template parameter

Adds an epilogue-class enum that describes which fusions a convolution's output stage needs (bias, residual, relu, pool, mask, arb backward). The Winograd fp16x2, pointwise and direct h2 kernels are templated on that class, so each common case gets a compile-time specialized epilogue. This replaces the generic runtime-branching epilogue and is meant to cut branches, register pressure and dead loads. It adds many kernel instantiations, which means more code size and compile time, plus a query API that reports which class a layer gets.

```diff
diff --git a/include/p2l.h b/include/p2l.h
--- a/include/p2l.h
+++ b/include/p2l.h
@@ -155,8 +155,12 @@
   P2L_FORM_H2R_SEQ_EPI = 512,
   P2L_FORM_NO_SP_SKIP = 1024,
   P2L_FORM_NO_SP_PAIR = 2048,
-  P2L_FORM_SP_PAIR = 4096
+  P2L_FORM_SP_PAIR = 4096,
+  P2L_FORM_GENERIC_EPI = 8192
 };
+int p2l_conv_epilogue_class(const P2LConv* d, const P2LConvExtra* ex, const P2LArb* arb, const float* bias,
+                            const float* res, const float* mask, const float* y, const float* yp,
+                            const void* workspace, size_t ws_bytes);
 int p2l_wino_split_factor(int H, int W, int Cin, int Cout);
 int p2l_pack_conv_weight_bf3w(const float* w_oihw, int O, int I, int taps, int N_pad,
                               int K_pad, int transpose_flip, float* w_packed, void* stream);
diff --git a/pix2latent_amd/_native.py b/pix2latent_amd/_native.py
--- a/pix2latent_amd/_native.py
+++ b/pix2latent_amd/_native.py
@@ -168,6 +168,7 @@
 FORM_NO_SP_PAIR = 2048
 FORM_SP_PAIR = 4096
 FORM_NO_H2R = 256
+FORM_GENERIC_EPI = 8192
 
 
 def default_wfmt():
@@ -242,7 +243,7 @@
 
 EXPORTS = [
     'p2l_version', 'p2l_strerror', 'p2l_last_hip_error',
-    'p2l_conv_workspace_bytes', 'p2l_conv_amax_slots', 'p2l_selftest_amaxreg', 'p2l_conv_suggest_splitk', 'p2l_conv_fwd', 'p2l_conv_fwd_ex',
+    'p2l_conv_workspace_bytes', 'p2l_conv_amax_slots', 'p2l_conv_epilogue_class', 'p2l_selftest_amaxreg', 'p2l_conv_suggest_splitk', 'p2l_conv_fwd', 'p2l_conv_fwd_ex',
     'p2l_pack_conv_weight', 'p2l_pack_conv_weight_subpix', 'p2l_pack_conv_weight_bf3',
     'p2l_pack_conv_weight_bf3w', 'p2l_packed_weight_floats', 
     'p2l_pack_conv_weight_bf3t',
@@ -320,6 +321,7 @@
             getattr(_lib, name).restype = C.c_size_t
         vp, i32, i64_, f32_ = C.c_void_p, C.c_int, C.c_int64, C.c_float
         _lib.p2l_relu_mask.argtypes = [vp, i32, vp, i32, vp, i32, i64_, i32, vp]
+        _lib.p2l_conv_epilogue_class.argtypes = [vp, vp, vp, vp, vp, vp, vp, vp, vp, C.c_size_t]
         _lib.p2l_tanh_bwd16.argtypes = [vp, vp, i64_, vp]
         _lib.p2l_clamp.argtypes = [vp, i64_, f32_, f32_, vp]
         _lib.p2l_adam_step.argtypes = [vp, vp, vp, vp, i64_, f32_, f32_, f32_, f32_, i32, vp]
diff --git a/pix2latent_amd/csrc/p2l_conv.hip b/pix2latent_amd/csrc/p2l_conv.hip
--- a/pix2latent_amd/csrc/p2l_conv.hip
+++ b/pix2latent_amd/csrc/p2l_conv.hip
@@ -1087,7 +1087,7 @@
                             const float* bias, const float* pro_s,
                             const float* pro_t, const float* res,
                             const float* mask, float* y, float* yp,
-                            void* workspace, size_t ws_bytes, void* stream) {
+                            void* workspace, size_t ws_bytes, void* stream, int* dry_class = nullptr) {
   if (!d || !x || !w) return P2L_EINVAL;
   if (d->taps != 1 && d->taps != 9) return P2L_EINVAL;
   const int kc = (d->taps == 9) ? 16 : (d->Cin % 32 == 0 ? 32 : 16);
@@ -1206,7 +1206,8 @@
   hipStream_t st = (hipStream_t)stream;
 
   int prof_slot = -1;
-  bool prof_ok = g_prof.on;
+  bool prof_ok = g_prof.on && !dry_class;
+  if (dry_class) *dry_class = EPI_GENERIC;
   if (prof_ok) {
     hipStreamCaptureStatus cs = hipStreamCaptureStatusNone;
     if (hipStreamIsCapturing(st, &cs) != hipSuccess || cs != hipStreamCaptureStatusNone) prof_ok = false;
@@ -1258,6 +1259,7 @@
     } else {
       kw.splitk = 1;
     }
+    if (dry_class) { *dry_class = p2l_wino_epi_class(kw, d->pro); return P2L_OK; }
     rc = p2l_wino_launch(kw, d->pro, st);
     if (rc == P2L_OK && wino_sliced) {
       const size_t total = (size_t)k.B * (k.H >> 1) * (k.W >> 1) * (k.n_store >> 2);
@@ -1282,6 +1284,7 @@
     kp.n_ntiles = d->Cout / 64;
     kp.nchunks = d->Cin / 64;
     kp.splitk = 1;
+    if (dry_class) { *dry_class = p2l_pw_epi_class(kp, d->pro); return P2L_OK; }
     rc = p2l_pw_launch(kp, d->pro, st);
     if (prof_slot >= 0) {
       if (k.amax_in != nullptr) g_prof.nprod[prof_slot] = 3;
@@ -1294,6 +1297,7 @@
     const int tm = thin_shape(d);
     const bool geom = k.tw_log == 4 && k.th_log == 3 && k.tb_log == 0 && !k.partial && !(ex && (ex->oscale || ex->noise));
     if (tm == 1 && geom) {
+      if (dry_class) return P2L_OK;
       ConvK kt = k;
       kt.w = w + (size_t)9 * d->Cout * d->Cin * 3 / 2;
       kt.splitk = 1;
@@ -1306,6 +1310,7 @@
       return rc;
     }
     if (tm == 0 && geom && !arb && !res && !mask && d->pool == P2L_POOL_NONE && y) {
+      if (dry_class) return P2L_OK;
       ConvK kt = k;
       kt.w = w + (size_t)9 * d->Cout * d->Cin * 3 / 2;
       kt.nchunks = d->Cin / 16;
@@ -1354,6 +1359,10 @@
       kh.hp = halo_pitch_h2(1 << k.tw_log);
       kh.w = w + (size_t)16 * d->Cout * d->Cin * 3 / 2;
       kh.w_tail = reinterpret_cast<const unsigned*>(kh.w + (size_t)16 * d->Cout * d->Cin);
+      if (dry_class) {
+        *dry_class = d->ups == 3 ? p2l_h2_epi_class(kh, d->pro, 4) : EPI_GENERIC;
+        return P2L_OK;
+      }
       if (kh.amax_in == nullptr) {
         ConvK ka = kh;
         ka.H = k.ibH; ka.W = k.ibW;
@@ -1389,6 +1398,7 @@
     size_t lds_sp = (size_t)(a_lds_sp + 4 * bn) * (bf3 ? 24 : 20) * sizeof(float);
     const size_t lds_epi = (size_t)4 * 32 * (bn + 4) * sizeof(float);
     if (lds_epi > lds_sp) lds_sp = lds_epi;
+    if (dry_class) return P2L_OK;
     dim3 grid(k.n_mtiles * k.n_ntiles, d->ups == 2 ? 4 : 1), block(256);
 #define P2L_LAUNCH_SP(BNV, AIT, PROV)                                                     \
     do {                                                                                  \
@@ -1440,14 +1450,20 @@
     if (p2l_wino_weight_ok(d->Cout, d->Cin))
       kh.w += p2l_wino_weight_floats(d->Cout, d->Cin) + p2l_wino_h2_weight_floats(d->Cout, d->Cin);
     kh.w_tail = reinterpret_cast<const unsigned*>(kh.w + (size_t)9 * d->Cout * d->Cin);
+    const bool small = (a_rows * 4 <= 3 * 256) && TB == 1;
+    const bool h2r = direct_h2r(d) && k.splitk == 1 && !k.partial && TB == 1 && p2l_h2r_takes(kh);
+    if (dry_class) {
+      *dry_class = h2r ? EPI_GENERIC : p2l_h2_epi_class(kh, d->pro, 9);
+      return P2L_OK;
+    }
     if (kh.amax_in == nullptr) {
       rc = p2l_amax_launch(kh, d->pro, st);
       if (rc) return rc;
     }
-    const bool small = (a_rows * 4 <= 3 * 256) && TB == 1;
-    const bool h2r = direct_h2r(d) && k.splitk == 1 && !k.partial && TB == 1 && p2l_h2r_takes(kh);
     rc = h2r ? p2l_h2r_launch(kh, d->pro, st) : p2l_h2_launch(kh, d->pro, 9, bn, small, st);
     if (prof_slot >= 0) { g_prof.nprod[prof_slot] = 3; g_prof.fam[prof_slot] = h2r ? P2L_PROF_FAM_DIRECT_H2R : P2L_PROF_FAM_DIRECT_H2; }
+  } else if (dry_class) {
+    return P2L_OK;
   } else
   if (d->taps == 9) {
     const bool small = (a_rows * 4 <= 3 * 256) && TB == 1;
@@ -1510,6 +1526,24 @@
                                void* stream) {
   return conv_launch_impl(d, nullptr, ex, x, w, bias, pro_s, pro_t, res, mask, y, yp, workspace,
                           ws_bytes, stream);
+}
+
+extern "C" int p2l_conv_epilogue_class(const P2LConv* d, const P2LConvExtra* ex, const P2LArb* arb,
+                                       const float* bias, const float* res, const float* mask, const float* y,
+                                       const float* yp, const void* workspace, size_t ws_bytes) {
+  if (!d) return 0;
+  const float* some = reinterpret_cast<const float*>(d);
+  P2LConv dd = *d;
+  if (arb) {
+    if (dd.ups == 3) dd.pool = P2L_POOL_NONE;
+    if (effective_splitk(&dd) <= 1) dd.splitk = 1;
+    if (dd.pool == P2L_POOL_SUM) { yp = y; y = nullptr; }
+  }
+  int ec = 0;
+  const int rc = conv_launch_impl(&dd, arb, arb ? nullptr : ex, some, some, arb ? nullptr : bias, some, some,
+                                  arb ? nullptr : res, arb ? nullptr : mask, const_cast<float*>(y),
+                                  const_cast<float*>(yp), const_cast<void*>(workspace), ws_bytes, nullptr, &ec);
+  return rc == P2L_OK ? ec : 0;
 }
 
 extern "C" int p2l_conv_arb_fusable(const P2LConv* d) {
diff --git a/pix2latent_amd/csrc/p2l_conv_k.h b/pix2latent_amd/csrc/p2l_conv_k.h
--- a/pix2latent_amd/csrc/p2l_conv_k.h
+++ b/pix2latent_amd/csrc/p2l_conv_k.h
@@ -269,6 +269,169 @@
   }
 }
 
+enum {
+  EPI_GENERIC = 0,
+  EPI_BIAS_PS = 1,
+  EPI_BIAS_RES_PS = 2,
+  EPI_BIAS_RESUP_PS = 3,
+  EPI_BIAS_RELU = 4,
+  EPI_BIAS_RELU_POOL = 5,
+  EPI_MASK = 6,
+  EPI_ARB = 7,
+  EPI_ARB_SKIP = 8,
+  EPI_ARB_SKIP_UP = 9,
+  EPI_N_CLASSES = 10
+};
+struct EpiDesc {
+  bool bias;
+  int res;
+  bool relu, mask;
+  int pool;
+  int amax;
+  int arb;
+};
+constexpr EpiDesc epi_desc(int ec) {
+  switch (ec) {
+    case EPI_BIAS_PS:        return {true, 0, false, false, 0, 2, 0};
+    case EPI_BIAS_RES_PS:    return {true, 1, false, false, 0, 2, 0};
+    case EPI_BIAS_RESUP_PS:  return {true, 2, false, false, 0, 2, 0};
+    case EPI_BIAS_RELU:      return {true, 0, true, false, 0, 1, 0};
+    case EPI_BIAS_RELU_POOL: return {true, 0, true, false, 2, 1, 0};
+    case EPI_MASK:           return {false, 0, false, true, 0, 1, 0};
+    case EPI_ARB:            return {false, 0, false, false, 0, 1, 1};
+    case EPI_ARB_SKIP:       return {false, 0, false, false, 0, 1, 2};
+    case EPI_ARB_SKIP_UP:    return {false, 0, false, false, 0, 1, 3};
+    default:                 return {false, 0, false, false, 0, 0, 0};
+  }
+}
+inline int epi_class(const ConvK& k) {
+#ifdef P2L_AB_GENERIC_EPI
+  return EPI_GENERIC;
+#endif
+  if (k.form & P2L_FORM_GENERIC_EPI) return EPI_GENERIC;
+  if (k.partial || k.oscale || k.noise || !k.y || k.sp_mode == 1 || k.splitk > 1) return EPI_GENERIC;
+  if (!k.amax_out) return EPI_GENERIC;
+  if (k.arb_x) {
+    if (k.arb_nomask || k.pool != P2L_POOL_NONE || k.amax_outp) return EPI_GENERIC;
+    return !k.arb_skip ? EPI_ARB : (k.arb_skip_ups ? EPI_ARB_SKIP_UP : EPI_ARB_SKIP);
+  }
+  const bool ps = k.amax_ps != nullptr;
+  if (k.bias && !k.mask && k.act == P2L_ACT_NONE && k.pool == P2L_POOL_NONE && ps && !k.amax_outp)
+    return !k.res ? EPI_BIAS_PS : (k.res_ups ? EPI_BIAS_RESUP_PS : EPI_BIAS_RES_PS);
+  if (k.bias && !k.res && !k.mask && k.act == P2L_ACT_RELU && !ps) {
+    if (k.pool == P2L_POOL_NONE && !k.amax_outp) return EPI_BIAS_RELU;
+    if (k.pool == P2L_POOL_MAX && k.yp && k.amax_outp) return EPI_BIAS_RELU_POOL;
+    return EPI_GENERIC;
+  }
+  if (!k.bias && !k.res && k.mask && k.act == P2L_ACT_NONE && k.pool == P2L_POOL_NONE && !ps && !k.amax_outp)
+    return EPI_MASK;
+  return EPI_GENERIC;
+}
+inline int epi_class_wino(const ConvK& k, int pro) {
+  const int ec = epi_class(k);
+  if (pro == P2L_PRO_AFFINE_RELU) return ec == EPI_BIAS_PS ? ec : EPI_GENERIC;
+  if (pro == P2L_PRO_NONE)
+    return (ec == EPI_BIAS_RELU || ec == EPI_BIAS_RELU_POOL || ec == EPI_MASK || ec == EPI_ARB) ? ec : EPI_GENERIC;
+  return EPI_GENERIC;
+}
+inline int epi_class_h2(const ConvK& k, int pro, int taps) {
+  if (pro != P2L_PRO_NONE) return EPI_GENERIC;
+  const int ec = epi_class(k);
+  if (taps == 9) return ec == EPI_ARB ? ec : EPI_GENERIC;
+  if (taps == 4 && k.sp_mode == 2 && !k.sp_skip) return ec == EPI_ARB ? ec : EPI_GENERIC;
+  return EPI_GENERIC;
+}
+inline int epi_class_pw(const ConvK& k, int pro) {
+  const int ec = epi_class(k);
+  if (pro == P2L_PRO_AFFINE_RELU)
+    return (ec == EPI_BIAS_PS || ec == EPI_BIAS_RES_PS || ec == EPI_BIAS_RESUP_PS) ? ec : EPI_GENERIC;
+  if (pro == P2L_PRO_NONE)
+    return (ec == EPI_ARB || ec == EPI_ARB_SKIP || ec == EPI_ARB_SKIP_UP) ? ec : EPI_GENERIC;
+  return EPI_GENERIC;
+}
+
+template <int EC>
+__device__ __forceinline__ void epi_item_ct(const ConvK& k, f32x4 (&v)[4], int b, int oy0, int ox0,
+                                            int n, EpiSums& S) {
+  constexpr EpiDesc D = epi_desc(EC);
+  static_assert(EC > EPI_GENERIC && EC < EPI_N_CLASSES, "a class of its own");
+  const unsigned OW = (unsigned)k.obW;
+  const unsigned pix0 = ((unsigned)(b * k.obH) + (unsigned)oy0) * OW + (unsigned)ox0;
+  const unsigned sub[4] = {0u, 1u, OW, OW + 1u};
+  const unsigned ppix = (unsigned)((b * (k.H >> 1) + (oy0 >> 1)) * (k.W >> 1) + (ox0 >> 1));
+#pragma unroll
+  for (int s = 0; s < 4; ++s) asm("" : "+v"(v[s]));
+  if constexpr (D.arb == 0) {
+    f32x4 bias4 = {0, 0, 0, 0};
+    if constexpr (D.bias) bias4 = ld4(k.bias, (unsigned)n);
+    f32x4 ns4 = {1.f, 1.f, 1.f, 1.f}, nt4 = {0, 0, 0, 0};
+    if constexpr (D.amax == 2) {
+      ns4 = ld4(k.amax_ps, (unsigned)(b * k.amax_pbstride + n));
+      nt4 = ld4(k.amax_pt, (unsigned)(b * k.amax_pbstride + n));
+    }
+#pragma unroll
+    for (int s = 0; s < 4; ++s) {
+      const unsigned pix = pix0 + sub[s];
+      f32x4 t = v[s] + bias4;
+      if constexpr (D.res != 0) t += ld4(k.res, (D.res == 2 ? ppix : pix) * (unsigned)k.res_ld + (unsigned)n);
+      if constexpr (D.relu) t = act4(t, P2L_ACT_RELU);
+      if constexpr (D.mask) {
+        const f32x4 m = ld4(k.mask, pix * (unsigned)k.mask_ld + (unsigned)n);
+        t.x = m.x > 0.f ? t.x : 0.f; t.y = m.y > 0.f ? t.y : 0.f;
+        t.z = m.z > 0.f ? t.z : 0.f; t.w = m.w > 0.f ? t.w : 0.f;
+      }
+      st4(k.y, pix * (unsigned)k.y_ld + (unsigned)n, t);
+      if constexpr (D.amax == 2) S.amax = absmax4(S.amax, t * ns4 + nt4);
+      else if constexpr (D.amax == 1) S.amax = absmax4(S.amax, t);
+      v[s] = t;
+    }
+    if constexpr (D.pool != 0) {
+      f32x4 p;
+      p.x = fmaxf(fmaxf(v[0].x, v[1].x), fmaxf(v[2].x, v[3].x));
+      p.y = fmaxf(fmaxf(v[0].y, v[1].y), fmaxf(v[2].y, v[3].y));
+      p.z = fmaxf(fmaxf(v[0].z, v[1].z), fmaxf(v[2].z, v[3].z));
+      p.w = fmaxf(fmaxf(v[0].w, v[1].w), fmaxf(v[2].w, v[3].w));
+      st4(k.yp, ppix * (unsigned)k.yp_ld + (unsigned)n, p);
+      if constexpr (D.pool == 2) S.amaxp = absmax4(S.amaxp, p);
+    }
+  } else {
+    const f32x4 s4 = ld4(k.arb_s, (unsigned)(b * k.arb_bstride + n));
+    const f32x4 t4 = ld4(k.arb_t, (unsigned)(b * k.arb_bstride + n));
+    const bool has_skip = D.arb >= 2 && n < k.arb_skip_C;
+#pragma unroll
+    for (int s = 0; s < 4; ++s) {
+      const unsigned pix = pix0 + sub[s];
+      const f32x4 xv = ld4(k.arb_x, pix * (unsigned)k.arb_x_ld + (unsigned)n);
+      const f32x4 pre = xv * s4 + t4;
+      f32x4 g = v[s];
+      g.x = pre.x > 0.f ? g.x : 0.f; g.y = pre.y > 0.f ? g.y : 0.f;
+      g.z = pre.z > 0.f ? g.z : 0.f; g.w = pre.w > 0.f ? g.w : 0.f;
+      f32x4 o = g * s4;
+      if (has_skip) {
+        const unsigned ld = (unsigned)k.arb_skip_ld;
+        if constexpr (D.arb == 3) {
+          const unsigned W2 = 2u * (unsigned)k.W;
+          const unsigned cq = ((unsigned)(b * 2 * k.H + 2 * (oy0 + (s >> 1)))) * W2 + 2u * (unsigned)(ox0 + (s & 1));
+          o += (ld4(k.arb_skip, cq * ld + n) + ld4(k.arb_skip, (cq + 1) * ld + n)) +
+               (ld4(k.arb_skip, (cq + W2) * ld + n) + ld4(k.arb_skip, (cq + W2 + 1) * ld + n));
+        } else {
+          o += ld4(k.arb_skip, pix * ld + (unsigned)n);
+        }
+      }
+      st4(k.y, pix * (unsigned)k.y_ld + (unsigned)n, o);
+      if constexpr (D.amax != 0) S.amax = absmax4(S.amax, o);
+      S.sgx += g * xv;
+      S.sg += g;
+    }
+  }
+}
+template <int EC>
+__device__ __forceinline__ void epi_item_of(const ConvK& k, f32x4 (&v)[4], int b, int oy0, int ox0,
+                                            int n, int osh, int ph_y, int ph_x, EpiSums& S) {
+  if constexpr (EC == EPI_GENERIC) epi_item(k, v, b, oy0, ox0, n, osh, ph_y, ph_x, S);
+  else epi_item_ct<EC>(k, v, b, oy0, ox0, n, S);
+}
+
 template <int COLS, int C4>
 __device__ __forceinline__ void epi_arb_reduce(const ConvK& k, EpiSums& S, float* smem, int wave,
                                                int lane, int tid, size_t slot, int n0,
@@ -307,11 +470,11 @@
   }
 }
 
-template <int NT>
+template <int NT, int EC = EPI_GENERIC>
 __device__ __forceinline__ void epilogue_vec_items(const ConvK& k, float* smem, int wave, int lane, int b0,
                                                    int y0, int x0, int n0, int tile_in_image, int osh,
                                                    int ph_y, int ph_x);
-template <int NT>
+template <int NT, int EC = EPI_GENERIC>
 __device__ __forceinline__ void epilogue_vec(const ConvK& k, const f32x16 (&acc)[NT],
                                              float* smem, int wave, int lane, int b0, int y0,
                                              int x0, int n0, int tile_in_image, int osh,
@@ -325,13 +488,14 @@
     for (int r = 0; r < 16; ++r)
       tb[((r & 3) + 8 * (r >> 2) + 4 * lhi) * EP + j * 32 + l31] = acc[j][r];
   __syncthreads();
-  epilogue_vec_items<NT>(k, smem, wave, lane, b0, y0, x0, n0, tile_in_image, osh, ph_y, ph_x);
-}
-template <int NT>
+  epilogue_vec_items<NT, EC>(k, smem, wave, lane, b0, y0, x0, n0, tile_in_image, osh, ph_y, ph_x);
+}
+template <int NT, int EC>
 __device__ __forceinline__ void epilogue_vec_items(const ConvK& k, float* smem, int wave, int lane, int b0,
                                                    int y0, int x0, int n0, int tile_in_image, int osh,
                                                    int ph_y, int ph_x) {
   constexpr int COLS = NT * 32, EP = COLS + 4, C4 = COLS / 4, ITEMS = 8 * C4;
+  constexpr EpiDesc D = epi_desc(EC);
   float* tb = smem + wave * 32 * EP;
 
   const int TWh = (1 << k.tw_log) >> 1, THh = (1 << k.th_log) >> 1;
@@ -351,14 +515,14 @@
 #pragma unroll
     for (int s = 0; s < 4; ++s)
       v[s] = *reinterpret_cast<const f32x4*>(tb + (4 * q + s) * EP + c4 * 4) * k.alpha;
-    epi_item(k, v, b, oy0, ox0, n, osh, ph_y, ph_x, Sx);
+    epi_item_of<EC>(k, v, b, oy0, ox0, n, osh, ph_y, ph_x, Sx);
   }
   static_assert(ITEMS == 64 || ITEMS == 128, "one or two items per lane");
-  if (k.arb_x != nullptr)
+  if (EC == EPI_GENERIC ? k.arb_x != nullptr : D.arb != 0)
     epi_arb_reduce<COLS, C4>(k, S, smem, wave, lane, threadIdx.x,
                              (size_t)b0 * k.arb_nblk + tile_in_image, n0, &S2);
   S.amax = fmaxf(S.amax, S2.amax); S.amaxp = fmaxf(S.amaxp, S2.amaxp);
-  if (k.amax_out != nullptr || k.amax_outp != nullptr) {
+  if (EC == EPI_GENERIC ? (k.amax_out != nullptr || k.amax_outp != nullptr) : (D.amax != 0 || D.pool == 2)) {
     float m = S.amax, mp = S.amaxp;
 #pragma unroll
     for (int o = 1; o < 64; o <<= 1) { m = fmaxf(m, __shfl_xor(m, o, 64)); mp = fmaxf(mp, __shfl_xor(mp, o, 64)); }
@@ -366,8 +530,8 @@
       const int nph = osh ? 4 : 1;
       const size_t slot = (size_t)b0 * k.amax_out_n +
                           (((size_t)tile_in_image * k.n_ntiles + n0 / COLS) * nph + (osh ? ph_y * 2 + ph_x : 0)) * 4 + wave;
-      if (k.amax_out != nullptr) k.amax_out[slot] = m;
-      if (k.amax_outp != nullptr) k.amax_outp[slot] = mp;
+      if (EC == EPI_GENERIC ? k.amax_out != nullptr : D.amax != 0) k.amax_out[slot] = m;
+      if (EC == EPI_GENERIC ? k.amax_outp != nullptr : D.pool == 2) k.amax_outp[slot] = mp;
     }
   }
 }
@@ -376,6 +540,9 @@
 }
 
 int p2l_pw_launch(const p2lconv::ConvK& k, int pro, hipStream_t st);
+int p2l_pw_epi_class(const p2lconv::ConvK& k, int pro);
+int p2l_wino_epi_class(const p2lconv::ConvK& k, int pro);
+int p2l_h2_epi_class(const p2lconv::ConvK& k, int pro, int taps);
 
 size_t p2l_thin_weight_floats(int N_pad, int K_pad);
 int p2l_thin_mode(int N_pad, int K_pad);
diff --git a/pix2latent_amd/csrc/p2l_h2.hip b/pix2latent_amd/csrc/p2l_h2.hip
--- a/pix2latent_amd/csrc/p2l_h2.hip
+++ b/pix2latent_amd/csrc/p2l_h2.hip
@@ -15,8 +15,9 @@
 
 #define P2L_WAIT(VM, LGKM) __builtin_amdgcn_s_waitcnt(((VM) & 15) | (7 << 4) | ((LGKM) << 8) | (((VM) >> 4) << 14))
 
-template <int TAPS, int BN, int A_ITERS, int PRO, bool SKIP = false>
+template <int TAPS, int BN, int A_ITERS, int PRO, bool SKIP = false, int EC = EPI_GENERIC>
 __global__ __launch_bounds__(256, 2) void conv_h2_kernel(const ConvK k) {
+  static_assert(EC == EPI_GENERIC || TAPS == 9 || (TAPS == 4 && !SKIP), "compiled epilogues: direct 3x3 and sub-pixel input gradient");
   constexpr bool SUBPIX = (TAPS == 4 || TAPS == 8);
   constexpr int NP = (TAPS == 8) ? 2 : 1;
   constexpr int NT = BN / 32;
@@ -404,8 +405,8 @@
                            tile_in_image, 1, ph_y, p);
         }
       } else {
-        epilogue_vec<NT>(k, reinterpret_cast<f32x16 (&)[NT]>(acc[0]), smem, wave, lane, b0, y0, x0, n0, tile_in_image,
-                         sp_fwd ? 1 : 0, ph_y, ph_x);
+        epilogue_vec<NT, EC>(k, reinterpret_cast<f32x16 (&)[NT]>(acc[0]), smem, wave, lane, b0, y0, x0, n0,
+                             tile_in_image, sp_fwd ? 1 : 0, ph_y, ph_x);
       }
     }
   }
@@ -517,6 +518,11 @@
   return (size_t)(main_floats + 2 * TB + 16) * sizeof(float);
 }
 
+int p2l_h2_epi_class(const ConvK& k, int pro, int taps) {
+  if (k.splitk > 1) return EPI_GENERIC;
+  return epi_class_h2(k, pro, taps);
+}
+
 int p2l_h2_launch(const ConvK& k, int pro, int taps, int bn, bool small, hipStream_t st) {
   dim3 grid(k.n_mtiles * k.n_ntiles, taps == 8 ? 2 : (taps == 4 && k.sp_mode == 1) ? 4 : k.splitk), block(256);
   const size_t lds = p2l_h2_lds_bytes(k, taps, bn);
@@ -525,9 +531,10 @@
     if ((TAPS == 4 || TAPS == 8) && k.sp_skip) P2L_H2K(TAPS, BNV, AIT, PROV, (TAPS == 4 || TAPS == 8)); \
     else P2L_H2K(TAPS, BNV, AIT, PROV, false);                                                \
   } while (0)
-#define P2L_H2K(TAPS, BNV, AIT, PROV, SKIPV)                                                  \
+#define P2L_H2K(TAPS, BNV, AIT, PROV, SKIPV) P2L_H2KE(TAPS, BNV, AIT, PROV, SKIPV, EPI_GENERIC)
+#define P2L_H2KE(TAPS, BNV, AIT, PROV, SKIPV, ECV)                                            \
   do {                                                                                        \
-    auto kfn = conv_h2_kernel<TAPS, BNV, AIT, PROV, SKIPV>;                                   \
+    auto kfn = conv_h2_kernel<TAPS, BNV, AIT, PROV, SKIPV, ECV>;                              \
     static std::atomic<bool> attr_set{false};                                                 \
     if (!attr_set) {                                                                          \
       (void)hipFuncSetAttribute((const void*)kfn, hipFuncAttributeMaxDynamicSharedMemorySize, \
@@ -542,7 +549,15 @@
     else if (pro == P2L_PRO_AFFINE_RELU) P2L_H2L(TAPS, BNV, AIT, P2L_PRO_AFFINE_RELU);        \
     else P2L_H2L(TAPS, BNV, AIT, P2L_PRO_AFFINE);                                             \
   } while (0)
-  if (taps == 9) {
+#define P2L_H2E(TAPS, ECV)                                                                    \
+  do {                                                                                        \
+    if (bn == 64) { if (small) P2L_H2KE(TAPS, 64, 3, P2L_PRO_NONE, false, ECV); else P2L_H2KE(TAPS, 64, 5, P2L_PRO_NONE, false, ECV); } \
+    else          { if (small) P2L_H2KE(TAPS, 32, 3, P2L_PRO_NONE, false, ECV); else P2L_H2KE(TAPS, 32, 5, P2L_PRO_NONE, false, ECV); } \
+  } while (0)
+  const int ec = p2l_h2_epi_class(k, pro, taps);
+  if (ec == EPI_ARB && taps == 9) P2L_H2E(9, EPI_ARB);
+  else if (ec == EPI_ARB && taps == 4) P2L_H2E(4, EPI_ARB);
+  else if (taps == 9) {
     if (bn == 64) { if (small) P2L_H2P(9, 64, 3); else P2L_H2P(9, 64, 5); }
     else          { if (small) P2L_H2P(9, 32, 3); else P2L_H2P(9, 32, 5); }
   } else if (taps == 8) {
@@ -552,8 +567,10 @@
     if (bn == 64) { if (small) P2L_H2P(4, 64, 3); else P2L_H2P(4, 64, 5); }
     else          { if (small) P2L_H2P(4, 32, 3); else P2L_H2P(4, 32, 5); }
   }
+#undef P2L_H2E
 #undef P2L_H2P
 #undef P2L_H2L
 #undef P2L_H2K
+#undef P2L_H2KE
   return p2l_check_launch();
 }
diff --git a/pix2latent_amd/csrc/p2l_pw.hip b/pix2latent_amd/csrc/p2l_pw.hip
--- a/pix2latent_amd/csrc/p2l_pw.hip
+++ b/pix2latent_amd/csrc/p2l_pw.hip
@@ -165,8 +165,9 @@
 #ifndef P2L_PW_ABL
 #define P2L_PW_ABL 0
 #endif
-template <int PRO, bool SM = false>
+template <int PRO, bool SM = false, int EC = EPI_GENERIC>
 __global__ __launch_bounds__(256, SM ? 3 : 4) void pw_h2_kernel(const ConvK k) {
+  static_assert(!SM || EC == EPI_GENERIC, "the small-grid form keeps the shared item");
   constexpr int KS = 32, VPP = KS / 4;
   constexpr int A_ITERS = 128 * VPP / 256;
   extern __shared__ __attribute__((aligned(16))) float smem[];
@@ -445,7 +446,7 @@
 #pragma unroll
       for (int r = 0; r < 16; ++r) acc[j][r] *= out_scale;
     if (!(P2L_PW_ABL & 32) || acc[0][0] == 12345.678f)
-    epilogue_vec<2>(k, acc, smem, wave, lane, b0, y0, x0, n0, tile_in_image, 0, 0, 0);
+    epilogue_vec<2, EC>(k, acc, smem, wave, lane, b0, y0, x0, n0, tile_in_image, 0, 0, 0);
     return;
   }
 #pragma unroll
@@ -533,6 +534,11 @@
   return p2l_check_launch();
 }
 
+int p2l_pw_epi_class(const ConvK& k, int pro) {
+  if (k.amax_in == nullptr || k.amax != nullptr) return EPI_GENERIC;
+  return epi_class_pw(k, pro);
+}
+
 int p2l_pw_launch(const ConvK& k, int pro, hipStream_t st) {
   dim3 grid(k.n_mtiles * k.n_ntiles), block(256);
 #define P2L_PW(PRO)                                                                          \
@@ -545,15 +551,16 @@
     }                                                                                        \
     hipLaunchKernelGGL((pw_bf3_kernel<PRO, 32>), grid, block, PwCfg<32>::LDS_BYTES, st, k);  \
   } while (0)
-#define P2L_PWH(PRO, SMV)                                                                    \
+#define P2L_PWH(PRO, SMV) P2L_PWHE(PRO, SMV, EPI_GENERIC)
+#define P2L_PWHE(PRO, SMV, ECV)                                                              \
   do {                                                                                       \
     static std::atomic<bool> attr_set{false};                                                \
     if (!attr_set) {                                                                         \
-      (void)hipFuncSetAttribute((const void*)pw_h2_kernel<PRO, SMV>,                         \
+      (void)hipFuncSetAttribute((const void*)pw_h2_kernel<PRO, SMV, ECV>,                    \
                                 hipFuncAttributeMaxDynamicSharedMemorySize, 160 * 1024);     \
       attr_set = true;                                                                       \
     }                                                                                        \
-    hipLaunchKernelGGL((pw_h2_kernel<PRO, SMV>), gridh, block,                               \
+    hipLaunchKernelGGL((pw_h2_kernel<PRO, SMV, ECV>), gridh, block,                          \
                        PWH_LDS_BYTES + 128 + ((!SMV && PRO != P2L_PRO_NONE) ? (size_t)k.Cin * 8 : 0), st, k); \
   } while (0)
   if (k.amax_in != nullptr || k.amax != nullptr) {
@@ -565,12 +572,22 @@
       else P2L_PWH(P2L_PRO_AFFINE, true);
       return p2l_check_launch();
     }
-    if (pro == P2L_PRO_NONE) P2L_PWH(P2L_PRO_NONE, false);
-    else if (pro == P2L_PRO_AFFINE_RELU) P2L_PWH(P2L_PRO_AFFINE_RELU, false);
-    else P2L_PWH(P2L_PRO_AFFINE, false);
+    switch (p2l_pw_epi_class(k, pro)) {
+      case EPI_BIAS_PS:       P2L_PWHE(P2L_PRO_AFFINE_RELU, false, EPI_BIAS_PS); break;
+      case EPI_BIAS_RES_PS:   P2L_PWHE(P2L_PRO_AFFINE_RELU, false, EPI_BIAS_RES_PS); break;
+      case EPI_BIAS_RESUP_PS: P2L_PWHE(P2L_PRO_AFFINE_RELU, false, EPI_BIAS_RESUP_PS); break;
+      case EPI_ARB:           P2L_PWHE(P2L_PRO_NONE, false, EPI_ARB); break;
+      case EPI_ARB_SKIP:      P2L_PWHE(P2L_PRO_NONE, false, EPI_ARB_SKIP); break;
+      case EPI_ARB_SKIP_UP:   P2L_PWHE(P2L_PRO_NONE, false, EPI_ARB_SKIP_UP); break;
+      default:
+        if (pro == P2L_PRO_NONE) P2L_PWH(P2L_PRO_NONE, false);
+        else if (pro == P2L_PRO_AFFINE_RELU) P2L_PWH(P2L_PRO_AFFINE_RELU, false);
+        else P2L_PWH(P2L_PRO_AFFINE, false);
+    }
     return p2l_check_launch();
   }
 #undef P2L_PWH
+#undef P2L_PWHE
   if (pro == P2L_PRO_NONE) P2L_PW(P2L_PRO_NONE);
   else if (pro == P2L_PRO_AFFINE_RELU) P2L_PW(P2L_PRO_AFFINE_RELU);
   else P2L_PW(P2L_PRO_AFFINE);
diff --git a/pix2latent_amd/csrc/p2l_wino.hip b/pix2latent_amd/csrc/p2l_wino.hip
--- a/pix2latent_amd/csrc/p2l_wino.hip
+++ b/pix2latent_amd/csrc/p2l_wino.hip
@@ -267,9 +267,11 @@
   }
 };
 constexpr TxTableH kTxH{};
-template <int PRO, int ABL = 0, bool H2 = false, int MT = 2>
+template <int PRO, int ABL = 0, bool H2 = false, int MT = 2, int EC = EPI_GENERIC>
 __global__ __launch_bounds__(256 * MT, 1) void wino16s_conv_kernel(const ConvK k) {
   static_assert(MT == 2 || (MT == 1 && H2), "the 4-wave block exists in the fp16 x 2 arithmetic only");
+  static_assert(EC == EPI_GENERIC || (H2 && ABL == 0), "compiled epilogues: the fp16 x 2 product kernel");
+  constexpr EpiDesc ED = epi_desc(EC);
   constexpr int THREADS = 256 * MT, TILES = 32 * MT, NW = 4 * MT, NF = 4 / MT;
   constexpr int RAW_ROWS = (8 * MT + 2) * 18, RAW_FLOATS = RAW_ROWS * WN_RAW_PITCH, V_FLOATS = 16 * TILES * 16;
   constexpr int FV = TILES * 16;
@@ -700,7 +702,8 @@
   const int e_t = tid >> 3, e_c4 = tid & 7;
   const int ety = e_t >> 3, etx = e_t & 7;
   float* red = raw;
-  const bool split = k.splitk > 1;
+  const bool split = EC == EPI_GENERIC && k.splitk > 1;
+  const bool with_arb = EC == EPI_GENERIC ? k.arb_x != nullptr : ED.arb != 0;
   const float alpha = (split ? 1.f : k.alpha) * out_scale;
   float blk_amax = 0.f, blk_amaxp = 0.f;
 #pragma unroll
@@ -754,11 +757,11 @@
       } else if (ABL & 256) {
         if (v[0].x == 123.456f) k.y[0] = v[1].x + v[2].x + v[3].x;
       } else {
-        epi_item(k, v, b, y0 + 2 * ety, x0 + 2 * etx, nb + e_c4 * 4, 0, 0, 0, S);
+        epi_item_of<EC>(k, v, b, y0 + 2 * ety, x0 + 2 * etx, nb + e_c4 * 4, 0, 0, 0, S);
       }
     }
     if (j == 0) { P2L_TR(4, 62); }
-    if (k.arb_x != nullptr && !split) {
+    if (with_arb && !split) {
       f32x4 sgx = S.sgx, sg = S.sg;
 #pragma unroll
       for (int o = 8; o < 64; o <<= 1) {
@@ -788,7 +791,7 @@
     P2L_TR(3 + j, 63);
   }
 #undef P2L_TR
-  if ((k.amax_out != nullptr || k.amax_outp != nullptr) && !split) {
+  if (EC == EPI_GENERIC ? ((k.amax_out != nullptr || k.amax_outp != nullptr) && !split) : (ED.amax != 0 || ED.pool == 2)) {
 #pragma unroll
     for (int o = 1; o < 64; o <<= 1) {
       blk_amax = fmaxf(blk_amax, __shfl_xor(blk_amax, o, 64));
@@ -797,8 +800,8 @@
     if (lane == 0) {
       const size_t t16 = MT == 2 ? (size_t)tile_in_image : (size_t)(by >> 1) * k.tiles_x + bx;
       const size_t slot = (size_t)b * k.amax_out_n + (t16 * k.n_ntiles + (n0 >> 6)) * 8 + (MT == 2 ? 0 : (by & 1) * 4) + wave;
-      if (k.amax_out != nullptr) k.amax_out[slot] = blk_amax;
-      if (k.amax_outp != nullptr) k.amax_outp[slot] = blk_amaxp;
+      if (EC == EPI_GENERIC ? k.amax_out != nullptr : ED.amax != 0) k.amax_out[slot] = blk_amax;
+      if (EC == EPI_GENERIC ? k.amax_outp != nullptr : ED.pool == 2) k.amax_outp[slot] = blk_amaxp;
     }
   }
 }
@@ -970,6 +973,12 @@
 extern "C" int p2l_lab_set(int abl, void* trace) { g_lab_abl = abl; g_lab_trace = trace; return P2L_OK; }
 #endif
 
+int p2l_wino_epi_class(const ConvK& k, int pro) {
+  if (k.H % 16 != 0 || k.W % 16 != 0 || (k.form & P2L_FORM_WINO_8X16) || k.amax == nullptr || k.splitk > 1)
+    return EPI_GENERIC;
+  return epi_class_wino(k, pro);
+}
+
 int p2l_wino_launch(const ConvK& k_in, int pro, hipStream_t st) {
   ConvK k = k_in;
   if (k.H % 16 == 0 && k.W % 16 == 0 && !(k.form & P2L_FORM_WINO_8X16)) {
@@ -1040,19 +1049,33 @@
     }                                                                                        \
     hipLaunchKernelGGL(wino16s_conv_kernel<PRO>, grid, block, W16_LDS_BYTES, st, k);         \
   } while (0)
-#define P2L_W16H(PRO, MTV, LDSB)                                                             \
+#define P2L_W16H(PRO, MTV, LDSB) P2L_W16HE(PRO, MTV, LDSB, EPI_GENERIC)
+#define P2L_W16HE(PRO, MTV, LDSB, ECV)                                                       \
   do {                                                                                       \
     static std::atomic<bool> attr_set{false};                                                \
     if (!attr_set) {                                                                         \
-      (void)hipFuncSetAttribute((const void*)wino16s_conv_kernel<PRO, 0, true, MTV>,         \
+      (void)hipFuncSetAttribute((const void*)wino16s_conv_kernel<PRO, 0, true, MTV, ECV>,    \
                                 hipFuncAttributeMaxDynamicSharedMemorySize, 160 * 1024);     \
       attr_set = true;                                                                       \
     }                                                                                        \
     if (k.amax_in == nullptr)                                                                \
       hipLaunchKernelGGL(wino_amax_kernel<PRO>, dim3(64, k.B), dim3(256), 0, st, k);         \
-    hipLaunchKernelGGL((wino16s_conv_kernel<PRO, 0, true, MTV>), grid, block, LDSB, st, k);  \
+    hipLaunchKernelGGL((wino16s_conv_kernel<PRO, 0, true, MTV, ECV>), grid, block, LDSB, st, k); \
   } while (0)
+#define P2L_W16HC(MTV, LDSB)                                                                                \
+  switch (ec) {                                                                                             \
+    case EPI_BIAS_PS:        P2L_W16HE(P2L_PRO_AFFINE_RELU, MTV, LDSB, EPI_BIAS_PS); break;                 \
+    case EPI_BIAS_RELU:      P2L_W16HE(P2L_PRO_NONE, MTV, LDSB, EPI_BIAS_RELU); break;                      \
+    case EPI_BIAS_RELU_POOL: P2L_W16HE(P2L_PRO_NONE, MTV, LDSB, EPI_BIAS_RELU_POOL); break;                 \
+    case EPI_MASK:           P2L_W16HE(P2L_PRO_NONE, MTV, LDSB, EPI_MASK); break;                           \
+    case EPI_ARB:            P2L_W16HE(P2L_PRO_NONE, MTV, LDSB, EPI_ARB); break;                            \
+    default:                                                                                                \
+      if (pro == P2L_PRO_NONE) P2L_W16H(P2L_PRO_NONE, MTV, LDSB);                                           \
+      else if (pro == P2L_PRO_AFFINE_RELU) P2L_W16H(P2L_PRO_AFFINE_RELU, MTV, LDSB);                        \
+      else P2L_W16H(P2L_PRO_AFFINE, MTV, LDSB);                                                             \
+  }
     if (k.amax != nullptr) {
+      const int ec = p2l_wino_epi_class(k, pro);
       const long blocks16 = (long)k.n_mtiles * k.n_ntiles * k.splitk;
       const bool half = (k.form & P2L_FORM_WINO_H2_8X16) ||
                         (!(k.form & P2L_FORM_WINO_H2_16X16) && blocks16 <= 128);
@@ -1061,16 +1084,14 @@
         k.n_mtiles = k.B * k.tiles_x * k.tiles_y;
         grid = dim3(k.n_mtiles * k.n_ntiles, k.splitk);
         block = dim3(256);
-        if (pro == P2L_PRO_NONE) P2L_W16H(P2L_PRO_NONE, 1, W8_LDS_BYTES);
-        else if (pro == P2L_PRO_AFFINE_RELU) P2L_W16H(P2L_PRO_AFFINE_RELU, 1, W8_LDS_BYTES);
-        else P2L_W16H(P2L_PRO_AFFINE, 1, W8_LDS_BYTES);
+        P2L_W16HC(1, W8_LDS_BYTES)
         return p2l_check_launch();
       }
-      if (pro == P2L_PRO_NONE) P2L_W16H(P2L_PRO_NONE, 2, W16_LDS_BYTES);
-      else if (pro == P2L_PRO_AFFINE_RELU) P2L_W16H(P2L_PRO_AFFINE_RELU, 2, W16_LDS_BYTES);
-      else P2L_W16H(P2L_PRO_AFFINE, 2, W16_LDS_BYTES);
+      P2L_W16HC(2, W16_LDS_BYTES)
       return p2l_check_launch();
     }
+#undef P2L_W16HC
+#undef P2L_W16HE
 #undef P2L_W16H
     if (pro == P2L_PRO_NONE) P2L_W16S(P2L_PRO_NONE);
     else if (pro == P2L_PRO_AFFINE_RELU) P2L_W16S(P2L_PRO_AFFINE_RELU);
```

Measured after the change: 1216 (median of 6 runs). 1.02x the previous value.
